# Disty0/sdnq

Hardware: AMD Instinct MI355X
Metric: quantized-matmul GOP/s (SDXL UNet int8 Linear step, bs=1) (higher is better)
Workload: dtype i8; 1 GPU; sdxl_int8: 741 quantized Linear layers of one denoising step, bs=1 (722 w8a8 GEMMs + 19 M=1 layers); parallelism=single GPU, launch=hipGraph replay, activations=bf16, distinct_activation_tensors=446, activation_quant_cache=True, requantized_weight_cache=True, fused_projections=False, linked_projection_groups=71, one_launch_linears=232, weights_dtype=int8, group_size=-1, use_quantized_matmul=True

## Files before the change

include/sdnq_hip.h:

```cpp
#ifndef SDNQ_HIP_H
#define SDNQ_HIP_H

#include <stddef.h>
#include <stdint.h>

#ifdef __cplusplus
extern "C" {
#endif

#define SDNQ_HIP_ABI_VERSION 1

typedef void* sdnq_stream_t;

typedef enum SdnqStatus {
    SDNQ_OK = 0,
    SDNQ_ERR_NULL = -1,
    SDNQ_ERR_DTYPE = -2,
    SDNQ_ERR_SHAPE = -3,
    SDNQ_ERR_ALIGN = -4,
    SDNQ_ERR_UNSUPPORTED = -5,
    SDNQ_ERR_ARCH = -6,
    SDNQ_ERR_LAUNCH = -7,
    SDNQ_ERR_WORKSPACE = -8
} SdnqStatus;

typedef enum SdnqFloat { SDNQ_F32 = 0, SDNQ_BF16 = 1, SDNQ_F16 = 2 } SdnqFloat;

typedef enum SdnqMM { SDNQ_MM_I8 = 0, SDNQ_MM_FP8 = 1, SDNQ_MM_F16 = 2  } SdnqMM;

typedef enum SdnqStorage {
    SDNQ_ST_PACKED_U8 = 0,
    SDNQ_ST_PACKED_I16 = 1,
    SDNQ_ST_RAW8 = 2,
    SDNQ_ST_RAW16 = 3
} SdnqStorage;

typedef enum SdnqKind {
    SDNQ_KIND_INT = 0,
    SDNQ_KIND_UINT = 1,
    SDNQ_KIND_FLOAT = 2,
    SDNQ_KIND_UFLOAT = 3,
    SDNQ_KIND_CODEBOOK = 4
} SdnqKind;

typedef struct SdnqWeight {
    const void* weight;
    const float* scale;
    const float* zero_point;
    const void* svd_up;
    const void* svd_down;
    int32_t n;
    int32_t k;
    int32_t group_size;
    int32_t svd_rank;
    int32_t svd_dtype;
    int32_t storage;
    int32_t kind;
    int32_t bits;
    int32_t exponent;
    int32_t mantissa;
    int32_t native_float;
    int32_t positions;
    int32_t scale_dtype;
} SdnqWeight;

int sdnq_hip_version(void);
const char* sdnq_hip_strerror(int status);
int sdnq_hip_device_supported(int ordinal);

int sdnq_hip_rowquant(const void* x, int x_dtype, int64_t m, int64_t k, int64_t ldx, int mm_dtype,
                      int hadamard_group, void* xq, float* xs, int32_t* rowsum, void* xrot,
                      const void* prefetch, int64_t prefetch_bytes, float* xzp, sdnq_stream_t stream);

int sdnq_hip_rowquant_lp(const void* x, int x_dtype, int64_t m, int64_t k, int64_t ldx, int mm_dtype, int hadamard_group,
                         void* xq, float* xs, int32_t* rowsum, void* xrot, sdnq_stream_t stream);

int sdnq_hip_scaled_mm(int mm_dtype, const void* a, const void* b, const float* sa, const float* sb,
                       const void* bias, int bias_dtype, int bias_ndim, int64_t ld_bias, void* out,
                       int out_dtype, int64_t m, int64_t n, int64_t k, sdnq_stream_t stream);

int sdnq_hip_scaled_mm_tile(int mm_dtype, int out_dtype, int has_bias, int64_t m, int64_t n, int64_t k, int* bm, int* bn, int* threads,
                            int64_t* workgroups);

int sdnq_hip_rowquant_f16(const void* x, int x_dtype, int64_t m, int64_t k, int64_t ldx, void* xq, float* xs, sdnq_stream_t stream);
int sdnq_hip_scaled_mm_f16(const void* a, const void* b, const float* sa, const float* sb, const void* bias, int bias_dtype, int bias_ndim,
                           int64_t ld_bias, void* out, int out_dtype, int64_t m, int64_t n, int64_t k, sdnq_stream_t stream);

int sdnq_hip_lut4_build(const SdnqWeight* w, int mm_dtype, float* ws, int ws_known, void* lut, sdnq_stream_t stream);
int sdnq_hip_scaled_mm_w4(const void* a, const void* codes, const void* lut, const float* sa, const float* sb, const void* bias, int bias_dtype,
                          void* out, int out_dtype, int64_t m, int64_t n, int64_t k, int64_t lda, sdnq_stream_t stream);
int sdnq_hip_scaled_mm_w4_supported(int mm_dtype, int out_dtype, int64_t m, int64_t n, int64_t k);

int sdnq_hip_scaled_mm_lp(int mm_dtype, const void* a, const void* b, const float* sa, const float* sb, const void* bias,
                          int bias_ndim, int64_t ld_bias, const void* t, const void* svd_up, int rank, void* out,
                          int64_t m, int64_t n, int64_t k, sdnq_stream_t stream);

int sdnq_hip_scaled_mm_lp_zp(int mm_dtype, const void* a, const void* b, const float* sa, const float* sb, const void* bias,
                             int bias_ndim, int64_t ld_bias, const void* t, const void* svd_up, int rank, const int32_t* zp_rowsum,
                             const float* zp, void* out, int64_t m, int64_t n, int64_t k, sdnq_stream_t stream);

int sdnq_hip_rowquant_lp_asym(const void* x, int x_dtype, int64_t m, int64_t k, int64_t ldx, int hadamard_group, void* xq, float* xs,
                              float* xzp, int32_t* rowsum, void* xrot, sdnq_stream_t stream);
int sdnq_hip_scaled_mm_lp_uzp(const void* a, const void* b, const float* sa, const float* sb, const void* bias, const int32_t* zp_rowsum,
                              const float* zp, const float* a_zp, const float* w_colsum_scaled, int64_t zp_k, void* out, int64_t m,
                              int64_t n, int64_t k, sdnq_stream_t stream);
int sdnq_hip_scaled_mm_lp_uzp_svd(const void* a, const void* b, const float* sa, const float* sb, const void* bias,
                                  const int32_t* zp_rowsum, const float* zp, const float* a_zp, const float* w_colsum_scaled, int64_t zp_k,
                                  const void* t, const void* svd_up, int rank, void* out, int64_t m, int64_t n, int64_t k,
                                  sdnq_stream_t stream);

int sdnq_hip_scaled_mm_multi(int mm_dtype, const void* a, const void* b, const float* sa, const float* sb, const void* bias,
                             int bias_dtype, void* const* outs, int n_outs, int64_t seg_n, int out_dtype, int64_t m, int64_t n,
                             int64_t k, sdnq_stream_t stream);

int sdnq_hip_linear_w8a16(const void* x, int x_dtype, const void* w, const float* scale, const float* zero_point, const void* bias,
                          void* out, int64_t m, int64_t n, int64_t k, int64_t ldx, sdnq_stream_t stream);

struct SdnqGemmUnit;
int sdnq_hip_linear_w8a16_grouped(const void* x, int x_dtype, const struct SdnqGemmUnit* units, int64_t n_units, int64_t unit_n,
                                  int has_bias, void* out, int64_t m, int64_t k, int64_t ldx, sdnq_stream_t stream);

typedef struct SdnqGemmUnit {
    const void* b;
    const float* sb;
    const void* bias;
    int64_t n_start;
    int32_t n_seg;
    int32_t n_loc;
} SdnqGemmUnit;
int sdnq_hip_scaled_mm_grouped(int mm_dtype, const void* a, const float* sa, const SdnqGemmUnit* units, int64_t n_units,
                               int64_t unit_n, int bias_dtype, void* out, int out_dtype, int64_t m, int64_t k,
                               sdnq_stream_t stream);

void sdnq_hip_set_tile_override(int tile_id);

int sdnq_hip_linear_float_multi(const void* x, const void* wd, const void* bias, int dtype, void* const* outs, int n_outs,
                                int64_t seg_n, int64_t m, int64_t n, int64_t k, int64_t ldx, sdnq_stream_t stream);

int sdnq_hip_dequant(const SdnqWeight* w, int hadamard_group, void* out, int out_dtype, sdnq_stream_t stream);

typedef enum SdnqIds { SDNQ_IDS_I32 = 0, SDNQ_IDS_I64 = 1 } SdnqIds;
int sdnq_hip_embedding(const SdnqWeight* w, int hadamard_group, const void* ids, int ids_dtype, int64_t n_ids,
                       int has_embed_scale, double embed_scale, void* out, int out_dtype, sdnq_stream_t stream);

int64_t sdnq_hip_dequant_loss_workspace_bytes(int64_t n, int64_t k);
int sdnq_hip_dequant_loss(const SdnqWeight* w, int hadamard_group, const void* ref, int ref_dtype, int64_t ld_ref,
                          double* sum_out, void* workspace, int64_t workspace_bytes, sdnq_stream_t stream);

int sdnq_hip_requant(const SdnqWeight* w, int mm_dtype, void* wq, float* ws, sdnq_stream_t stream);

int sdnq_hip_requant_ws(const SdnqWeight* w, int mm_dtype, void* wq, float* ws, int ws_known, sdnq_stream_t stream);

int sdnq_hip_requant_asym(const SdnqWeight* w, void* wq, float* ws, float* wzp, sdnq_stream_t stream);

int sdnq_hip_unpack_mm(const SdnqWeight* w, int mm_dtype, void* wq, sdnq_stream_t stream);

int sdnq_hip_hadamard(const void* x, int dtype, int64_t rows, int64_t k, int64_t ldx, int hadamard_group,
                      void* y, int64_t ldy, sdnq_stream_t stream);

int sdnq_hip_lowrank_down(const void* x, int x_dtype, int64_t m, int64_t k, int64_t ldx, const void* svd_down,
                          int svd_dtype, int rank, void* t, sdnq_stream_t stream);

int sdnq_hip_scaled_mm_lowrank(int mm_dtype, const void* a, const void* b, const float* sa, const float* sb,
                               const void* bias, int bias_dtype, const void* t, const void* svd_up, int svd_dtype,
                               int rank, const int32_t* zp_rowsum, const float* zp, const float* a_zp,
                               const float* w_colsum_scaled, void* out, int out_dtype,
                               int64_t m, int64_t n, int64_t k, sdnq_stream_t stream);

int sdnq_hip_linear_float(const void* x, const void* wd, const void* bias, int dtype, void* out, int64_t m,
                          int64_t n, int64_t k, int64_t ldx, sdnq_stream_t stream);

int sdnq_hip_linear_skinny(const SdnqWeight* w, int hadamard_group, const void* x, const void* bias, int dtype, void* out,
                           int64_t m, int64_t ldx, sdnq_stream_t stream);

int sdnq_hip_quantize_weight(const void* src, int src_dtype, int64_t ld_src, const SdnqWeight* w, float qmin,
                             float qmax, sdnq_stream_t stream);

int sdnq_hip_quantize_codebook(const void* src, int src_dtype, int64_t ld_src, const SdnqWeight* w, int steps, sdnq_stream_t stream);

int sdnq_hip_prefetch(const void* ptr, int64_t bytes, int workgroups, sdnq_stream_t stream);
int sdnq_hip_prefetch_hint(const void* p0, int64_t b0, const void* p1, int64_t b1, const void* p2, int64_t b2, const void* p3, int64_t b3);

#define SDNQ_MAX_TP_RANKS 64
int sdnq_hip_unshard_columns(const void* gathered, void* out, int elem_bytes, int64_t m0, int64_t m_rows, int64_t m,
                             int64_t wmax, int world, const int64_t* starts, sdnq_stream_t stream);

#define SDNQ_MAX_PUSH_RANKS 16
#define SDNQ_SIGNAL_UNCACHED 1
#define SDNQ_SIGNAL_FINEGRAINED 2
#define SDNQ_SIGNAL_HOST_COHERENT 3
int sdnq_hip_signal_alloc(int64_t bytes, int kind, void** ptr, int* granted);
int sdnq_hip_signal_free(void* ptr, int kind);
int sdnq_hip_ipc_export(const void* ptr, void* handle64);
int sdnq_hip_ipc_import(const void* handle64, void** ptr);
int sdnq_hip_ipc_close(void* ptr);
int sdnq_hip_push_post(void* const* post, int world, int rank, uint64_t seq, uint64_t arena_offset, sdnq_stream_t stream);
int sdnq_hip_push_columns(const void* y, int elem_bytes, int64_t rows, int64_t w, int64_t ldy, void* const* arena, void* const* post,
                          void* const* done, int world, int rank, uint64_t seq, int64_t ldc, int64_t col0, int64_t row0, void* ticket,
                          void* status, int timeout_ms, sdnq_stream_t stream);

int sdnq_hip_im2col(const void* x, int dtype, int batch, int channels, int height, int width, int kh, int kw, int stride_h,
                    int stride_w, int pad_h, int pad_w, int dil_h, int dil_w, void* out, sdnq_stream_t stream);

int sdnq_hip_linear_w8a8(int mm_dtype, const void* x, int x_dtype, int64_t m, int64_t k, int64_t ldx, int hadamard_group,
                         void* xq, float* xs, const void* b, const float* sb, const void* bias, int bias_dtype, void* out,
                         int out_dtype, int64_t n, sdnq_stream_t stream);

int sdnq_hip_stream_capture_id(sdnq_stream_t stream, unsigned long long* id);

int sdnq_hip_linear_w8a8_fused(int mm_dtype, const void* x, int x_dtype, int64_t m, int64_t k, int64_t ldx, const void* b, const float* sb,
                               const void* bias, int bias_dtype, void* out, int out_dtype, int64_t n, sdnq_stream_t stream);
int sdnq_hip_linear_w8a8_fused_supported(int mm_dtype, int x_dtype, int out_dtype, int64_t m, int64_t n, int64_t k);

typedef struct SdnqLinearArgs {
    int32_t struct_size;
    int32_t mm_dtype;
    int32_t x_dtype;
    int32_t out_dtype;
    int32_t bias_dtype;
    int32_t svd_dtype;
    int32_t hadamard_group;
    int32_t svd_rank;
    int32_t asymmetric;
    int32_t x_prequantized;
    int64_t m, n, k, ldx;
    const void* x;
    void* out;
    const void* wq;
    const float* ws;
    const void* bias;
    const void* svd_down;
    const void* svd_up;
    const float* zp;
    const float* w_colsum_scaled;
    void* xq;
    float* xs;
    int32_t* rowsum;
    void* xrot;
    float* xzp;
    void* workspace;
    int64_t workspace_bytes;
} SdnqLinearArgs;
int sdnq_hip_linear(const SdnqLinearArgs* args, sdnq_stream_t stream);
int sdnq_hip_linear_workspace_bytes(const SdnqLinearArgs* args, int64_t* bytes);

int sdnq_hip_scaled_mm_nchw(int mm_dtype, const void* a, const void* b, const float* sa, const float* sb, const void* bias,
                            int bias_dtype, void* out, int out_dtype, int64_t m, int64_t n, int64_t k, int64_t hw,
                            sdnq_stream_t stream);

int sdnq_hip_scaled_mm_strided(int mm_dtype, const void* a, int64_t lda, const void* b, const float* sa, const float* sb,
                               const void* bias, int bias_dtype, void* out, int64_t ldc, int out_dtype, int64_t m, int64_t n,
                               int64_t k, int64_t hw, sdnq_stream_t stream);

int sdnq_hip_scaled_mm_lowrank_strided(int mm_dtype, const void* a, int64_t lda, const void* b, const float* sa, const float* sb,
                                       const void* bias, int bias_dtype, const int32_t* zp_rowsum, const float* zp, const float* a_zp,
                                       const float* w_colsum_scaled, int64_t zp_k, void* out, int64_t ldc, int out_dtype, int64_t m,
                                       int64_t n, int64_t k, sdnq_stream_t stream);

int sdnq_hip_linear_float_strided(const void* x, const void* wd, const void* bias, int dtype, void* out, int64_t m,
                                  int64_t n, int64_t k, int64_t ldx, int64_t ldc, sdnq_stream_t stream);

int sdnq_hip_im2col_rowquant(const void* x, int dtype, int batch, int channels, int height, int width, int kh, int kw,
                             int stride_h, int stride_w, int pad_h, int pad_w, int dil_h, int dil_w, int mm_dtype,
                             void* xq, float* xs, void* amax_ws, sdnq_stream_t stream);

int sdnq_hip_im2col_rowquant_z(const void* x, int dtype, int batch, int channels, int height, int width, int kh, int kw,
                               int stride_h, int stride_w, int pad_h, int pad_w, int dil_h, int dil_w, int mm_dtype,
                               void* xq, float* xs, void* zeroed_ws, sdnq_stream_t stream);

int sdnq_hip_linear_skinny_svd(const SdnqWeight* w, const void* svd_down_t, const void* x, const void* bias, int dtype,
                               void* out, int64_t m, int64_t ldx, sdnq_stream_t stream);

int sdnq_hip_attn_prepare(const void* q, const void* k, const void* v, int dtype, int64_t batch, int64_t q_heads,
                          int64_t kv_heads, int64_t q_len, int64_t kv_len, int64_t head_dim, int smooth_k, int hadamard_group,
                          const int64_t* q_strides, const int64_t* k_strides, const int64_t* v_strides, void* qq, float* qs,
                          void* kq, float* ks, void* vt, float* kmean, sdnq_stream_t stream);
int sdnq_hip_attn_fwd(const void* qq, const float* qs, const void* kq, const float* ks, const void* vt, int v_dtype,
                      float sm_scale, int is_causal, const void* mask, int mask_dtype, int64_t mask_stride_b,
                      int64_t mask_stride_h, int64_t mask_stride_q, void* out, int out_dtype, const int64_t* out_strides,
                      int64_t batch, int64_t q_heads, int64_t kv_heads, int64_t q_len, int64_t kv_len, int64_t head_dim,
                      sdnq_stream_t stream);
int sdnq_hip_attn_fwd_q16(const void* q, const int64_t* q_strides, const void* kq, const float* ks, const void* vt, int v_dtype,
                          float sm_scale, int is_causal, const void* mask, int mask_dtype, int64_t mask_stride_b,
                          int64_t mask_stride_h, int64_t mask_stride_q, void* out, int out_dtype, const int64_t* out_strides,
                          int64_t batch, int64_t q_heads, int64_t kv_heads, int64_t q_len, int64_t kv_len, int64_t head_dim,
                          sdnq_stream_t stream);

int sdnq_hip_attn_prepare_ex(const void* q, const void* k, const void* v, int dtype, int64_t batch, int64_t q_heads, int64_t kv_heads,
                             int64_t q_len, int64_t kv_len, int64_t head_dim, int smooth_k, int hadamard_group, const int64_t* q_strides,
                             const int64_t* k_strides, const int64_t* v_strides, int qk_dtype, int pv_dtype, void* qq, float* qs, void* kq,
                             float* ks, void* vt, float* vs, float* kmean, sdnq_stream_t stream);
int sdnq_hip_attn_fwd_ex(const void* qq, const float* qs, const void* kq, const float* ks, const void* vt, const float* vs, int v_dtype,
                         int qk_dtype, int pv_dtype, float sm_scale, int is_causal, const void* mask, int mask_dtype, int64_t mask_stride_b,
                         int64_t mask_stride_h, int64_t mask_stride_q, void* out, int out_dtype, const int64_t* out_strides, int64_t batch,
                         int64_t q_heads, int64_t kv_heads, int64_t q_len, int64_t kv_len, int64_t head_dim, sdnq_stream_t stream);

int64_t sdnq_hip_attn_workspace_bytes(int64_t batch, int64_t q_heads, int64_t kv_heads, int64_t q_len, int64_t kv_len, int64_t head_dim,
                                      int hadamard_group);
int sdnq_hip_attn(const void* q, const void* k, const void* v, int dtype, int64_t batch, int64_t q_heads, int64_t kv_heads, int64_t q_len,
                  int64_t kv_len, int64_t head_dim, const int64_t* q_strides, const int64_t* k_strides, const int64_t* v_strides,
                  int smooth_k, int hadamard_group, float sm_scale, int is_causal, const void* mask, int mask_dtype,
                  int64_t mask_stride_b, int64_t mask_stride_h, int64_t mask_stride_q, void* out, int out_dtype,
                  const int64_t* out_strides, void* workspace, int64_t workspace_bytes, sdnq_stream_t stream);

int sdnq_hip_attn_lse(const void* qq, const float* qs, const void* kq, const float* ks, float sm_scale, int is_causal, const void* mask,
                      int mask_dtype, int64_t mask_stride_b, int64_t mask_stride_h, int64_t mask_stride_q, void* lse, int lse_dtype,
                      int64_t batch, int64_t q_heads, int64_t kv_heads, int64_t q_len, int64_t kv_len, int64_t head_dim, sdnq_stream_t stream);
int sdnq_hip_attn_bwd(const void* qq, const float* qs, const void* kq, const float* ks, const void* v, const int64_t* v_strides, int v_dtype,
                      const void* out, const int64_t* out_strides, const void* grad, const int64_t* grad_strides, int grad_dtype,
                      const void* grad_v, const int64_t* grad_v_strides, const void* lse, float sm_scale, int is_causal, const void* mask,
                      int mask_dtype, int64_t mask_stride_b, int64_t mask_stride_h, int64_t mask_stride_q, float* delta,
                      void* dq, const int64_t* dq_strides, int64_t dq_channels, void* dk, const int64_t* dk_strides, int64_t dk_channels,
                      void* dv, const int64_t* dv_strides, int64_t batch, int64_t q_heads, int64_t kv_heads, int64_t q_len,
                      int64_t kv_len, int64_t head_dim, sdnq_stream_t stream);

int64_t sdnq_hip_colquant_t_workspace_bytes(int64_t r, int64_t c);
int sdnq_hip_colquant_t(const void* x, int x_dtype, int64_t r, int64_t c, int64_t ldx, void* xq_t, int64_t ld_t, float* xs, float* colsum,
                        void* workspace, int64_t workspace_bytes, sdnq_stream_t stream);

int sdnq_hip_adamw_step(void* param, const void* grad, void* exp_avg, void* exp_avg_sq, int dtype, int64_t numel, float lr, float w1,
                        float w2, float bc1, float bc2, float clip, float decay, const float* grad_scale, int sr_param, int sr_state,
                        uint64_t seed, uint64_t offset, sdnq_stream_t stream);
int sdnq_hip_adamw_step_q8(void* param, const void* grad, int dtype, int64_t numel, void* exp_avg_q, float* exp_avg_scale,
                           float* exp_avg_zp, void* exp_avg_sq_q, float* exp_avg_sq_scale, float* exp_avg_sq_zp, float lr, float w1,
                           float w2, float bc1, float bc2, float clip, float decay, const float* grad_scale, int sr_param, int sr_state,
                           uint64_t seed, uint64_t offset, sdnq_stream_t stream);

int sdnq_hip_adamw_multi_capacity(int quantized);
int sdnq_hip_adamw_step_multi(int64_t count, void* const* params, const void* const* grads, void* const* exp_avgs,
                              void* const* exp_avg_sqs, const int64_t* numels, const float* bc1, const float* bc2,
                              const uint64_t* offsets, int dtype, float lr, float w1, float w2, float clip, float decay,
                              const float* grad_scale, int sr_param, int sr_state, uint64_t seed, sdnq_stream_t stream);
int sdnq_hip_adamw_step_multi_q8(int64_t count, void* const* params, const void* const* grads, void* const* exp_avg_qs,
                                 void* const* exp_avg_scales, void* const* exp_avg_zps, void* const* exp_avg_sq_qs,
                                 void* const* exp_avg_sq_scales, void* const* exp_avg_sq_zps, const int64_t* numels, const float* bc1,
                                 const float* bc2, const uint64_t* offsets, int dtype, float lr, float w1, float w2, float clip,
                                 float decay, const float* grad_scale, int sr_param, int sr_state, uint64_t seed, sdnq_stream_t stream);

int sdnq_hip_dequant_convt(const SdnqWeight* w, int groups, int scale_groups, void* out, int out_dtype, sdnq_stream_t stream);
int sdnq_hip_linear_float_f32out(const void* x, const void* wd, int dtype, float* out, int64_t m, int64_t n, int64_t k, int64_t ldx,
                                 sdnq_stream_t stream);
int sdnq_hip_linear_float_f32out_strided(const void* x, const void* wd, int dtype, float* out, int64_t m, int64_t n, int64_t k,
                                         int64_t ldx, int64_t ldc, sdnq_stream_t stream);
int sdnq_hip_col2im(const float* cols, int64_t ldcols, const void* bias, int dtype, void* out, int batch, int channels, int in_d,
                    int in_h, int in_w, int out_d, int out_h, int out_w, int kd, int kh, int kw, int stride_d, int stride_h,
                    int stride_w, int pad_d, int pad_h, int pad_w, int dil_d, int dil_h, int dil_w, sdnq_stream_t stream);

int sdnq_hip_dequant_t(const SdnqWeight* w, void* out, int out_dtype, sdnq_stream_t stream);
int sdnq_hip_transpose2d(const void* x, int dtype, int64_t r, int64_t c, int64_t ldx, void* out, sdnq_stream_t stream);

int sdnq_hip_im2col_bwd(const void* dy, int dtype, int batch, int channels, int out_h, int out_w, int in_h, int in_w, int kh, int kw,
                        int stride_h, int stride_w, int pad_h, int pad_w, int dil_h, int dil_w, int groups, int64_t row0, int64_t rows,
                        void* out, sdnq_stream_t stream);

int sdnq_hip_lowrank_add(const void* t, const void* up, int dtype, int rank, float scale, void* y, int64_t m, int64_t n, int64_t ldy,
                         sdnq_stream_t stream);
int64_t sdnq_hip_lowrank_grad_workspace_bytes(int64_t m, int64_t p, int rank);
int sdnq_hip_lowrank_grad(const void* a, int64_t lda, const void* b, int dtype, int64_t m, int64_t p, int rank, float scale, int out_t,
                          void* out, int out_dtype, void* workspace, int64_t workspace_bytes, sdnq_stream_t stream);

int sdnq_hip_lowrank_down_dropout(const void* x, int dtype, int64_t m, int64_t k, int64_t ldx, const void* down, int rank, void* t,
                                  int threshold, uint64_t seed, uint64_t offset, sdnq_stream_t stream);
int sdnq_hip_lowrank_add_dropout(const void* t, const void* up, int dtype, int rank, float scale, void* y, int64_t m, int64_t n, int64_t ldy,
                                 int threshold, uint64_t seed, uint64_t offset, sdnq_stream_t stream);
int sdnq_hip_lowrank_grad_dropout(const void* a, int64_t lda, const void* b, int dtype, int64_t m, int64_t p, int rank, float scale,
                                  int out_t, void* out, int out_dtype, void* workspace, int64_t workspace_bytes, int threshold,
                                  uint64_t seed, uint64_t offset, sdnq_stream_t stream);

int sdnq_hip_dora_normsq(const SdnqWeight* w, const void* up, const void* down, int dtype, int rank, float scale, float* out,
                         sdnq_stream_t stream);
int sdnq_hip_dora_normsq_dense(const void* wd, int dtype, int64_t n, int64_t k, int64_t ldw, const void* up, const void* down, int rank,
                               float scale, float* out, sdnq_stream_t stream);
int sdnq_hip_lowrank_add_dora(const void* t, const void* up, int dtype, int rank, float scale, void* y, int64_t m, int64_t n, int64_t ldy,
                              const float* c, const void* bias, sdnq_stream_t stream);
int64_t sdnq_hip_dora_bwd_workspace_bytes(int64_t m, int64_t n);
int sdnq_hip_dora_bwd(const void* dy, int64_t lddy, const void* y, int64_t ldy, const void* bias, const float* c, int dtype, int64_t m,
                      int64_t n, void* g, float* q, void* workspace, int64_t workspace_bytes, sdnq_stream_t stream);

int sdnq_hip_conv_lowrank_down(const void* x, int dtype, int batch, int channels, int height, int width, int kh, int kw, int stride_h,
                               int stride_w, int pad_h, int pad_w, int dil_h, int dil_w, const void* down, int rank, void* t,
                               sdnq_stream_t stream);
int64_t sdnq_hip_conv_lowrank_grad_workspace_bytes(int batch, int channels, int height, int width, int kh, int kw, int stride_h,
                                                   int stride_w, int pad_h, int pad_w, int dil_h, int dil_w, int rank);
int sdnq_hip_conv_lowrank_grad(const void* x, int dtype, int batch, int channels, int height, int width, int kh, int kw, int stride_h,
                               int stride_w, int pad_h, int pad_w, int dil_h, int dil_w, const void* g, int rank, float scale, void* out,
                               int out_dtype, void* workspace, int64_t workspace_bytes, sdnq_stream_t stream);

#ifdef __cplusplus
}
#endif
#endif
```

sdnq_amd/capture.py:

```python
from __future__ import annotations

import torch

from . import linear as _L


def _flatten(obj, out):
    if isinstance(obj, torch.Tensor):
        out.append(obj)
        return ("T", tuple(obj.shape), obj.dtype, str(obj.device))
    if isinstance(obj, (tuple, list)):
        return (type(obj).__name__, tuple(_flatten(o, out) for o in obj))
    if isinstance(obj, dict):
        return ("dict", tuple((k, _flatten(obj[k], out)) for k in sorted(obj)))
    try:
        hash(obj)
        return ("V", obj)
    except TypeError:
        return ("V", repr(obj))


def _rebuild(obj, it):
    if isinstance(obj, torch.Tensor):
        return next(it)
    if isinstance(obj, (tuple, list)):
        return type(obj)(_rebuild(o, it) for o in obj)
    if isinstance(obj, dict):
        return {k: _rebuild(obj[k], it) for k in obj}
    return obj


def _fingerprint(model: torch.nn.Module):
    fp = []
    for t in list(model.parameters()) + list(model.buffers()):
        fp.append((t.data_ptr(), t.numel(), t.dtype))
    for mod in model.modules():
        st = mod.__dict__.get("_sdnq_hip_state")
        if st is not None:
            for name in ("mm_weight", "mm_scale"):
                t = getattr(st, name, None)
                if isinstance(t, torch.Tensor):
                    fp.append((t.data_ptr(), t.numel(), t.dtype))
    return hash(tuple(fp))


class CapturedModel:

    def __init__(self, model: torch.nn.Module, args, kwargs, warmup: int = 3, clone_outputs: bool = False, recapture: bool = False, pool=None):
        if not torch.cuda.is_available():
            raise _L.ops._lib.SdnqHipError("sdnq_amd.capture needs a GPU (no CPU fallback)")
        self.model, self.warmup, self.clone_outputs, self.recapture, self.pool = model, max(int(warmup), 1), clone_outputs, recapture, pool
        self.replays = 0
        self.graph = None
        self._capture(args, kwargs)

    def _capture(self, args, kwargs):
        tensors = []
        self._spec = _flatten((args, kwargs), tensors)
        if not tensors or not all(t.is_cuda for t in tensors):
            raise ValueError("sdnq_amd.capture: every tensor argument must live on the GPU (the graph reads static device buffers)")
        self._device = tensors[0].device
        self._static_in = [t.detach().clone() for t in tensors]
        s_args, s_kwargs = _rebuild((args, kwargs), iter(self._static_in))
        self._stream = torch.cuda.Stream(device=self._device)
        self._stream.wait_stream(torch.cuda.current_stream(self._device))
        was_training = self.model.training
        self.model.eval()
        with torch.no_grad(), torch.cuda.stream(self._stream):
            for _ in range(self.warmup):
                _L.clear_activation_cache()
                self.model(*s_args, **s_kwargs)
                _L.join_weight_pipeline()
            self._stream.synchronize()
            _L.clear_activation_cache()
            self.graph = torch.cuda.CUDAGraph()
            with torch.cuda.graph(self.graph, stream=self._stream, **({"pool": self.pool} if self.pool is not None else {})):
                out = self.model(*s_args, **s_kwargs)
                _L.join_weight_pipeline()
            _L.clear_activation_cache()
        torch.cuda.current_stream(self._device).wait_stream(self._stream)
        self.model.train(was_training)
        self._static_out = out
        self._fp = _fingerprint(self.model)

    def __call__(self, *args, **kwargs):
        tensors = []
        spec = _flatten((args, kwargs), tensors)
        if spec != self._spec:
            if not self.recapture:
                raise ValueError("sdnq_amd.capture: the arguments differ from the captured ones in shape, dtype, device or a non-tensor value "
                                 "(capture again, or pass recapture=True)")
            self._capture(args, kwargs)
            tensors = []
            _flatten((args, kwargs), tensors)
        if _fingerprint(self.model) != self._fp:
            if not self.recapture:
                raise RuntimeError("sdnq_amd.capture: the model's parameters moved since the capture (model.to / load_state_dict / "
                                   "apply_sdnq_options_to_model?): the graph would read freed memory -- capture again")
            self._capture(args, kwargs)
        cur = torch.cuda.current_stream(self._device)
        with torch.no_grad():
            for dst, src in zip(self._static_in, tensors):
                if dst.data_ptr() != src.data_ptr():
                    dst.copy_(src, non_blocking=True)
        self.graph.replay()
        self.replays += 1
        del cur
        if self.clone_outputs:
            outs = []
            _flatten(self._static_out, outs)
            return _rebuild(self._static_out, iter([o.clone() for o in outs]))
        return self._static_out


def capture(model: torch.nn.Module, *example_args, warmup: int = 3, clone_outputs: bool = False, recapture: bool = False, pool=None,
            **example_kwargs) -> CapturedModel:
    return CapturedModel(model, example_args, example_kwargs, warmup=warmup, clone_outputs=clone_outputs, recapture=recapture, pool=pool)
```

sdnq_amd/csrc/fastpath.cpp:

```cpp
#define PY_SSIZE_T_CLEAN
#include <Python.h>
#include <structmember.h>

#include <ATen/ATen.h>
#include <c10/hip/HIPFunctions.h>
#include <c10/hip/HIPStream.h>
#include <torch/csrc/autograd/python_variable.h>

#include <dlfcn.h>

#include <atomic>
#include <memory>
#include <mutex>
#include <unordered_map>
#include <vector>

#include "../../include/sdnq_hip.h"

namespace {

decltype(&sdnq_hip_linear_w8a8) f_linear_w8a8 = nullptr;
decltype(&sdnq_hip_linear_w8a8_fused) f_fused = nullptr;
decltype(&sdnq_hip_linear_w8a8_fused_supported) f_fused_supported = nullptr;
decltype(&sdnq_hip_prefetch_hint) f_hint = nullptr;
decltype(&sdnq_hip_stream_capture_id) f_capture_id = nullptr;

std::atomic<long> g_epoch{0};
std::atomic<long> g_fused_calls{0};
std::atomic<long> g_plan_calls{0};
thread_local int t_no_reuse = 0;

int float_code(at::ScalarType t) {
    if (t == at::kBFloat16) return SDNQ_BF16;
    if (t == at::kHalf) return SDNQ_F16;
    if (t == at::kFloat) return SDNQ_F32;
    return -1;
}

struct Unit {
    const void* p[4] = {nullptr, nullptr, nullptr, nullptr};
    int64_t b[4] = {0, 0, 0, 0};
    int nr = 0;
    int device = -1;
    std::weak_ptr<Unit> next;
};
thread_local std::weak_ptr<Unit> t_prev;
thread_local int64_t t_last_hint[9] = {0, 0, 0, 0, 0, 0, 0, 0, 0};

void unit_launch(const std::shared_ptr<Unit>& u) {
    auto prev = t_prev.lock();
    if (prev && prev != u) {
        auto nx = prev->next.lock();
        if (nx != u) prev->next = u;
    }
    t_prev = u;
    auto n1 = u->next.lock();
    if (!n1 || n1->device != u->device) return;
    auto n2 = n1->next.lock();
    const void* p[4] = {nullptr, nullptr, nullptr, nullptr};
    int64_t b[4] = {0, 0, 0, 0};
    int c = 0;
    for (int i = 0; i < n1->nr && c < 4; ++i, ++c) { p[c] = n1->p[i]; b[c] = n1->b[i]; }
    if (n2 && n2 != u && n2->device == u->device)
        for (int i = 0; i < n2->nr && c < 4; ++i, ++c) { p[c] = n2->p[i]; b[c] = n2->b[i]; }
    if (c == 0 || !f_hint) return;
    t_last_hint[0] += 1;
    for (int i = 0; i < 4; ++i) { t_last_hint[1 + 2 * i] = (int64_t)(uintptr_t)p[i]; t_last_hint[2 + 2 * i] = b[i]; }
    f_hint(p[0], b[0], p[1], b[1], p[2], b[2], p[3], b[3]);
}

struct UnitObj {
    PyObject_HEAD
    std::shared_ptr<Unit>* u;
};

PyObject* unit_new(PyTypeObject* type, PyObject* args, PyObject*) {
    PyObject* ranges;
    int device;
    if (!PyArg_ParseTuple(args, "Oi", &ranges, &device)) return nullptr;
    PyObject* seq = PySequence_Fast(ranges, "ranges must be a sequence of (address, bytes)");
    if (!seq) return nullptr;
    auto u = std::make_shared<Unit>();
    u->device = device;
    Py_ssize_t n = PySequence_Fast_GET_SIZE(seq);
    if (n > 4) { Py_DECREF(seq); PyErr_SetString(PyExc_ValueError, "at most four ranges"); return nullptr; }
    for (Py_ssize_t i = 0; i < n; ++i) {
        unsigned long long ptr;
        long long bytes;
        if (!PyArg_ParseTuple(PySequence_Fast_GET_ITEM(seq, i), "KL", &ptr, &bytes)) { Py_DECREF(seq); return nullptr; }
        u->p[i] = (const void*)(uintptr_t)ptr;
        u->b[i] = bytes;
    }
    u->nr = (int)n;
    Py_DECREF(seq);
    UnitObj* self = (UnitObj*)type->tp_alloc(type, 0);
    if (!self) return nullptr;
    self->u = new std::shared_ptr<Unit>(std::move(u));
    return (PyObject*)self;
}
void unit_dealloc(UnitObj* self) {
    delete self->u;
    Py_TYPE(self)->tp_free((PyObject*)self);
}
PyObject* unit_launch_py(UnitObj* self, PyObject*) {
    unit_launch(*self->u);
    Py_RETURN_NONE;
}
PyMethodDef unit_methods[] = {{"launch", (PyCFunction)unit_launch_py, METH_NOARGS, "this unit launches now: link it behind the thread's previous unit, hand its successors' weights to the library"},
                              {nullptr, nullptr, 0, nullptr}};
PyTypeObject UnitType = {PyVarObject_HEAD_INIT(nullptr, 0)};

struct TensorKey {
    const void* ptr = nullptr;
    int64_t offset = 0, version = 0;
    std::vector<int64_t> sizes, strides;
    bool matches(const at::Tensor& t) const {
        return t.data_ptr() == ptr && t.storage_offset() == offset && (int64_t)t._version() == version && t.sizes() == at::IntArrayRef(sizes) &&
               t.strides() == at::IntArrayRef(strides);
    }
    void take(const at::Tensor& t) {
        ptr = t.data_ptr();
        offset = t.storage_offset();
        version = (int64_t)t._version();
        sizes = t.sizes().vec();
        strides = t.strides().vec();
    }
};

void* current_stream_of(const at::Tensor& t) {
    if (!t.is_cuda()) return nullptr;
    return (void*)c10::hip::getCurrentHIPStream(t.device().index()).stream();
}

struct GroupObj {
    PyObject_HEAD
    int n;
    int wasted;
    PyObject* input;
    TensorKey* key;
    void* stream;
    std::vector<PyObject*>* outs;
    std::vector<uint8_t>* pending;
    int n_pending;
};

void group_clear(GroupObj* g) {
    Py_CLEAR(g->input);
    for (PyObject* o : *g->outs) Py_XDECREF(o);
    g->outs->clear();
    std::fill(g->pending->begin(), g->pending->end(), (uint8_t)0);
    g->n_pending = 0;
}

PyObject* group_new(PyTypeObject* type, PyObject* args, PyObject*) {
    int n;
    if (!PyArg_ParseTuple(args, "i", &n)) return nullptr;
    if (n <= 0) { PyErr_SetString(PyExc_ValueError, "a group has at least one member"); return nullptr; }
    GroupObj* g = (GroupObj*)type->tp_alloc(type, 0);
    if (!g) return nullptr;
    g->n = n;
    g->wasted = 0;
    g->input = nullptr;
    g->key = new TensorKey();
    g->stream = nullptr;
    g->outs = new std::vector<PyObject*>();
    g->pending = new std::vector<uint8_t>((size_t)n, (uint8_t)0);
    g->n_pending = 0;
    return (PyObject*)g;
}
void group_dealloc(GroupObj* g) {
    group_clear(g);
    delete g->key;
    delete g->outs;
    delete g->pending;
    Py_TYPE(g)->tp_free((PyObject*)g);
}

PyObject* group_claim(GroupObj* g, int idx, PyObject* input_obj, const at::Tensor& x) {
    if (g->input == nullptr || g->input != input_obj || idx < 0 || idx >= g->n || !(*g->pending)[(size_t)idx]) return nullptr;
    if (x.is_inference() || !g->key->matches(x) || current_stream_of(x) != g->stream) return nullptr;
    const at::Tensor& o = THPVariable_Unpack((*g->outs)[(size_t)idx]);
    std::vector<int64_t> shape = x.sizes().vec();
    shape.back() = o.size(-1);
    at::Tensor y = o.view(shape);
    (*g->pending)[(size_t)idx] = 0;
    if (--g->n_pending == 0) {
        group_clear(g);
        g->wasted = 0;
    }
    return THPVariable_Wrap(y);
}

PyObject* group_claim_py(GroupObj* g, PyObject* args) {
    int idx;
    PyObject* input;
    if (!PyArg_ParseTuple(args, "iO", &idx, &input)) return nullptr;
    if (!THPVariable_Check(input)) Py_RETURN_NONE;
    try {
        PyObject* y = group_claim(g, idx, input, THPVariable_Unpack(input));
        if (y) return y;
        if (PyErr_Occurred()) return nullptr;
    } catch (const std::exception& e) {
        PyErr_SetString(PyExc_RuntimeError, e.what());
        return nullptr;
    }
    Py_RETURN_NONE;
}

PyObject* group_publish_py(GroupObj* g, PyObject* args) {
    PyObject *input, *outs;
    if (!PyArg_ParseTuple(args, "OO", &input, &outs)) return nullptr;
    if (!THPVariable_Check(input)) { PyErr_SetString(PyExc_TypeError, "input must be a tensor"); return nullptr; }
    PyObject* seq = PySequence_Fast(outs, "outs must be a sequence of tensors");
    if (!seq) return nullptr;
    if (PySequence_Fast_GET_SIZE(seq) != g->n) { Py_DECREF(seq); PyErr_SetString(PyExc_ValueError, "one output per member"); return nullptr; }
    for (Py_ssize_t i = 0; i < g->n; ++i)
        if (!THPVariable_Check(PySequence_Fast_GET_ITEM(seq, i))) { Py_DECREF(seq); PyErr_SetString(PyExc_TypeError, "outs must be tensors"); return nullptr; }
    try {
        const at::Tensor& x = THPVariable_Unpack(input);
        group_clear(g);
        if (x.is_inference()) { Py_DECREF(seq); Py_RETURN_NONE; }
        g->key->take(x);
        g->stream = current_stream_of(x);
    } catch (const std::exception& e) {
        Py_DECREF(seq);
        PyErr_SetString(PyExc_RuntimeError, e.what());
        return nullptr;
    }
    Py_INCREF(input);
    g->input = input;
    for (Py_ssize_t i = 0; i < g->n; ++i) {
        PyObject* o = PySequence_Fast_GET_ITEM(seq, i);
        Py_INCREF(o);
        g->outs->push_back(o);
        (*g->pending)[(size_t)i] = 1;
    }
    g->n_pending = g->n;
    Py_DECREF(seq);
    Py_RETURN_NONE;
}

PyObject* group_clear_py(GroupObj* g, PyObject*) {
    group_clear(g);
    Py_RETURN_NONE;
}
PyObject* group_pending_py(GroupObj* g, PyObject*) { return PyLong_FromLong(g->n_pending); }
PyObject* group_peek_py(GroupObj* g, PyObject*) {
    if (!g->input) Py_RETURN_NONE;
    PyObject* outs = PyList_New((Py_ssize_t)g->outs->size());
    if (!outs) return nullptr;
    for (size_t i = 0; i < g->outs->size(); ++i) {
        Py_INCREF((*g->outs)[i]);
        PyList_SET_ITEM(outs, (Py_ssize_t)i, (*g->outs)[i]);
    }
    PyObject* pend = PySet_New(nullptr);
    if (!pend) { Py_DECREF(outs); return nullptr; }
    for (int i = 0; i < g->n; ++i)
        if ((*g->pending)[(size_t)i]) {
            PyObject* v = PyLong_FromLong(i);
            PySet_Add(pend, v);
            Py_DECREF(v);
        }
    return Py_BuildValue("(ONN)", g->input, outs, pend);
}

PyMethodDef group_methods[] = {
    {"claim", (PyCFunction)group_claim_py, METH_VARARGS, "claim(idx, input) -> member idx's output as input.shape[:-1] + (N,), or None"},
    {"publish", (PyCFunction)group_publish_py, METH_VARARGS, "publish(input, outs): the group's launch computed outs from input"},
    {"clear", (PyCFunction)group_clear_py, METH_NOARGS, "forget the stored outputs"},
    {"pending", (PyCFunction)group_pending_py, METH_NOARGS, "how many stored outputs nobody has claimed"},
    {"peek", (PyCFunction)group_peek_py, METH_NOARGS, "(input, outputs, pending indices) or None"},
    {nullptr, nullptr, 0, nullptr}};
PyMemberDef group_members[] = {{"wasted", T_INT, offsetof(GroupObj, wasted), 0, "consecutive computes whose outputs were not all claimed"},
                               {nullptr, 0, 0, 0, nullptr}};
PyTypeObject GroupType = {PyVarObject_HEAD_INIT(nullptr, 0)};

struct WsKey {
    int dev;
    void* stream;
    bool operator==(const WsKey& o) const { return dev == o.dev && stream == o.stream; }
};
struct WsHash {
    size_t operator()(const WsKey& k) const { return std::hash<void*>()(k.stream) ^ (size_t)(k.dev * 0x9e3779b1u); }
};
std::unordered_map<WsKey, at::Tensor, WsHash>& workspaces() {
    static auto* m = new std::unordered_map<WsKey, at::Tensor, WsHash>();
    return *m;
}

uintptr_t workspace(const at::Tensor& like, void* stream, int64_t nbytes) {
    WsKey key{(int)like.device().index(), stream};
    auto& m = workspaces();
    auto it = m.find(key);
    if (it == m.end() || it->second.numel() < nbytes + 255) {
        at::Tensor buf = at::empty({std::max<int64_t>(nbytes, (int64_t)1 << 20) + 255}, like.options().dtype(at::kByte));
        m[key] = buf;
        return ((uintptr_t)buf.data_ptr() + 255) & ~(uintptr_t)255;
    }
    return ((uintptr_t)it->second.data_ptr() + 255) & ~(uintptr_t)255;
}

struct KeyEnt {
    PyObject* name;
    PyObject* ref;
    const void* ptr;
    int64_t version;
};

struct PlanObj {
    PyObject_HEAD
    vectorcallfunc vc;
    std::vector<KeyEnt>* keys;
    at::Tensor* wq;
    at::Tensor* ws;
    at::Tensor* bias;
    int mm, had, device, bias_code;
    int64_t n, k;
    bool allow_fused, allow_ws;
    std::shared_ptr<Unit>* unit;
    GroupObj* group;
    int idx;
    long epoch;
    std::vector<std::pair<int64_t, int>>* fused_yes;
    std::vector<std::pair<int64_t, int>>* fused_no;
};

PyObject *s_parameters, *s_buffers;

int64_t param_version(const at::Tensor& t) { return t.is_inference() ? -1 : (int64_t)t._version(); }

PyObject* module_attr(PyObject* dict, PyObject* params, PyObject* name) {
    PyObject* t = params ? PyDict_GetItem(params, name) : nullptr;
    if (t) return t;
    t = PyDict_GetItem(dict, name);
    if (t) return t;
    PyObject* buffers = PyDict_GetItem(dict, s_buffers);
    t = buffers ? PyDict_GetItem(buffers, name) : nullptr;
    return t ? t : Py_None;
}

bool keys_current(PlanObj* p, PyObject* mod) {
    PyObject** dp = _PyObject_GetDictPtr(mod);
    if (!dp || !*dp) return false;
    PyObject* params = PyDict_GetItem(*dp, s_parameters);
    for (const KeyEnt& e : *p->keys) {
        PyObject* t = module_attr(*dp, params, e.name);
        if (t != e.ref) return false;
        if (t == Py_None) continue;
        const at::Tensor& tt = THPVariable_Unpack(t);
        if (tt.data_ptr() != e.ptr || param_version(tt) != e.version) return false;
    }
    return true;
}

PyObject* plan_call(PyObject* self, PyObject* const* args, size_t nargsf, PyObject* kwnames) {
    PlanObj* p = (PlanObj*)self;
    if (PyVectorcall_NARGS(nargsf) != 2 || (kwnames && PyTuple_GET_SIZE(kwnames))) {
        PyErr_SetString(PyExc_TypeError, "Plan(mod, input)");
        return nullptr;
    }
    PyObject* mod = args[0];
    PyObject* in = args[1];
    if (p->epoch != g_epoch.load(std::memory_order_relaxed)) Py_RETURN_FALSE;
    if (!THPVariable_CheckExact(in)) Py_RETURN_NONE;
    try {
        const at::Tensor& x = THPVariable_Unpack(in);
        if (!x.is_cuda() || x.device().index() != p->device || x.dim() < 1 || x.size(-1) != p->k) Py_RETURN_NONE;
        const int code = float_code(x.scalar_type());
        if (code != SDNQ_BF16 && code != SDNQ_F16) Py_RETURN_NONE;
        const int64_t m = x.numel() / p->k;
        if (m < 32) Py_RETURN_NONE;
        if ((int)c10::hip::current_device() != p->device) Py_RETURN_NONE;
        if (!keys_current(p, mod)) Py_RETURN_FALSE;
        if (p->group) {
            if (t_no_reuse) Py_RETURN_NONE;
            PyObject* y = group_claim(p->group, p->idx, in, x);
            if (y) { g_plan_calls.fetch_add(1, std::memory_order_relaxed); return y; }
            if (PyErr_Occurred()) return nullptr;
            Py_RETURN_NONE;
        }
        at::Tensor x2 = x.dim() == 2 ? x : x.reshape({-1, p->k});
        if (x2.stride(-1) != 1 || (x2.stride(0) * (int64_t)x2.element_size()) % 16) x2 = x2.contiguous();
        void* stream = (void*)c10::hip::getCurrentHIPStream((c10::DeviceIndex)p->device).stream();
        bool fused = false;
        if (p->allow_fused && x2.stride(0) * 128 < ((int64_t)1 << 31)) {
            const std::pair<int64_t, int> q{m, code};
            bool known = false;
            for (auto& e : *p->fused_yes) if (e == q) { fused = true; known = true; break; }
            if (!known) for (auto& e : *p->fused_no) if (e == q) { known = true; break; }
            if (!known) {
                fused = f_fused_supported(p->mm, code, code, m, p->n, p->k) != 0;
                auto* v = fused ? p->fused_yes : p->fused_no;
                if (v->size() < 64) v->push_back(q);
            }
        }
        if (!fused) {
            if (!p->allow_ws) Py_RETURN_NONE;
            unsigned long long cap = 0;
            if (f_capture_id(stream, &cap) != SDNQ_OK || cap != 0) Py_RETURN_NONE;
        }
        if (p->unit) unit_launch(*p->unit);
        at::Tensor out = at::empty({m, p->n}, x.options());
        const void* bias = p->bias->defined() ? p->bias->data_ptr() : nullptr;
        int rc;
        if (fused) {
            rc = f_fused(p->mm, x2.data_ptr(), code, m, p->k, x2.stride(0), p->wq->data_ptr(), (const float*)p->ws->data_ptr(), bias, p->bias_code,
                         out.data_ptr(), code, p->n, stream);
            g_fused_calls.fetch_add(1, std::memory_order_relaxed);
        } else {
            const int64_t xq_bytes = (m * p->k + 255) & ~(int64_t)255;
            const uintptr_t base = workspace(x, stream, xq_bytes + 4 * m + 512);
            rc = f_linear_w8a8(p->mm, x2.data_ptr(), code, m, p->k, x2.stride(0), p->had, (void*)base, (float*)(base + (uintptr_t)xq_bytes), p->wq->data_ptr(),
                               (const float*)p->ws->data_ptr(), bias, p->bias_code, out.data_ptr(), code, p->n, stream);
        }
        if (rc != SDNQ_OK) Py_RETURN_NONE;
        g_plan_calls.fetch_add(1, std::memory_order_relaxed);
        if (x.dim() == 2) return THPVariable_Wrap(out);
        std::vector<int64_t> shape = x.sizes().vec();
        shape.back() = p->n;
        return THPVariable_Wrap(out.view(shape));
    } catch (const std::exception& e) {
        PyErr_SetString(PyExc_RuntimeError, e.what());
        return nullptr;
    }
}

PyObject* plan_new(PyTypeObject* type, PyObject* args, PyObject* kw) {
    static const char* kwlist[] = {"names", "refs", "mm", "n", "k", "wq", "ws", "bias", "had", "allow_fused", "allow_ws", "unit", "group", "idx", nullptr};
    PyObject *names, *refs, *wq = Py_None, *ws = Py_None, *bias = Py_None, *unit = Py_None, *group = Py_None;
    int mm = 0, had = 0, allow_fused = 0, allow_ws = 0, idx = 0;
    long long n = 0, k = 0;
    if (!PyArg_ParseTupleAndKeywords(args, kw, "OOiLL|OOOippOOi", (char**)kwlist, &names, &refs, &mm, &n, &k, &wq, &ws, &bias, &had, &allow_fused, &allow_ws, &unit,
                                     &group, &idx))
        return nullptr;
    if (!PyTuple_Check(names) || !PyTuple_Check(refs) || PyTuple_GET_SIZE(names) != PyTuple_GET_SIZE(refs)) {
        PyErr_SetString(PyExc_TypeError, "names and refs must be tuples of one length");
        return nullptr;
    }
    if (unit != Py_None && !PyObject_TypeCheck(unit, &UnitType)) { PyErr_SetString(PyExc_TypeError, "unit must be a Unit"); return nullptr; }
    if (group != Py_None && !PyObject_TypeCheck(group, &GroupType)) { PyErr_SetString(PyExc_TypeError, "group must be a Group"); return nullptr; }
    if (group == Py_None && (!THPVariable_Check(wq) || !THPVariable_Check(ws))) { PyErr_SetString(PyExc_TypeError, "wq / ws must be tensors"); return nullptr; }
    if (bias != Py_None && !THPVariable_Check(bias)) { PyErr_SetString(PyExc_TypeError, "bias must be a tensor or None"); return nullptr; }
    PlanObj* p = (PlanObj*)type->tp_alloc(type, 0);
    if (!p) return nullptr;
    p->vc = plan_call;
    p->keys = new std::vector<KeyEnt>();
    p->wq = new at::Tensor();
    p->ws = new at::Tensor();
    p->bias = new at::Tensor();
    p->unit = nullptr;
    p->group = nullptr;
    p->fused_yes = new std::vector<std::pair<int64_t, int>>();
    p->fused_no = new std::vector<std::pair<int64_t, int>>();
    p->mm = mm; p->had = had; p->n = n; p->k = k; p->idx = idx; p->device = -1; p->bias_code = 0;
    p->allow_fused = allow_fused != 0;
    p->allow_ws = allow_ws != 0;
    p->epoch = g_epoch.load();
    try {
        for (Py_ssize_t i = 0; i < PyTuple_GET_SIZE(names); ++i) {
            PyObject* name = PyTuple_GET_ITEM(names, i);
            PyObject* ref = PyTuple_GET_ITEM(refs, i);
            if (!PyUnicode_Check(name) || (ref != Py_None && !THPVariable_Check(ref))) {
                PyErr_SetString(PyExc_TypeError, "names must be str, refs tensors or None");
                Py_DECREF(p);
                return nullptr;
            }
            KeyEnt e{name, ref, nullptr, 0};
            Py_INCREF(name);
            PyUnicode_InternInPlace(&e.name);
            Py_INCREF(ref);
            if (ref != Py_None) {
                const at::Tensor& t = THPVariable_Unpack(ref);
                e.ptr = t.data_ptr();
                e.version = param_version(t);
                if (p->device < 0 && t.is_cuda()) p->device = (int)t.device().index();
            }
            p->keys->push_back(e);
        }
        if (group != Py_None) {
            Py_INCREF(group);
            p->group = (GroupObj*)group;
        } else {
            *p->wq = THPVariable_Unpack(wq);
            *p->ws = THPVariable_Unpack(ws);
            if (!p->wq->is_cuda() || !p->ws->is_cuda() || p->ws->scalar_type() != at::kFloat || !p->ws->is_contiguous()) {
                PyErr_SetString(PyExc_ValueError, "wq / ws must be device tensors, ws contiguous float32");
                Py_DECREF(p);
                return nullptr;
            }
            p->device = (int)p->wq->device().index();
            if (bias != Py_None) {
                *p->bias = THPVariable_Unpack(bias);
                p->bias_code = float_code(p->bias->scalar_type());
                if (!p->bias->is_cuda() || !p->bias->is_contiguous() || p->bias_code < 0 || p->bias->numel() != n) {
                    PyErr_SetString(PyExc_ValueError, "bias must be a contiguous device tensor of N floats");
                    Py_DECREF(p);
                    return nullptr;
                }
            }
            if (unit != Py_None) p->unit = new std::shared_ptr<Unit>(*((UnitObj*)unit)->u);
        }
    } catch (const std::exception& e) {
        PyErr_SetString(PyExc_RuntimeError, e.what());
        Py_DECREF(p);
        return nullptr;
    }
    if (p->device < 0) {
        PyErr_SetString(PyExc_ValueError, "a plan needs parameters on a device");
        Py_DECREF(p);
        return nullptr;
    }
    return (PyObject*)p;
}

void plan_dealloc(PlanObj* p) {
    if (p->keys) {
        for (KeyEnt& e : *p->keys) { Py_XDECREF(e.name); Py_XDECREF(e.ref); }
        delete p->keys;
    }
    delete p->wq;
    delete p->ws;
    delete p->bias;
    delete p->unit;
    Py_XDECREF((PyObject*)p->group);
    delete p->fused_yes;
    delete p->fused_no;
    Py_TYPE(p)->tp_free((PyObject*)p);
}
PyMemberDef plan_members[] = {{"mm", T_INT, offsetof(PlanObj, mm), READONLY, "matmul dtype code of the forward this plan restates"},
                              {nullptr, 0, 0, 0, nullptr}};
PyTypeObject PlanType = {PyVarObject_HEAD_INIT(nullptr, 0)};

PyObject* m_init(PyObject*, PyObject* arg) {
    const char* path = PyUnicode_AsUTF8(arg);
    if (!path) return nullptr;
    void* h = dlopen(path, RTLD_NOW | RTLD_GLOBAL);
    if (!h) { PyErr_Format(PyExc_OSError, "dlopen(%s): %s", path, dlerror()); return nullptr; }
#define RESOLVE(var, name)                                                                                          \
    var = (decltype(var))dlsym(h, #name);                                                                           \
    if (!var) { PyErr_Format(PyExc_OSError, "%s does not export " #name, path); return nullptr; }
    RESOLVE(f_linear_w8a8, sdnq_hip_linear_w8a8)
    RESOLVE(f_fused, sdnq_hip_linear_w8a8_fused)
    RESOLVE(f_fused_supported, sdnq_hip_linear_w8a8_fused_supported)
    RESOLVE(f_hint, sdnq_hip_prefetch_hint)
    RESOLVE(f_capture_id, sdnq_hip_stream_capture_id)
#undef RESOLVE
    Py_RETURN_NONE;
}
PyObject* m_bump_epoch(PyObject*, PyObject*) { return PyLong_FromLong(g_epoch.fetch_add(1) + 1); }
PyObject* m_set_no_reuse(PyObject*, PyObject* arg) {
    long v = PyLong_AsLong(arg);
    if (v == -1 && PyErr_Occurred()) return nullptr;
    t_no_reuse = (int)v;
    Py_RETURN_NONE;
}
PyObject* m_chain_reset(PyObject*, PyObject*) {
    t_prev.reset();
    Py_RETURN_NONE;
}
PyObject* m_last_hint(PyObject*, PyObject*) {
    PyObject* t = PyTuple_New(9);
    if (!t) return nullptr;
    for (int i = 0; i < 9; ++i) PyTuple_SET_ITEM(t, i, PyLong_FromLongLong(t_last_hint[i]));
    return t;
}
PyObject* m_fused_calls(PyObject*, PyObject*) { return PyLong_FromLong(g_fused_calls.load()); }
PyObject* m_plan_calls(PyObject*, PyObject*) { return PyLong_FromLong(g_plan_calls.load()); }
PyObject* m_reset_counters(PyObject*, PyObject*) {
    g_fused_calls = 0;
    g_plan_calls = 0;
    Py_RETURN_NONE;
}

PyMethodDef module_methods[] = {
    {"init", m_init, METH_O, "init(path of libsdnq_hip.so): resolve the entry points the plans launch"},
    {"bump_epoch", m_bump_epoch, METH_NOARGS, "every plan made so far is stale from now on"},
    {"set_no_reuse", m_set_no_reuse, METH_O, "this thread's identity_reuse_disabled() depth"},
    {"chain_reset", m_chain_reset, METH_NOARGS, "this thread's prefetch chain forgets its last unit"},
    {"last_hint", m_last_hint, METH_NOARGS, "(hints handed to the library by this thread, then the ranges of the last one)"},
    {"fused_calls", m_fused_calls, METH_NOARGS, "plan calls that took the one-launch route"},
    {"plan_calls", m_plan_calls, METH_NOARGS, "calls a plan carried"},
    {"reset_counters", m_reset_counters, METH_NOARGS, ""},
    {nullptr, nullptr, 0, nullptr}};
struct PyModuleDef module_def = {PyModuleDef_HEAD_INIT, "_fastpath", "host-side fast path of the eager SDNQ Linear forward (see csrc/fastpath.cpp)", -1, module_methods};

}

PyMODINIT_FUNC PyInit__fastpath(void) {
    s_parameters = PyUnicode_InternFromString("_parameters");
    s_buffers = PyUnicode_InternFromString("_buffers");

    UnitType.tp_name = "sdnq_amd._fastpath.Unit";
    UnitType.tp_basicsize = sizeof(UnitObj);
    UnitType.tp_flags = Py_TPFLAGS_DEFAULT;
    UnitType.tp_new = unit_new;
    UnitType.tp_dealloc = (destructor)unit_dealloc;
    UnitType.tp_methods = unit_methods;

    GroupType.tp_name = "sdnq_amd._fastpath.Group";
    GroupType.tp_basicsize = sizeof(GroupObj);
    GroupType.tp_flags = Py_TPFLAGS_DEFAULT;
    GroupType.tp_new = group_new;
    GroupType.tp_dealloc = (destructor)group_dealloc;
    GroupType.tp_methods = group_methods;
    GroupType.tp_members = group_members;

    PlanType.tp_name = "sdnq_amd._fastpath.Plan";
    PlanType.tp_basicsize = sizeof(PlanObj);
    PlanType.tp_flags = Py_TPFLAGS_DEFAULT | Py_TPFLAGS_HAVE_VECTORCALL;
    PlanType.tp_new = plan_new;
    PlanType.tp_dealloc = (destructor)plan_dealloc;
    PlanType.tp_members = plan_members;
    PlanType.tp_call = PyVectorcall_Call;
    PlanType.tp_vectorcall_offset = offsetof(PlanObj, vc);

    if (PyType_Ready(&UnitType) < 0 || PyType_Ready(&GroupType) < 0 || PyType_Ready(&PlanType) < 0) return nullptr;
    PyObject* m = PyModule_Create(&module_def);
    if (!m) return nullptr;
    Py_INCREF(&UnitType);
    Py_INCREF(&GroupType);
    Py_INCREF(&PlanType);
    PyModule_AddObject(m, "Unit", (PyObject*)&UnitType);
    PyModule_AddObject(m, "Group", (PyObject*)&GroupType);
    PyModule_AddObject(m, "Plan", (PyObject*)&PlanType);
    return m;
}
```

sdnq_amd/csrc/gemm_aq.hip:

```cpp
#include "gemm_dev.h"
#include "quant8_dev.h"

namespace {

constexpr int BK = 128, NW = 8, NT = NW * 64;

struct AqParams {
    const float* sb;
    const void* bias;
    void* out;
    int64_t ldc;
    int bias_dtype;
    const uint8_t* pf_ptr[4];
    int pf_lines[4];
    unsigned long long* trace;
#ifdef SDNQ_AQ_LAB
    int lab;
#endif
};

typedef unsigned short us2 __attribute__((ext_vector_type(2)));

template <int MM> struct AqMma;
template <> struct AqMma<SDNQ_MM_I8> {
    typedef v16i acc_t;
    typedef v4i frag_t;
    static constexpr int KB = 32;
    static __device__ __forceinline__ frag_t load(const uint8_t* s, int r, int ks, int fgrp) {
        return *(const v4i*)(s + r * 128 + (((ks * 2 + fgrp) ^ ((r >> 1) & 7)) << 4));
    }
    static __device__ __forceinline__ void mma(acc_t& c, const frag_t& w, const frag_t& x) { c = __builtin_amdgcn_mfma_i32_32x32x32_i8(w, x, c, 0, 0, 0); }
    static __device__ __forceinline__ float tof(const acc_t& c, int i) { return (float)c[i]; }
};
template <> struct AqMma<SDNQ_MM_FP8> {
    typedef v16f acc_t;
    typedef v8i frag_t;
    static constexpr int KB = 64;
    static __device__ __forceinline__ frag_t load(const uint8_t* s, int r, int ks, int fgrp) {
        const int sw = (r >> 1) & 7;
        const v4i lo = *(const v4i*)(s + r * 128 + (((ks * 4 + fgrp * 2) ^ sw) << 4));
        const v4i hi = *(const v4i*)(s + r * 128 + (((ks * 4 + fgrp * 2 + 1) ^ sw) << 4));
        return (v8i){lo[0], lo[1], lo[2], lo[3], hi[0], hi[1], hi[2], hi[3]};
    }
    static __device__ __forceinline__ void mma(acc_t& c, const frag_t& w, const frag_t& x) {
        c = __builtin_amdgcn_mfma_scale_f32_32x32x64_f8f6f4(w, x, c, 0, 0, 0, 0x7f7f7f7f, 0, 0x7f7f7f7f);
    }
    static __device__ __forceinline__ float tof(const acc_t& c, int i) { return c[i]; }
};

template <int X_T, int MM, bool HAS_BIAS, int NJ, int NSB, int BM, int BN>
__global__ __launch_bounds__(NT) void linear_aq_kernel(const uint16_t* __restrict__ x, const uint8_t* __restrict__ w, int ldx, int ldb, int M, int N,
                                                       int K, int tiles_m, int tiles_n, int group_m, AqParams p_) {
    SDNQ_KERNARGS_NOW("s"(x), "s"(w), "s"(ldx), "s"(ldb), "s"(M), "s"(N), "s"(K), "s"(tiles_m), "s"(tiles_n), "s"(group_m));
    const AqParams& p = p_;
    typedef AqMma<MM> MT;
    constexpr int NACC = (BM / 32) * (BN / 32) / NW;
    static_assert(BM % 32 == 0 && BN % 32 == 0 && NACC * NW == (BM / 32) * (BN / 32) && NACC >= 1 && NACC <= 2, "one or two 32x32 accumulators per wave");
    constexpr int A_STAGE = BM * BK, B_STAGE = BN * BK;
    constexpr int PS = BM / (4 * NW);
    constexpr int PPW = BN / (8 * NW);
    static_assert(PS >= 1 && PS <= 4 && PS * 4 * NW == BM && PPW >= 1 && PPW * 8 * NW == BN && BN <= NT, "geometry");
    constexpr bool SLAB = BN / 32 == NW;
    constexpr int KS = BK / MT::KB;
    static_assert(!SLAB || (NSB <= NJ && PPW == 4), "register slab: the ring is no deeper than the stages held; a wave's 32 rows are four pieces");
    extern __shared__ __attribute__((aligned(1024))) uint8_t lds[];
    uint8_t* const ldsA = lds;
    uint8_t* const ldsB = lds + NJ * A_STAGE;
    float* const s_sb = (float*)(ldsB + NSB * B_STAGE);
    float* const s_bias = s_sb + BN;
    float* const s_xs = s_bias + BN;

    const int tid = threadIdx.x, lane = tid & 63;
    const int wave = __builtin_amdgcn_readfirstlane(tid >> 6);
    const int nwg = tiles_m * tiles_n;
    const int bid = blockIdx.x;
    if (bid >= nwg) {
        SDNQ_PREFETCH_LINES(tid, bid - nwg, NT, (int)gridDim.x - nwg, p);
        return;
    }
    const unsigned long long t_entry = __builtin_amdgcn_s_memtime();
    int tile_m, tile_n;
    grouped_tile(xcd_contiguous(bid, nwg), tiles_m, tiles_n, group_m, tile_m, tile_n);
    const int m0 = tile_m * BM, n0 = tile_n * BN;
    const int nk = K / BK;
    const int m_rows = (M - m0) < BM ? (M - m0) : BM, n_lim = (N - n0) < BN ? (N - n0) : BN;

    const auto rsX = SDNQ_MAKE_RSRC_N((const uint8_t*)x + (int64_t)m0 * ldx * 2, ((int64_t)(m_rows - 1) * ldx + K) * 2);
    v4i xr[PS][NJ];
    int qrow[PS];
#pragma unroll
    for (int ps = 0; ps < PS; ++ps) {
        qrow[ps] = wave * (4 * PS) + ps * 4 + (lane >> 4);
        const int rc = qrow[ps] < m_rows ? qrow[ps] : m_rows - 1;
        const int vo = rc * ldx * 2 + (lane & 15) * 16;
#pragma unroll
        for (int j = 0; j < NJ; ++j) xr[ps][j] = SDNQ_BUF_LOAD16(rsX, vo, j < nk ? j * 256 : 0x40000000);
    }
    const auto rsB = SDNQ_MAKE_RSRC_N(w + (int64_t)n0 * ldb, (int64_t)(n_lim - 1) * ldb + K);
    int voB[PPW];
    auto pieceB = [&](int u) { return SLAB ? wave * PPW + u : wave + u * NW; };
#pragma unroll
    for (int u = 0; u < PPW; ++u) {
        const int r = pieceB(u) * 8 + (lane >> 3);
        const int rc = r < n_lim ? r : n_lim - 1;
        voB[u] = rc * ldb + (((lane & 7) ^ ((r >> 1) & 7)) << 4);
    }
    auto issueB = [&](int st, int slot) {
        const int s = st < nk ? st : 0;
#pragma unroll
        for (int u = 0; u < PPW; ++u) SDNQ_DMA16(rsB, ldsB + slot * B_STAGE + pieceB(u) * 1024, voB[u], s * BK);
    };
    constexpr int AHEAD = SLAB ? NSB : NSB - 1;
#pragma unroll
    for (int s = 0; s < AHEAD; ++s) issueB(s, s);
    __builtin_amdgcn_sched_barrier(0);
    SDNQ_KERNARGS_NOW("s"(p_.sb), "s"(p_.bias), "s"(p_.out), "s"(p_.ldc), "s"(p_.bias_dtype), "s"(p_.trace));
    if (p.trace != nullptr && tid == 0 && blockIdx.x < 1024) p.trace[blockIdx.x * 8] = t_entry;
    SDNQ_PHASE_STAMP(p.trace, 1);
    float ev_sb = 0.0f;
    u32 ev_bias = 0;
    if (tid < BN) {
        const int64_t gi = n0 + (tid < n_lim ? tid : n_lim - 1);
        ev_sb = p.sb[gi];
        if constexpr (HAS_BIAS) {
            if (p.bias_dtype == SDNQ_F32) ev_bias = ((const u32*)p.bias)[gi];
            else ev_bias = ((const uint16_t*)p.bias)[gi];
        }
    }

    constexpr float QMAX = (MM == SDNQ_MM_I8) ? 127.0f : 448.0f;
    constexpr int DF = !SLAB ? 0 : (NJ < 2 ? NJ : 2);
    typename MT::frag_t fbr[DF > 0 ? DF : 1][KS], fbs[KS];
    auto drainB = [&](int j, typename MT::frag_t* dst) {
        if (j < nk) {
            static_for_up<NJ>([&](auto jc) {
                constexpr int later = NJ - 1 - decltype(jc)::value;
                if (decltype(jc)::value == j) wait_vmcnt<PPW * (later < NSB - 1 ? later : NSB - 1)>();
            });
#ifdef SDNQ_AQ_LAB
            if (!(p.lab & 2))
#endif
            static_for_up<KS>([&](auto ksc) { dst[decltype(ksc)::value] = MT::load(ldsB + (j % NSB) * B_STAGE, wave * 32 + (lane & 31), decltype(ksc)::value, lane >> 5); });
            asm volatile("s_waitcnt lgkmcnt(0)" ::: "memory");
        }
        if (j + NSB < NJ) issueB(j + NSB, j % NSB);
    };
#pragma unroll
    for (int ps = 0; ps < PS; ++ps) {
        static_for_up<PS>([&](auto pc) {
            if (decltype(pc)::value == ps) wait_vmcnt<(PS - 1 - decltype(pc)::value) * NJ + PPW * AHEAD>();
        });
        us2 mx = {0, 0};
#pragma unroll
        for (int j = 0; j < NJ; ++j)
#pragma unroll
            for (int d = 0; d < 4; ++d)
                mx = __builtin_elementwise_max(mx, __builtin_bit_cast(us2, (u32)xr[ps][j][d] & 0x7fff7fffu));
        u32 m32 = __builtin_bit_cast(u32, mx);
#pragma unroll
        for (int s = 1; s <= 8; s <<= 1) {
            const u32 o = (u32)lane_xor_i32((int)m32, s);
            m32 = __builtin_bit_cast(u32, __builtin_elementwise_max(__builtin_bit_cast(us2, m32), __builtin_bit_cast(us2, o)));
        }
        u32 mb = (m32 & 0xffffu) > (m32 >> 16) ? (m32 & 0xffffu) : (m32 >> 16);
        constexpr u32 INF_BITS = X_T == SDNQ_BF16 ? 0x7f80u : 0x7c00u;
        if (__builtin_amdgcn_ballot_w64(mb > INF_BITS) != 0) {
            u32 mn = 0;
#pragma unroll
            for (int j = 0; j < NJ; ++j)
#pragma unroll
                for (int d = 0; d < 4; ++d) {
                    const u32 lo = (u32)xr[ps][j][d] & 0x7fffu, hi = ((u32)xr[ps][j][d] >> 16) & 0x7fffu;
                    mn = lo > INF_BITS ? mn : (lo > mn ? lo : mn);
                    mn = hi > INF_BITS ? mn : (hi > mn ? hi : mn);
                }
#pragma unroll
            for (int s = 1; s <= 8; s <<= 1) {
                const u32 o = (u32)lane_xor_i32((int)mn, s);
                mn = o > mn ? o : mn;
            }
            mb = mn;
        }
        const float amax = X_T == SDNQ_BF16 ? __uint_as_float(mb << 16) : f16_bits_to_f32((uint16_t)mb);
        const float scale = amax / QMAX;
        RowDiv rd;
        rd.set(scale);
        if ((lane & 15) == 0) s_xs[qrow[ps]] = scale;
        const int r = qrow[ps];
        uint8_t* dst = ldsA + r * 128 + ((lane & 1) << 3) + ((((lane & 15) >> 1) ^ ((r >> 1) & 7)) << 4);
        const bool all_fast = __builtin_amdgcn_ballot_w64(!rd.fast) == 0;
#ifdef SDNQ_AQ_LAB
        if (p.lab & 16) {
            if constexpr (SLAB) {
                if (ps == PS - 1) {
#pragma unroll
                    for (int j = 0; j < DF; ++j) drainB(j, fbr[j]);
                }
            }
            continue;
        }
#endif
        if (all_fast) {
#pragma unroll
            for (int j = 0; j < NJ; ++j) {
                float v[8];
                const v4i t = xr[ps][j];
                Vec16<X_T>::unpack(make_uint4((u32)t[0], (u32)t[1], (u32)t[2], (u32)t[3]), v);
                const uint2 q = quant8_fast<MM>(v, rd);
                *(v2i*)(dst + j * A_STAGE) = (v2i){(int)q.x, (int)q.y};
                if constexpr (DF > 0) { if (ps == PS - 1 && j >= NJ - DF) drainB(j - (NJ - DF), fbr[j - (NJ - DF)]); }
            }
        } else {
#pragma unroll
            for (int j = 0; j < NJ; ++j) {
                float v[8];
                const v4i t = xr[ps][j];
                Vec16<X_T>::unpack(make_uint4((u32)t[0], (u32)t[1], (u32)t[2], (u32)t[3]), v);
                int isum = 0;
                const uint2 q = quant8<MM>(v, rd, isum);
                *(v2i*)(dst + j * A_STAGE) = (v2i){(int)q.x, (int)q.y};
                if constexpr (DF > 0) { if (ps == PS - 1 && j >= NJ - DF) drainB(j - (NJ - DF), fbr[j - (NJ - DF)]); }
            }
        }
    }
    if (tid < BN && !SLAB) {
        s_sb[tid] = ev_sb;
        if constexpr (HAS_BIAS)
            s_bias[tid] = p.bias_dtype == SDNQ_F32 ? __uint_as_float(ev_bias) : (p.bias_dtype == SDNQ_BF16 ? __uint_as_float(ev_bias << 16) : f16_bits_to_f32((uint16_t)ev_bias));
    }
    SDNQ_PHASE_STAMP(p.trace, 2);

    typename MT::acc_t acc[NACC];
#pragma unroll
    for (int a = 0; a < NACC; ++a)
#pragma unroll
        for (int e = 0; e < 16; ++e) acc[a][e] = 0;
    const int wm = (wave / (BN / 32)) * NACC, wn = wave % (BN / 32);
    const int frow = lane & 31, fgrp = lane >> 5;
    asm volatile("s_waitcnt lgkmcnt(0)" ::: "memory");
#ifdef SDNQ_AQ_LAB
    const int lab = __builtin_amdgcn_readfirstlane(p.lab);
#else
    constexpr int lab = 0;
#endif
    typename MT::frag_t fa[2][NACC][KS];
    if constexpr (SLAB) {
        auto read_a = [&](auto setc, auto ksc, int st) {
            constexpr int sx = decltype(setc)::value, ks = decltype(ksc)::value;
#pragma unroll
            for (int a = 0; a < NACC; ++a) fa[sx][a][ks] = MT::load(ldsA + (st < nk ? st : 0) * A_STAGE, (wm + a) * 32 + frow, ks, fgrp);
        };
        __builtin_amdgcn_s_barrier();
        __builtin_amdgcn_sched_barrier(0);
        static_for_up<KS>([&](auto ksc) { read_a(std::integral_constant<int, 0>{}, ksc, 0); });
        static_for_up<NJ>([&](auto ktc) {
            constexpr int kt = decltype(ktc)::value, sx = kt & 1;
            if (kt < nk) {
                if constexpr (kt >= DF) drainB(kt, fbs);
                __builtin_amdgcn_sched_barrier(0);
                static_for_up<KS>([&](auto ksc) {
                    constexpr int ks = decltype(ksc)::value;
                    if (!(lab & 4)) {
#pragma unroll
                        for (int a = 0; a < NACC; ++a) MT::mma(acc[a], kt < DF ? fbr[kt < DF ? kt : 0][ks] : fbs[ks], fa[sx][a][ks]);
                    }
                    __builtin_amdgcn_sched_barrier(0);
                    if constexpr (kt + 1 < NJ) { if (!(lab & 2)) read_a(std::integral_constant<int, sx ^ 1>{}, ksc, kt + 1); }
                    __builtin_amdgcn_sched_barrier(0);
                });
            }
        });
    } else {
        typename MT::frag_t fb[2][KS];
        auto read_stage = [&](auto setc, auto ksc, int st, int slot) {
            constexpr int sx = decltype(setc)::value, ks = decltype(ksc)::value;
#pragma unroll
            for (int a = 0; a < NACC; ++a) fa[sx][a][ks] = MT::load(ldsA + (st < nk ? st : 0) * A_STAGE, (wm + a) * 32 + frow, ks, fgrp);
            fb[sx][ks] = MT::load(ldsB + slot * B_STAGE, wn * 32 + frow, ks, fgrp);
        };
        wait_vmcnt<(AHEAD - 1) * PPW>();
        __builtin_amdgcn_s_barrier();
        __builtin_amdgcn_sched_barrier(0);
        issueB(AHEAD, AHEAD);
        static_for_up<KS>([&](auto ksc) { read_stage(std::integral_constant<int, 0>{}, ksc, 0, 0); });
        int slot_c = 0;
        auto half = [&](auto setc, int kt) {
            constexpr int sx = decltype(setc)::value;
            wait_vmcnt<(NSB - 2) * PPW>();
            asm volatile("s_waitcnt lgkmcnt(0)" ::: "memory");
            __builtin_amdgcn_sched_barrier(0);
            if (!(lab & 8)) __builtin_amdgcn_s_barrier();
            __builtin_amdgcn_sched_barrier(0);
            const int slot_free = slot_c;
            slot_c = (slot_c + 1 == NSB) ? 0 : slot_c + 1;
            static_for_up<KS>([&](auto ksc) {
                constexpr int ks = decltype(ksc)::value;
                if (!(lab & 4)) {
#pragma unroll
                    for (int a = 0; a < NACC; ++a) MT::mma(acc[a], fb[sx][ks], fa[sx][a][ks]);
                }
                __builtin_amdgcn_sched_barrier(0);
                if (!(lab & 2)) read_stage(std::integral_constant<int, sx ^ 1>{}, ksc, kt + 1, slot_c);
                if constexpr (ks == 0) { if (!(lab & 1)) issueB(kt + NSB, slot_free); }
                __builtin_amdgcn_sched_barrier(0);
            });
        };
#pragma nounroll
        for (int kt = 0; kt < nk; kt += 2) {
            half(std::integral_constant<int, 0>{}, kt);
            if (kt + 1 < nk) half(std::integral_constant<int, 1>{}, kt + 1);
        }
    }
    SDNQ_PHASE_STAMP(p.trace, 3);
    if (tid < BN && SLAB) {
        s_sb[tid] = ev_sb;
        if constexpr (HAS_BIAS)
            s_bias[tid] = p.bias_dtype == SDNQ_F32 ? __uint_as_float(ev_bias) : (p.bias_dtype == SDNQ_BF16 ? __uint_as_float(ev_bias << 16) : f16_bits_to_f32((uint16_t)ev_bias));
    }
    asm volatile("s_waitcnt vmcnt(0)" ::: "memory");
    __syncthreads();
    SDNQ_PHASE_STAMP(p.trace, 4);

    constexpr int OUT_ROW = BN * 2 + 16;
    static_assert(BM * OUT_ROW <= NJ * A_STAGE + NSB * B_STAGE, "output staging fits the operand area");
#pragma unroll
    for (int a = 0; a < NACC; ++a) {
        const int ml = (wm + a) * 32 + frow;
        const float sa = s_xs[ml];
#pragma unroll
        for (int q = 0; q < 4; ++q) {
            const int nl0 = wn * 32 + 8 * q + 4 * fgrp;
            float o[4];
#pragma unroll
            for (int e = 0; e < 4; ++e) {
                const float vv = MT::tof(acc[a], 4 * q + e) * sa;
                if constexpr (HAS_BIAS) o[e] = fmaf(vv, s_sb[nl0 + e], s_bias[nl0 + e]);
                else o[e] = vv * s_sb[nl0 + e];
            }
            *(uint2*)(lds + ml * OUT_ROW + nl0 * 2) = make_uint2(pack2<X_T>(o[0], o[1]), pack2<X_T>(o[2], o[3]));
        }
    }
    __syncthreads();
    SDNQ_PHASE_STAMP(p.trace, 5);
    constexpr int PPR = BN * 2 / 16;
#pragma unroll
    for (int v = tid; v < BM * PPR; v += NT) {
        const int r = v / PPR, c = v % PPR;
        if (r >= m_rows || c * 8 >= n_lim) continue;
        const uint4 val = *(const uint4*)(lds + r * OUT_ROW + c * 16);
        __builtin_nontemporal_store((v4i){(int)val.x, (int)val.y, (int)val.z, (int)val.w},
                                    (v4i*)((uint8_t*)p.out + ((int64_t)(m0 + r) * p.ldc + n0 + c * 8) * 2));
    }
    SDNQ_PHASE_STAMP(p.trace, 6);
}

std::atomic<unsigned long long*> g_aq_trace{nullptr};
std::atomic<int> g_aq_geometry{-1};

constexpr int64_t AQ_TALL_MAX_K = 640;

struct AqPlan { int geometry, bm, bn, tiles_m, tiles_n, group_m, resident; int64_t prefetch_room; };
inline AqPlan aq_plan(int mm_dtype, int64_t m, int64_t n, int64_t k, int cus) {
    static const int geo_env = (int)env_int("SDNQ_HIP_FUSED_ROWQUANT_GEOMETRY", -1);
    static const int gm_env = (int)env_int("SDNQ_HIP_FUSED_ROWQUANT_GROUP_M", 8);
    static const int gm_tall_env = (int)env_int("SDNQ_HIP_FUSED_ROWQUANT_GROUP_M_TALL", 8);
    static const int tall = env_int("SDNQ_HIP_FUSED_ROWQUANT_TALL_GEOMETRY", 2) == 3 ? 3 : 2;
    struct Geo { int bm, bn, resident; };
    static constexpr Geo GEOS[4] = {{64, 128, 1}, {32, 256, 1}, {64, 128, 2}, {128, 128, 1}};
    const bool tall_ok = mm_dtype == SDNQ_MM_I8 && k <= AQ_TALL_MAX_K;
    auto tiles_of = [&](int g) { return ((m + GEOS[g].bm - 1) / GEOS[g].bm) * ((n + GEOS[g].bn - 1) / GEOS[g].bn); };
    int geo = g_aq_geometry.load(std::memory_order_relaxed);
    if (geo < 0) geo = geo_env;
    if (geo > 3 || (geo >= 2 && !tall_ok)) geo = -1;
    if (geo < 0) {
        if (mm_dtype == SDNQ_MM_I8 && k > 640 && (n % 256) == 0 && ((m + 31) / 32) * (n / 256) <= cus) geo = 1;
        else if (tall_ok && tiles_of(0) > cus && tiles_of(tall) <= (int64_t)GEOS[tall].resident * cus) geo = tall;
        else geo = 0;
    }
    AqPlan pl;
    pl.geometry = geo;
    pl.bm = GEOS[geo].bm;
    pl.bn = GEOS[geo].bn;
    pl.resident = GEOS[geo].resident;
    pl.tiles_m = (int)((m + pl.bm - 1) / pl.bm);
    pl.tiles_n = (int)((n + pl.bn - 1) / pl.bn);
    const int gm_e = geo >= 2 ? gm_tall_env : gm_env;
    const int gm = gm_e < 1 ? 1 : gm_e;
    pl.group_m = gm > pl.tiles_m ? pl.tiles_m : gm;
    pl.prefetch_room = (int64_t)pl.resident * cus - (int64_t)pl.tiles_m * pl.tiles_n;
    return pl;
}

template <int X_T, int MM, bool HAS_BIAS, int NJ, int NSB, int BM, int BN, int RESIDENT = 1>
int launch_aq(const void* x, const void* w, int64_t ldx, int64_t m, int64_t n, int64_t k, const AqPlan& pl, AqParams p, hipStream_t s) {
    constexpr int LDS_BYTES = NJ * BM * BK + NSB * BN * BK + (2 * BN + BM) * 4;
    static_assert(RESIDENT * LDS_BYTES <= 160 * 1024 && (RESIDENT + 1) * LDS_BYTES > 160 * 1024, "LDS budget: exactly RESIDENT workgroups per CU (aq_plan's prefetch room)");
    auto kern = linear_aq_kernel<X_T, MM, HAS_BIAS, NJ, NSB, BM, BN>;
    static std::atomic<uint64_t> attr_devices{0};
    if (LDS_BYTES > 64 * 1024 && !allow_dynamic_lds((const void*)kern, LDS_BYTES, attr_devices)) return SDNQ_ERR_LAUNCH;
    if (pl.bm != BM || pl.bn != BN || pl.resident != RESIDENT) return SDNQ_ERR_LAUNCH;
    const int tiles_m = pl.tiles_m, tiles_n = pl.tiles_n, group_m = pl.group_m;
    const int64_t tiles = (int64_t)tiles_m * tiles_n;
    p.trace = g_aq_trace.load(std::memory_order_relaxed);
#ifdef SDNQ_AQ_LAB
    p.lab = (int)env_int("SDNQ_HIP_AQ_LAB", 0);
#endif
    const int pf_wgs = sdnq_internal_take_prefetch(pl.prefetch_room, NT, p.pf_ptr, p.pf_lines);
    hipLaunchKernelGGL(kern, dim3((unsigned)(tiles + pf_wgs)), dim3(NT), LDS_BYTES, s, (const uint16_t*)x, (const uint8_t*)w, (int)ldx, (int)k, (int)m,
                       (int)n, (int)k, tiles_m, tiles_n, group_m, p);
    SDNQ_CHECK_LAUNCH();
    return SDNQ_OK;
}

}

extern "C" int sdnq_hip_linear_w8a8_fused_supported(int mm_dtype, int x_dtype, int out_dtype, int64_t m, int64_t n, int64_t k) {
    static const int64_t on = env_int("SDNQ_HIP_FUSED_ROWQUANT", 1), max_tn = env_int("SDNQ_HIP_FUSED_ROWQUANT_MAX_TILES_N", 12),
                         min_m = env_int("SDNQ_HIP_FUSED_ROWQUANT_MIN_M", 33), min_k = env_int("SDNQ_HIP_FUSED_ROWQUANT_MIN_K", 128),
                         max_k = env_int("SDNQ_HIP_FUSED_ROWQUANT_MAX_K", 1280);
    static const int64_t fp8_on = env_int("SDNQ_HIP_FUSED_ROWQUANT_FP8", 0);
    if (!on) return 0;
    if (mm_dtype != SDNQ_MM_I8 && !(mm_dtype == SDNQ_MM_FP8 && fp8_on)) return 0;
    if ((x_dtype != SDNQ_BF16 && x_dtype != SDNQ_F16) || out_dtype != x_dtype) return 0;
    if (m < min_m || n <= 0 || (n % 8) != 0 || k <= 0 || (k % 128) != 0 || k > 1280) return 0;
    const int64_t tiles_m = (m + 63) / 64, tiles_n = (n + 127) / 128;
    if (tiles_n > max_tn || k < min_k || k > max_k) return 0;
    if (tiles_m * tiles_n > (int64_t)cu_count() && aq_plan(mm_dtype, m, n, k, cu_count()).geometry < 2) return 0;
    return 1;
}

extern "C" int sdnq_hip_linear_w8a8_fused(int mm_dtype, const void* x, int x_dtype, int64_t m, int64_t k, int64_t ldx, const void* b,
                                          const float* sb, const void* bias, int bias_dtype, void* out, int out_dtype, int64_t n,
                                          sdnq_stream_t stream) {
    if (!x || !b || !sb || !out) return SDNQ_ERR_NULL;
    if (mm_dtype != SDNQ_MM_I8 && mm_dtype != SDNQ_MM_FP8) return SDNQ_ERR_DTYPE;
    if ((x_dtype != SDNQ_BF16 && x_dtype != SDNQ_F16) || out_dtype != x_dtype) return SDNQ_ERR_UNSUPPORTED;
    if (bias && (bias_dtype < 0 || bias_dtype > 2)) return SDNQ_ERR_DTYPE;
    if (m <= 0 || n <= 0 || k <= 0 || ldx < k || (n % 8) != 0) return SDNQ_ERR_SHAPE;
    if ((k % 128) != 0 || k > 1280) return SDNQ_ERR_UNSUPPORTED;
    if (m > 0x7fffffffll / 2 || n > 0x7fffffffll || ldx * 2 * 128 > 0x7fffffffll || k * 128 > 0x7fffffffll) return SDNQ_ERR_SHAPE;
    if (((uintptr_t)x % 16) || ((uintptr_t)b % 16) || ((uintptr_t)out % 16) || ((ldx * 2) % 16)) return SDNQ_ERR_ALIGN;
    AqParams p{};
    p.sb = sb; p.bias = bias; p.out = out; p.ldc = n; p.bias_dtype = bias_dtype;
    hipStream_t s = (hipStream_t)stream;
    const AqPlan pl = aq_plan(mm_dtype, m, n, k, cu_count());
#define AQ_L(XT, MMV, HB, NJV, ...) launch_aq<XT, MMV, HB, NJV, __VA_ARGS__>(x, b, ldx, m, n, k, pl, p, s)
#define AQ_G(XT, MMV, HB, NJV) (pl.geometry == 1 ? AQ_L(XT, MMV, HB, NJV, 3, 32, 256) : AQ_L(XT, MMV, HB, NJV, 4, 64, 128))
#define AQ_NJ(XT, MMV, HB) (k <= 640 ? AQ_G(XT, MMV, HB, 5) : AQ_G(XT, MMV, HB, 10))
#define AQ_B(XT, MMV) (bias ? AQ_NJ(XT, MMV, true) : AQ_NJ(XT, MMV, false))
#define AQ_X(MMV) (x_dtype == SDNQ_BF16 ? AQ_B(SDNQ_BF16, MMV) : AQ_B(SDNQ_F16, MMV))
#define AQ_TB(XT, ...) (bias ? AQ_L(XT, SDNQ_MM_I8, true, 5, __VA_ARGS__) : AQ_L(XT, SDNQ_MM_I8, false, 5, __VA_ARGS__))
#define AQ_T(...) (x_dtype == SDNQ_BF16 ? AQ_TB(SDNQ_BF16, __VA_ARGS__) : AQ_TB(SDNQ_F16, __VA_ARGS__))
    if (pl.geometry == 2) return AQ_T(2, 64, 128, 2);
    if (pl.geometry == 3) return AQ_T(3, 128, 128, 1);
    return mm_dtype == SDNQ_MM_I8 ? AQ_X(SDNQ_MM_I8) : AQ_X(SDNQ_MM_FP8);
#undef AQ_T
#undef AQ_TB
#undef AQ_X
#undef AQ_B
#undef AQ_NJ
#undef AQ_G
#undef AQ_L
}

void sdnq_internal_aq_trace(unsigned long long* device_buf) { g_aq_trace.store(device_buf, std::memory_order_relaxed); }

void sdnq_internal_aq_geometry(int geometry) { g_aq_geometry.store(geometry < 0 ? -1 : (geometry <= 3 ? geometry : 1), std::memory_order_relaxed); }

void sdnq_internal_aq_plan(int mm_dtype, long long m, long long n, long long k, int cus, long long* out) {
    const AqPlan pl = aq_plan(mm_dtype, m, n, k, cus);
    out[0] = pl.geometry; out[1] = pl.bm; out[2] = pl.bn; out[3] = pl.tiles_m; out[4] = pl.tiles_n; out[5] = pl.group_m; out[6] = pl.prefetch_room;
}
```

sdnq_amd/csrc/gemm_dev.h:

```cpp
#pragma once
#include <atomic>
#include <cstdlib>
#include <type_traits>

#include "sdnq_dev.h"

int sdnq_internal_take_prefetch(int64_t room, int threads, const uint8_t* pf_ptr[4], int pf_lines[4]);
int sdnq_float_gemm(const void* x, const void* w, const void* bias, int dtype, void* out, int64_t m, int64_t n, int64_t k,
                    int64_t ldx, hipStream_t s, void* const* outs = nullptr, int n_outs = 0, int64_t seg_n = 0, int64_t ldc = 0);
int sdnq_float_gemm_f32out(const void* x, const void* w, int dtype, float* out, int64_t m, int64_t n, int64_t k, int64_t ldx, int64_t ldc,
                           hipStream_t s);
bool sdnq_internal_ks_eligible(int64_t m, int64_t n, int64_t k, int64_t lda, int64_t ldb);
bool sdnq_internal_ks_preferred(int64_t m, int64_t n, int64_t k);
int sdnq_internal_scaled_mm_ks(const void* a, const void* b, const float* sa, const float* sb, const void* bias, int bias_dtype, void* out,
                               int out_dtype, int64_t m, int64_t n, int64_t k, int64_t lda, int64_t ldb, int64_t ldc, hipStream_t s);
void sdnq_internal_ks_trace(unsigned long long* device_buf);
void sdnq_internal_aq_trace(unsigned long long* device_buf);
void sdnq_internal_aq_geometry(int geometry);
void sdnq_internal_aq_plan(int mm_dtype, long long m, long long n, long long k, int cus, long long* out);

template <int N> __device__ __forceinline__ void wait_vmcnt() { asm volatile("s_waitcnt vmcnt(%0)" ::"n"(N) : "memory"); }

template <int N, int I = 0, typename F> __device__ __forceinline__ void static_for_up(F&& f) {
    if constexpr (I < N) {
        f(std::integral_constant<int, I>{});
        static_for_up<N, I + 1>(f);
    }
}

#define SDNQ_PHASE_STAMP(trace, slot)                                                                                                      \
    do {                                                                                                                                   \
        if ((trace) != nullptr && threadIdx.x == 0 && blockIdx.x < 1024) (trace)[blockIdx.x * 8 + (slot)] = __builtin_amdgcn_s_memtime(); \
    } while (0)

__device__ __forceinline__ int xcd_contiguous(int bid, int nwg) {
    const int q = nwg / 8, r = nwg % 8, xcd = bid % 8, j = bid / 8;
    return (xcd < r ? xcd * (q + 1) : r * (q + 1) + (xcd - r) * q) + j;
}

__device__ __forceinline__ void grouped_tile(int pos, int tiles_m, int tiles_n, int group_m, int& tile_m, int& tile_n) {
    const int per_group = group_m * tiles_n;
    const int gid = pos / per_group, first_m = gid * group_m;
    const int gsz = (tiles_m - first_m) < group_m ? (tiles_m - first_m) : group_m;
    const int in_g = pos - gid * per_group;
    tile_n = in_g / gsz;
    tile_m = first_m + in_g - tile_n * gsz;
}

#define SDNQ_PREFETCH_LINES(tid, wg, nt, nwgs, p)                                                                           \
    do {                                                                                                                    \
        const int t = (wg) * (nt) + (tid), stride = (nwgs) * (nt);                                                          \
        _Pragma("nounroll") for (int r = 0; r < 4; ++r) {                                                                   \
            const uint8_t* base = (p).pf_ptr[r];                                                                            \
            const int lines = (p).pf_lines[r];                                                                              \
            for (int i = t; i < lines; i += stride) {                                                                       \
                int v;                                                                                                      \
                asm volatile("global_load_dword %0, %1, off" : "=v"(v) : "v"(base + (int64_t)i * 128) : "memory");          \
            }                                                                                                               \
        }                                                                                                                   \
        asm volatile("s_waitcnt vmcnt(0)" ::: "memory");                                                                    \
    } while (0)

inline int64_t env_int(const char* name, int64_t dflt) {
    const char* e = getenv(name);
    return e ? atoll(e) : dflt;
}

inline int cu_count() {
    static std::atomic<int> cus[64];
    int dev = 0;
    if (hipGetDevice(&dev) != hipSuccess || dev < 0 || dev >= 64) return 256;
    int v = cus[dev].load(std::memory_order_relaxed);
    if (v == 0) {
        if (hipDeviceGetAttribute(&v, hipDeviceAttributeMultiprocessorCount, dev) != hipSuccess || v <= 0) v = 256;
        cus[dev].store(v, std::memory_order_relaxed);
    }
    return v;
}

inline bool allow_dynamic_lds(const void* kern, int bytes, std::atomic<uint64_t>& attr_devices) {
    int dev = 0;
    if (hipGetDevice(&dev) != hipSuccess) return false;
    const uint64_t bit = 1ull << (dev & 63);
    if (!(attr_devices.load(std::memory_order_acquire) & bit)) {
        if (hipFuncSetAttribute(kern, hipFuncAttributeMaxDynamicSharedMemorySize, bytes) != hipSuccess) return false;
        attr_devices.fetch_or(bit, std::memory_order_release);
    }
    return true;
}
```

sdnq_amd/linear.py:

```python
from __future__ import annotations

import functools
import os

import torch

from . import ops
from .common import dtype_dict

CACHE_WEIGHTS = os.environ.get("SDNQ_HIP_CACHE_WEIGHTS", "1").lower() not in {"0", "false", "no"}
PIPELINE_WEIGHTS = os.environ.get("SDNQ_HIP_PIPELINE_WEIGHTS", "0").lower() not in {"0", "false", "no"}
PREFETCH_WEIGHTS = os.environ.get("SDNQ_HIP_PREFETCH_WEIGHTS", "0").lower() not in {"0", "false", "no"}
PREFETCH_NEXT = os.environ.get("SDNQ_HIP_PREFETCH_NEXT", "1").lower() not in {"0", "false", "no"}
PREFETCH_NEXT_MAX_BYTES = int(os.environ.get("SDNQ_HIP_PREFETCH_NEXT_MAX_MB", "48")) << 20
FUSED_SKINNY = os.environ.get("SDNQ_HIP_FUSED_SKINNY", "1").lower() not in {"0", "false", "no"}
FUSED_DEQUANT_GEMM = os.environ.get("SDNQ_HIP_FUSED_DEQUANT_GEMM", "1").lower() not in {"0", "false", "no"}
FUSED_DEQUANT_GEMM_MAX_FLOP = float(os.environ.get("SDNQ_HIP_FUSED_DEQUANT_GEMM_MAX_FLOP", "4e10"))
FUSED_DEQUANT_GEMM_MAX_K = int(os.environ.get("SDNQ_HIP_FUSED_DEQUANT_GEMM_MAX_K", str(1 << 30)))
FUSED_ROWQUANT = os.environ.get("SDNQ_HIP_FUSED_ROWQUANT", "1").lower() not in {"0", "false", "no"}
FUSED_LUT4 = os.environ.get("SDNQ_HIP_FUSED_LUT4", "1").lower() not in {"0", "false", "no"}
CACHE_ACTIVATIONS = int(os.environ.get("SDNQ_HIP_CACHE_ACTIVATIONS", "12"))
_FP = ops._lib.fastpath()
FAST_PLANS = _FP is not None
_PLAN_NAMES = ("weight", "scale", "zero_point", "svd_up", "svd_down", "bias")


UNSHARED_FAST_PATH = os.environ.get("SDNQ_HIP_UNSHARED_FAST_PATH", "1").lower() not in {"0", "false", "no"}
UNSHARED_AFTER = 2
CACHE_ACTIVATION_BYTES = int(os.environ.get("SDNQ_HIP_CACHE_ACTIVATION_MB", "256")) << 20


def tensor_key(t: torch.Tensor):
    if t.is_inference():
        return None
    return (t.data_ptr(), t.storage_offset(), t.shape, t.stride(), t._version)


def _param_version(t: torch.Tensor) -> int:
    return -1 if t.is_inference() else t._version


class _ActivationCache:

    def __init__(self, size: int | None = None, max_bytes: int | None = None):
        self.size = size
        self.max_bytes = max_bytes
        self.entries = []

    def get(self, t: torch.Tensor, params, key=None):
        if key is None:
            key = None if _no_identity_reuse[0] else tensor_key(t)
        if key is None:
            return None
        for i in range(len(self.entries) - 1, -1, -1):
            e = self.entries[i]
            if e[0] is t and e[1] == key and e[2] == params:
                self.entries.append(self.entries.pop(i))
                e[6][0] = True
                return e[3]
        return None

    def put(self, t: torch.Tensor, params, result, key=None, nbytes=None, producer=None):
        if key is None:
            key = None if _no_identity_reuse[0] else tensor_key(t)
        if key is None:
            return
        if nbytes is None:
            nbytes = t.numel() * t.element_size() + sum(r.numel() * r.element_size() for r in result if isinstance(r, torch.Tensor) and r is not t)
        self.entries.append((t, key, params, result, nbytes, producer, [False]))
        cap = max(CACHE_ACTIVATIONS, 0) if self.size is None else self.size
        lim = CACHE_ACTIVATION_BYTES if self.max_bytes is None else self.max_bytes
        while len(self.entries) > cap or (len(self.entries) > 1 and sum(e[4] for e in self.entries) > lim):
            self._retire(self.entries.pop(0))

    @staticmethod
    def _retire(e):
        mod = e[5]
        if mod is not None:
            d = mod.__dict__
            d["_sdnq_unshared"] = -(1 << 30) if e[6][0] else d.get("_sdnq_unshared", 0) + 1

    def invalidate(self, t: torch.Tensor | None = None):
        if t is None:
            self.clear()
            return
        base = t.untyped_storage().data_ptr() if t.numel() else None
        keep = []
        for e in self.entries:
            if e[0] is not t and (base is None or e[0].untyped_storage().data_ptr() != base):
                keep.append(e)
            else:
                self._retire(e)
        self.entries = keep

    def clear(self):
        for e in self.entries:
            self._retire(e)
        self.entries.clear()


class _ThreadState(__import__("threading").local):

    def __init__(self):
        self.act_cache = _ActivationCache()
        self.no_reuse = 0
        self.weight_pipeline = None


_ts = _ThreadState()


class _PerThread:

    def __init__(self, getter):
        object.__setattr__(self, "_get", getter)

    def __getattr__(self, name):
        return getattr(self._get(), name)

    def __setattr__(self, name, value):
        setattr(self._get(), name, value)


class _PerThreadFlag:

    def __getitem__(self, i):
        return _ts.no_reuse

    def __setitem__(self, i, v):
        _ts.no_reuse = v
        if _FP is not None:
            _FP.set_no_reuse(v)


_act_cache = _PerThread(lambda: _ts.act_cache)

_no_identity_reuse = _PerThreadFlag()


class identity_reuse_disabled:
    def __enter__(self):
        _ts.no_reuse += 1
        if _FP is not None:
            _FP.set_no_reuse(_ts.no_reuse)

    def __exit__(self, *exc):
        _ts.no_reuse -= 1
        if _FP is not None:
            _FP.set_no_reuse(_ts.no_reuse)
        return False
_groups = []
_groups_lock = __import__("threading").Lock()


def clear_activation_cache():
    _ts.act_cache.clear()
    _weight_pipeline.start_step()


def invalidate(tensor: torch.Tensor | None = None):
    _ts.act_cache.invalidate(tensor)
    if tensor is None:
        _weight_pipeline.start_step()
    with _groups_lock:
        _groups[:] = [ref for ref in _groups if ref() is not None]
        live = list(_groups)
    for ref in live:
        g = ref()
        if g is None:
            continue
        if g.last is not None and (tensor is None or g.last[0] is tensor
                                     or (tensor.numel() and g.last[0].untyped_storage().data_ptr() == tensor.untyped_storage().data_ptr())):
            g.last = None


def _rowquant_cached(input: torch.Tensor, k: int, mm: int, had: int, want_rowsum: bool, want_xrot: bool, prefetch, asymmetric=False,
                     cache: bool = True):
    params = (mm, had, want_rowsum, want_xrot, asymmetric, ops._stream(input) if input.is_cuda else -1)
    cache = cache and CACHE_ACTIVATIONS > 0
    if cache:
        hit = _ts.act_cache.get(input, params)
        if hit is not None:
            return hit
    x2 = input.reshape(-1, k)
    if x2.stride(-1) != 1 or (x2.stride(0) * x2.element_size()) % 16:
        x2 = x2.contiguous()
    res = ops.rowquant(x2, mm, had, want_rowsum=want_rowsum, want_xrot=want_xrot, prefetch=prefetch, asymmetric=asymmetric)
    res = (x2,) + tuple(res)
    if cache:
        _ts.act_cache.put(input, params, res)
    return res


class _State:
    __slots__ = ("key", "qw", "mm", "mm_weight", "mm_scale", "mm_zp", "mm_wcs", "svd_up", "svd_down", "svd_down_t", "wd", "bias", "pf", "lut")


class _LaunchUnit:
    __slots__ = ("tensors", "ranges", "next", "device", "c", "__weakref__")

    def __init__(self, tensors):
        self.tensors = tuple(tensors)
        self.device = self.tensors[0].device if self.tensors else None
        if any(t.device != self.device for t in self.tensors):
            self.device = None
        self.ranges = tuple((t.data_ptr(), t.numel() * t.element_size()) for t in self.tensors) if self.device is not None else ()
        if sum(b for _, b in self.ranges) > PREFETCH_NEXT_MAX_BYTES or len(self.ranges) > 4:
            self.ranges = ()
        self.next = None
        self.c = None if _FP is None else _FP.Unit(self.ranges, -1 if self.device is None or self.device.index is None else self.device.index)


class _PrefetchChain:

    def __init__(self):
        import threading
        self._tls = threading.local()

    def launch(self, unit: _LaunchUnit):
        if unit.c is not None:
            unit.c.launch()
            return
        tls = self._tls
        prev = getattr(tls, "prev", None)
        prev = prev() if prev is not None else None
        if prev is not None and prev is not unit:
            nx = prev.next
            if nx is None or nx() is not unit:
                import weakref
                prev.next = weakref.ref(unit)
        import weakref
        tls.prev = weakref.ref(unit)
        n1 = unit.next() if unit.next is not None else None
        if n1 is None:
            return
        if n1.device != unit.device:
            return
        n2 = n1.next() if n1.next is not None else None
        rs = n1.ranges + (n2.ranges if (n2 is not None and n2 is not unit and n2.device == unit.device) else ())
        if not rs:
            return
        rs = (rs + ((0, 0),) * 4)[:4]
        ops._lib.load().sdnq_hip_prefetch_hint(rs[0][0], rs[0][1], rs[1][0], rs[1][1], rs[2][0], rs[2][1], rs[3][0], rs[3][1])

    def reset(self):
        self._tls.prev = None
        if _FP is not None:
            _FP.chain_reset()


_prefetch_chain = _PrefetchChain()


def _pf_launch(holder, tensors):
    unit = holder.pf
    if unit is None or len(unit.tensors) != len(tensors) or any(a is not b for a, b in zip(unit.tensors, tensors)):
        unit = holder.pf = _LaunchUnit(tensors)
    _prefetch_chain.launch(unit)


_STATE_FIELDS = ("weight", "scale", "zero_point", "svd_up", "svd_down")


def _no_grad(fn, plan_mm=None):
    import functools
    grad_on, no_grad = torch.is_grad_enabled, torch.no_grad

    @functools.wraps(fn)
    def forward(self, input):
        plan = self.__dict__.get("_sdnq_plan")
        if plan is not None:
            if plan.mm == plan_mm:
                y = plan(self, input)
                if y is not None:
                    if y is not False:
                        return y
                    del self.__dict__["_sdnq_plan"]
            else:
                del self.__dict__["_sdnq_plan"]
        if grad_on():
            with no_grad():
                return fn(self, input)
        return fn(self, input)
    return forward


def _install_plan(mod, **kw):
    refs = tuple(_attr(mod, name) for name in _PLAN_NAMES)
    try:
        mod.__dict__["_sdnq_plan"] = _FP.Plan(_PLAN_NAMES, refs, **kw)
    except (TypeError, ValueError):
        mod.__dict__["_sdnq_plan_declined"] = True


def drop_plans(mods):
    for m in mods:
        m.__dict__.pop("_sdnq_plan", None)
        m.__dict__.pop("_sdnq_plan_declined", None)


def _attr(mod, name):
    d = mod.__dict__
    t = d["_parameters"].get(name, d)
    if t is d:
        t = d.get(name, d)
        if t is d:
            t = getattr(mod, name, None)
    return t


def _signature(mod):
    out = []
    for name in _STATE_FIELDS:
        t = _attr(mod, name)
        out.append((name, t, None if t is None else t.data_ptr(), None if t is None else _param_version(t)))
    return tuple(out)


def _state(mod) -> _State:
    st = mod.__dict__.get("_sdnq_hip_state")
    if st is not None:
        for name, ref, ptr, ver in st.key:
            t = _attr(mod, name)
            if t is not ref or (t is not None and (t.data_ptr() != ptr or _param_version(t) != ver)):
                break
        else:
            return st
    from .support import require
    require(mod)
    dq = mod.sdnq_dequantizer
    st = _State()
    st.key = _signature(mod)
    st.qw = dq.quant_weight(mod.weight, mod.scale, getattr(mod, "zero_point", None), getattr(mod, "svd_up", None),
                            getattr(mod, "svd_down", None))
    st.mm = None
    st.mm_weight = st.mm_scale = st.mm_zp = st.mm_wcs = None
    st.svd_up, st.svd_down = st.qw.keep[3], st.qw.keep[4]
    st.svd_down_t = None
    st.wd = None
    st.pf = None
    st.lut = None
    mod.__dict__["_sdnq_hip_state"] = st
    return st


def _float_forward(mod, input: torch.Tensor, st: _State) -> torch.Tensor:
    dq = mod.sdnq_dequantizer
    k, n = dq.in_features, dq.out_features
    if input.dtype != dq.result_dtype:
        raise RuntimeError(f"expected input dtype {dq.result_dtype} (the layer's result_dtype) but got {input.dtype}")
    m = input.numel() // input.shape[-1]
    if m == 0:
        if not input.is_cuda:
            raise ops._lib.SdnqHipError("sdnq_amd forwards need CUDA/HIP tensors (no CPU fallback)")
        return input.new_empty(*input.shape[:-1], n)
    if FUSED_SKINNY and m <= 32 and st.svd_up is None and k % 16 == 0:
        x2 = input.reshape(-1, k)
        if x2.stride(-1) != 1 or (x2.stride(0) * x2.element_size()) % 16:
            x2 = x2.contiguous()
        return ops.linear_skinny(st.qw, x2, mod.bias, dq.hadamard_group_size if dq.use_hadamard else 0).view(*input.shape[:-1], n)
    if (FUSED_SKINNY and m <= 4 and st.svd_up is not None and not dq.use_hadamard and not dq.use_codebook and dq.weights_dtype in ("int8", "uint8", "int4", "uint4")
            and (dq.group_size <= 0 or dq.group_size % 4 == 0) and dq.kernel_positions == 1 and k % 32 == 0 and st.svd_up.shape[1] % 16 == 0 and input.dtype in (torch.bfloat16, torch.float16)
            and st.svd_up.dtype == input.dtype and m * k * 4 <= 150 * 1024):
        if st.svd_down_t is None:
            st.svd_down_t = st.svd_down.t().contiguous()
        x2 = input.reshape(-1, k)
        if x2.stride(-1) != 1:
            x2 = x2.contiguous()
        return ops.linear_skinny_svd(st.qw, st.svd_down_t, x2, mod.bias).view(*input.shape[:-1], n)
    group = mod.__dict__.get("_sdnq_group")
    if group is not None and group[0].float_mode and LINK_PROJECTIONS and m > 32 and input.is_cuda and st.wd is None and n % 8 == 0:
        y = group[0].forward_float(mod, group[1], input)
        if y is not None:
            return y
    if (FUSED_DEQUANT_GEMM and m > 32 and st.svd_up is None and not dq.use_hadamard and not dq.use_codebook and dq.weights_dtype in ("int8", "uint8")
            and dq.group_size <= 0 and dq.kernel_positions == 1 and input.dtype in (torch.bfloat16, torch.float16) and k % 16 == 0 and n % 8 == 0
            and st.wd is None and input.is_cuda and 2 * m * n * k <= FUSED_DEQUANT_GEMM_MAX_FLOP and k <= FUSED_DEQUANT_GEMM_MAX_K):
        x2 = input.reshape(-1, k)
        if x2.stride(-1) != 1 or (x2.stride(0) * x2.element_size()) % 16:
            x2 = x2.contiguous()
        w_phys, sc, zp = st.qw.keep[0], st.qw.keep[1], st.qw.keep[2]
        if PREFETCH_NEXT:
            _pf_launch(st, (w_phys,))
        return ops.linear_w8a16(x2, w_phys, sc, zp, _attr(mod, "bias")).view(*input.shape[:-1], n)
    wd = st.wd
    if wd is None:
        wd = ops.dequant(st.qw, dq.result_dtype, dq.hadamard_group_size if dq.use_hadamard else 0)
        if CACHE_WEIGHTS and os.environ.get("SDNQ_HIP_CACHE_DEQUANT", "0") == "1":
            st.wd = wd
    x2 = input.reshape(-1, k)
    if x2.stride(-1) != 1:
        x2 = x2.contiguous()
    y = ops.linear_float(x2, wd, mod.bias)
    return y.view(*input.shape[:-1], n)


@_no_grad
def quantized_linear_forward(self, input: torch.Tensor) -> torch.Tensor:
    return _float_forward(self, input, _state(self))


class _WeightPipeline:

    def __init__(self):
        self.order = {}
        self.prev = None
        self.pending = None
        self.slot = 0
        self.scratch = {}
        self.side = {}
        self.stats = {"prefetched": 0, "inline": 0, "wasted": 0}

    def _buffer(self, dev: torch.device, slot: int, nbytes: int) -> torch.Tensor:
        key = (dev.index, slot)
        buf = self.scratch.get(key)
        if buf is None or buf.numel() < nbytes:
            if torch.cuda.is_current_stream_capturing():
                raise ops._lib.SdnqHipError("per-call weight pipeline: run one eager step before capturing a graph (scratch not sized yet)")
            buf = torch.empty((nbytes + 255) // 256 * 256, device=dev, dtype=torch.uint8)
            self.scratch[key] = buf
        return buf

    def scratch_bytes(self) -> int:
        return sum(b.numel() for b in self.scratch.values())

    def join(self):
        if self.pending is not None:
            torch.cuda.current_stream(self.pending[2].device).wait_event(self.pending[4])
            self.pending = None
            self.stats["wasted"] += 1

    def start_step(self):
        self.join()
        self.prev = None

    def weights(self, mod, st, mm: int, known_ws):
        import weakref
        dev = st.qw.keep[0].device
        cur = torch.cuda.current_stream(dev)
        nbytes = st.qw.n * st.qw.k
        p = self.pending
        if p is not None and p[0] is st and p[1] == mm and p[6] == cur.cuda_stream:
            cur.wait_event(p[4])
            wq, ws, self.slot = p[2], p[3], p[5]
            self.pending = None
            self.stats["prefetched"] += 1
        else:
            self.join()
            self.slot ^= 1
            wq, ws = ops.requant(st.qw, mm, known_ws, out=self._buffer(dev, self.slot, nbytes))
            self.stats["inline"] += 1
        prev = self.prev() if self.prev is not None else None
        if prev is not None:
            self.order[id(prev)] = weakref.ref(mod)
        self.prev = weakref.ref(mod)
        nref = self.order.get(id(mod))
        nxt = nref() if nref is not None else None
        if nxt is not None and nxt is not mod:
            nst = nxt.__dict__.get("_sdnq_hip_state")
            ndq = getattr(nxt, "sdnq_dequantizer", None)
            if (nst is not None and ndq is not None and ndq.re_quantize_for_matmul and nst.mm == (mm, False) and nst.mm_weight is None
                    and nst.mm_scale is not None and nst.qw.keep[0].device == dev):
                side = self.side.get(dev.index)
                if side is None:
                    side = self.side[dev.index] = torch.cuda.Stream(device=dev)
                slot = self.slot ^ 1
                out = self._buffer(dev, slot, nst.qw.n * nst.qw.k)
                start = torch.cuda.Event()
                start.record(cur)
                with torch.cuda.stream(side):
                    side.wait_event(start)
                    nwq, nws = ops.requant(nst.qw, mm, nst.mm_scale, out=out)
                    done = torch.cuda.Event()
                    done.record(side)
                self.pending = (nst, mm, nwq, nws, done, slot, cur.cuda_stream)
        return wq, ws


def _thread_weight_pipeline():
    wp = _ts.weight_pipeline
    if wp is None:
        wp = _ts.weight_pipeline = _WeightPipeline()
    return wp


_weight_pipeline = _PerThread(_thread_weight_pipeline)


def join_weight_pipeline():
    _weight_pipeline.join()


def _prepare_mm_weights(mod, st: _State, mm: int, asymmetric: bool = False, for_group: bool = False):
    dq = mod.sdnq_dequantizer
    key = (mm, asymmetric)
    if st.mm == key and st.mm_weight is not None:
        return st.mm_weight, st.mm_scale, st.mm_zp
    zp = None
    if dq.re_quantize_for_matmul and asymmetric:
        wq, ws, zp = ops.requant_asym(st.qw)
    elif dq.re_quantize_for_matmul:
        known = st.mm_scale if (st.mm == key and st.mm_weight is None) else None
        if not CACHE_WEIGHTS and PIPELINE_WEIGHTS and known is not None and st.qw.keep[0].is_cuda and not for_group:
            wq, ws = _weight_pipeline.weights(mod, st, mm, known)
        else:
            wq, ws = ops.requant(st.qw, mm, known)
    else:
        ws = st.qw.keep[1]
        ent = dtype_dict[dq.weights_dtype]
        plain = (not ent["is_packed"]) and ((mm == ops.MM_I8 and dq.weights_dtype == "int8")
                                            or (mm == ops.MM_FP8 and ent["torch_dtype"] == torch.float8_e4m3fn))
        if plain:
            wq = st.qw.keep[0]
            if wq.dtype == torch.uint8:
                wq = wq.view(torch.int8)
        else:
            wq = ops.unpack_mm(st.qw, mm)
        if mm == ops.MM_I8 and ent["is_unsigned"]:
            zp = st.qw.keep[2]
            if not ent["is_packed"]:
                zp = torch.add(zp, ws, alpha=128) if zp is not None else ws * 128
                if st.qw.scale_dtype != torch.float32:
                    zp = zp.to(st.qw.scale_dtype).float()
    if CACHE_WEIGHTS:
        st.mm, st.mm_weight, st.mm_scale, st.mm_zp, st.mm_wcs = key, wq, ws, zp, None
    elif dq.re_quantize_for_matmul and not asymmetric:
        st.mm, st.mm_weight, st.mm_scale, st.mm_zp, st.mm_wcs = key, None, ws, None, None
    return wq, ws, zp


class ProjectionGroup:

    def __init__(self, mods, float_mode: bool = False):
        import weakref
        self.mods = list(mods)
        self.float_mode = float_mode
        self.sig = None
        self.gemm = None
        self._c = None if _FP is None else _FP.Group(len(self.mods))
        self._last = None
        self._wasted = 0
        self.fallback = None
        self.pf = None
        self.pf_tensors = ()
        with _groups_lock:
            _groups.append(weakref.ref(self))

    @property
    def last(self):
        if self._c is None:
            return self._last
        st = self._c.peek()
        return None if st is None else (st[0], None, None, st[1], st[2])

    @last.setter
    def last(self, value):
        if self._c is None:
            self._last = value
        elif value is None:
            self._c.clear()
        else:
            self._c.publish(value[0], value[3])

    @property
    def wasted(self):
        return self._wasted if self._c is None else self._c.wasted

    @wasted.setter
    def wasted(self, value):
        if self._c is None:
            self._wasted = value
        else:
            self._c.wasted = value

    def dissolve(self):
        for m in self.mods:
            if m.__dict__.get("_sdnq_group", (None,))[0] is self:
                m.__dict__.pop("_sdnq_group", None)
        drop_plans(self.mods)
        self.last = None
        self.gemm = None

    def _member_sig(self, m):
        out = []
        for name in ("weight", "scale", "bias"):
            t = _attr(m, name)
            out.append(None if t is None else (t, t.data_ptr(), _param_version(t), t.device))
        return out

    def _sig_current(self, mm) -> bool:
        sig = self.sig
        if sig is None or sig[0] != mm:
            return False
        for m, ref in zip(self.mods, sig[1]):
            for name, r in zip(("weight", "scale", "bias"), ref):
                t = _attr(m, name)
                if r is None:
                    if t is not None:
                        return False
                elif t is not r[0] or t.data_ptr() != r[1] or _param_version(t) != r[2] or t.device != r[3]:
                    return False
        return True

    def _operands(self, mm):
        if self._sig_current(mm):
            return self.gemm is not None
        self.sig = (mm, [self._member_sig(m) for m in self.mods])
        self.last = None
        self.gemm = None
        devs = set()
        for m in self.mods:
            for name in ("weight", "scale"):
                t = _attr(m, name)
                devs.add(None if t is None else t.device)
        if len(devs) != 1 or None in devs or next(iter(devs)).type != "cuda":
            return False
        try:
            states = [_state(m) for m in self.mods]
            parts = [_prepare_mm_weights(m, st, mm, for_group=True) for m, st in zip(self.mods, states)]
        except ops._lib.SdnqHipError:
            return False
        if any(zp is not None for (_, _, zp) in parts) or len({w.device for (w, _, _) in parts}) != 1:
            return False
        members = []
        for m, (wq, ws, _) in zip(self.mods, parts):
            members.append((wq.reshape(wq.shape[0], -1), ws.reshape(-1), _attr(m, "bias")))
        try:
            self.gemm = ops.GemmGroup(members)
        except ops._lib.SdnqHipError:
            return False
        self.pf_tensors = tuple(wq for (wq, _, _) in parts)
        return True

    def _float_operands(self, input: torch.Tensor) -> bool:
        tag = ("w8a16", input.dtype)
        if self._sig_current(tag):
            return self.gemm is not None
        self.sig = (tag, [self._member_sig(m) for m in self.mods])
        self.last = None
        self.gemm = None
        if input.dtype not in (torch.bfloat16, torch.float16):
            return False
        members = []
        for m in self.mods:
            d = m.sdnq_dequantizer
            st = _state(m)
            bias = _attr(m, "bias")
            if (d.weights_dtype != "int8" or d.group_size > 0 or d.use_hadamard or d.kernel_positions != 1 or st.svd_up is not None
                    or d.in_features % 16 or (bias is not None and bias.dtype != input.dtype) or st.wd is not None):
                return False
            members.append((st.qw.keep[0].view(torch.int8).reshape(d.out_features, -1), st.qw.keep[1].reshape(-1), bias))
        try:
            self.gemm = ops.GemmGroup(members)
        except ops._lib.SdnqHipError:
            return False
        self.pf_tensors = tuple(w for (w, _, _) in members)
        return True

    def _claim(self, idx: int, input: torch.Tensor, key, stream):
        if self._c is not None:
            return self._c.claim(idx, input)
        last = self._last
        if last is None or last[0] is not input or last[1] != key or last[2] != stream or idx not in last[4]:
            return None
        y = last[3][idx].view(*input.shape[:-1], -1)
        last[4].discard(idx)
        if not last[4]:
            self._last = None
            self._wasted = 0
        return y

    def _begin_compute(self) -> bool:
        if (self._c.pending() if self._c is not None else (self._last is not None and self._last[4])):
            self.wasted += 1
            if self.wasted >= 2:
                fallback = self.fallback
                self.dissolve()
                if fallback:
                    from . import loader
                    for mods in fallback:
                        if all("_sdnq_group" not in m.__dict__ for m in mods):
                            loader.link_layers(mods)
                return False
        return True

    def forward(self, mod, idx: int, input: torch.Tensor, mm: int):
        key = None if _ts.no_reuse else tensor_key(input)
        if key is None:
            return None
        stream = ops._stream(input)
        y = self._claim(idx, input, key, stream)
        if y is not None:
            return y
        if not self._begin_compute() or not self._operands(mm):
            return None
        x2, xq, xs, _, _ = _rowquant_cached(input, input.shape[-1], mm, 0, False, False, None)
        if PREFETCH_NEXT:
            _pf_launch(self, self.pf_tensors)
        outs = ops.scaled_mm_grouped(mm, xq, xs, self.gemm, input.dtype)
        self.last = (input, key, stream, outs, set(range(len(self.mods))))
        if FAST_PLANS and self._c is not None and "_sdnq_plan" not in mod.__dict__:
            for i, m in enumerate(self.mods):
                if "_sdnq_plan" not in m.__dict__ and m.__dict__.get("_sdnq_group", (None,))[0] is self:
                    _install_plan(m, mm=mm, n=m.sdnq_dequantizer.out_features, k=m.sdnq_dequantizer.in_features, group=self._c,
                                  idx=m.__dict__["_sdnq_group"][1])
        return self._claim(idx, input, key, stream)

    def forward_float(self, mod, idx: int, input: torch.Tensor):
        key = tensor_key(input)
        if key is None:
            return None
        stream = ops._stream(input)
        y = self._claim(idx, input, key, stream)
        if y is not None:
            return y
        if not self._begin_compute():
            return None
        dq = mod.sdnq_dequantizer
        k, n = dq.in_features, dq.out_features
        x2 = input.reshape(-1, k)
        if x2.stride(-1) != 1 or (x2.stride(0) * x2.element_size()) % 16:
            x2 = x2.contiguous()
        g = len(self.mods)
        if FUSED_DEQUANT_GEMM and self._float_operands(input):
            if PREFETCH_NEXT:
                _pf_launch(self, self.pf_tensors)
            outs = ops.linear_w8a16_grouped(x2, self.gemm)
            self.last = (input, key, stream, outs, set(range(g)))
            return self._claim(idx, input, key, stream)
        wd = torch.empty((g * n, k), device=input.device, dtype=input.dtype)
        for i, m in enumerate(self.mods):
            d = m.sdnq_dequantizer
            ops.dequant(_state(m).qw, input.dtype, d.hadamard_group_size if d.use_hadamard else 0, out=wd[i * n:(i + 1) * n])
        biases = [_attr(m, "bias") for m in self.mods]
        bias = None if biases[0] is None else torch.cat(biases, dim=0)
        outs = ops.linear_float_multi(x2, wd, bias, g)
        self.last = (input, key, stream, outs, set(range(g)))
        return self._claim(idx, input, key, stream)


LINK_PROJECTIONS = os.environ.get("SDNQ_HIP_LINK_PROJECTIONS", "1").lower() not in {"0", "false", "no"}


def _quantized_matmul_forward(self, input: torch.Tensor, mm: int, small_batch_branch: bool = True, cache_input: bool = True) -> torch.Tensor:
    dq = self.sdnq_dequantizer
    st = _state(self)
    k, n = dq.in_features, dq.out_features
    m = input.numel() // input.shape[-1]
    if m == 0 or (small_batch_branch and m < 32):
        return _float_forward(self, input, st)
    if st.qw.scale_dtype != torch.float32:
        return _lp_matmul_forward(self, input, st, mm)
    group = self.__dict__.get("_sdnq_group")
    if group is not None and not group[0].float_mode and LINK_PROJECTIONS and input.is_cuda:
        y = group[0].forward(self, group[1], input, mm)
        if y is not None:
            return y
    if FUSED_LUT4 and not CACHE_WEIGHTS and dq.re_quantize_for_matmul and mm == ops.MM_I8 and st.lut is not False and st.svd_up is None and input.is_cuda:
        y = _lut4_forward(self, input, st, mm, cache_input)
        if y is not None:
            return y
    wq, ws, zp = _prepare_mm_weights(self, st, mm)
    had = dq.hadamard_group_size if dq.use_hadamard else 0
    has_svd = st.svd_up is not None
    bias = _attr(self, "bias")
    pf_on = PREFETCH_NEXT and st.mm_weight is wq and input.is_cuda
    if pf_on:
        _pf_launch(st, (wq,))
    plannable = cache_input and small_batch_branch and group is None and st.mm_weight is wq
    if not has_svd and zp is None and (had == 0 or k <= 5120):
        use_cache = cache_input and CACHE_ACTIVATIONS > 0
        if (FUSED_ROWQUANT and had == 0 and input.is_cuda
                and (not use_cache or (UNSHARED_FAST_PATH and self.__dict__.get("_sdnq_unshared", 0) >= UNSHARED_AFTER))):
            x2 = input if input.dim() == 2 else input.reshape(-1, k)
            if x2.stride(-1) != 1 or (x2.stride(0) * x2.element_size()) % 16:
                x2 = x2.contiguous()
            if ops.linear_w8a8_fused_supported(mm, x2, n, input.dtype):
                y = ops.linear_w8a8_fused(mm, x2, wq, ws, bias, input.dtype)
                if FAST_PLANS and plannable and "_sdnq_plan_declined" not in self.__dict__:
                    _install_plan(self, mm=mm, n=n, k=k, wq=wq, ws=ws, bias=bias, had=0, allow_fused=True,
                                  allow_ws=use_cache and UNSHARED_FAST_PATH, unit=st.pf.c if pf_on else None)
                return y if input.dim() == 2 else y.view(*input.shape[:-1], n)
        if (use_cache and UNSHARED_FAST_PATH and self.__dict__.get("_sdnq_unshared", 0) >= UNSHARED_AFTER and input.is_cuda
                and not torch.cuda.is_current_stream_capturing()):
            x2 = input if input.dim() == 2 else input.reshape(-1, k)
            if x2.stride(-1) != 1 or (x2.stride(0) * x2.element_size()) % 16:
                x2 = x2.contiguous()
            y = ops.linear_w8a8_ws(mm, x2, wq, ws, bias, input.dtype, had)
            if FAST_PLANS and plannable and "_sdnq_plan_declined" not in self.__dict__:
                _install_plan(self, mm=mm, n=n, k=k, wq=wq, ws=ws, bias=bias, had=had, allow_fused=FUSED_ROWQUANT and had == 0, allow_ws=True,
                              unit=st.pf.c if pf_on else None)
            return y if input.dim() == 2 else y.view(*input.shape[:-1], n)
        params = (mm, had, False, False, False, ops._stream(input) if input.is_cuda else -1)
        key = tensor_key(input) if (use_cache and not _ts.no_reuse) else None
        hit = _ts.act_cache.get(input, params, key) if key is not None else None
        if hit is None:
            x2 = input if input.dim() == 2 else input.reshape(-1, k)
            if x2.stride(-1) != 1 or (x2.stride(0) * x2.element_size()) % 16:
                x2 = x2.contiguous()
            if not x2.is_cuda:
                raise ops._lib.SdnqHipError("sdnq_amd forwards need CUDA/HIP tensors (no CPU fallback)")
            y, xq, xs = ops.linear_w8a8(mm, x2, wq, ws, bias, input.dtype, had)
            if key is not None:
                _ts.act_cache.put(input, params, (x2, xq, xs, None, None), key, m * k * (input.element_size() + 1) + 4 * m, self)
            return y if input.dim() == 2 else y.view(*input.shape[:-1], n)
        x2, xq, xs, rowsum, xrot = hit
        return ops.scaled_mm(mm, xq, wq, xs, ws, bias, input.dtype).view(*input.shape[:-1], n)
    params = (mm, had, zp is not None, has_svd, False, ops._stream(input) if input.is_cuda else -1)
    use_cache = cache_input and CACHE_ACTIVATIONS > 0
    key = tensor_key(input) if (use_cache and not _ts.no_reuse) else None
    hit = _ts.act_cache.get(input, params, key) if key is not None else None
    if hit is not None:
        x2, xq, xs, rowsum, xrot = hit
        pre = (xq, xs, rowsum, xrot, None)
    else:
        x2 = input if input.dim() == 2 else input.reshape(-1, k)
        if x2.stride(-1) != 1 or (x2.stride(0) * x2.element_size()) % 16:
            x2 = x2.contiguous()
        pre = None
    svd_ok = (not has_svd) or st.svd_up.dtype == x2.dtype
    if not svd_ok:
        if pre is None:
            x2, xq, xs, rowsum, xrot = _rowquant_cached(input, k, mm, had, zp is not None, has_svd, None, cache=cache_input)
        t = ops.lowrank_down(xrot if xrot is not None else x2, st.svd_down)
        return ops.scaled_mm_lowrank(mm, xq, wq, xs, ws, bias, t, st.svd_up, rowsum, zp, input.dtype).view(*input.shape[:-1], n)
    y, inter = ops.linear_call(mm, x2, wq, ws, bias, input.dtype, had, st.svd_down if has_svd else None, st.svd_up if has_svd else None, zp,
                               pre=pre)
    if hit is None and key is not None:
        _ts.act_cache.put(input, params, (x2,) + tuple(inter[:4]), key)
    return y.view(*input.shape[:-1], n)


def _lut4_forward(self, input: torch.Tensor, st: _State, mm: int, cache_input: bool):
    dq = self.sdnq_dequantizer
    k, n = dq.in_features, dq.out_features
    m = input.numel() // input.shape[-1]
    if not ops.scaled_mm_w4_supported(mm, m, n, k, input.dtype):
        return None
    if st.lut is None:
        ent = dtype_dict[dq.weights_dtype]
        ok = (ent["num_bits"] == 4 and ent["is_packed"] and st.qw.scale_dtype == torch.float32 and dq.kernel_positions == 1 and k % 128 == 0
              and st.qw.group_size % 64 == 0)
        if ok:
            try:
                st.lut = ops.lut4_build(st.qw, mm)
            except ops._lib.SdnqHipError:
                ok = False
        if not ok:
            st.lut = False
            return None
    lut, ws = st.lut
    had = dq.hadamard_group_size if dq.use_hadamard else 0
    x2, xq, xs, _, _ = _rowquant_cached(input, k, mm, had, False, False, None, cache=cache_input)
    if PREFETCH_NEXT:
        _pf_launch(st, (st.qw.keep[0], lut))
    y = ops.scaled_mm_w4(xq, st.qw.keep[0], lut, xs, ws, _attr(self, "bias"), input.dtype)
    return y.view(*input.shape[:-1], n)


def _lp_matmul_forward(self, input: torch.Tensor, st: _State, mm: int) -> torch.Tensor:
    dq = self.sdnq_dequantizer
    sdt = st.qw.scale_dtype
    k, n = dq.in_features, dq.out_features
    if input.dtype != sdt:
        raise NotImplementedError(f"16-bit scales ({sdt}) with {input.dtype} activations are not built (the layer's dtype must match)")
    wq, ws, zp = _prepare_mm_weights(self, st, mm)
    had = dq.hadamard_group_size if dq.use_hadamard else 0
    has_svd = st.svd_up is not None
    bias = _attr(self, "bias")
    x2 = input.reshape(-1, k)
    if x2.stride(-1) != 1 or (x2.stride(0) * x2.element_size()) % 16:
        x2 = x2.contiguous()
    xq, xs, rowsum, xrot = ops.rowquant_lp(x2, mm, had, want_rowsum=zp is not None, want_xrot=has_svd)
    t = ops.lowrank_down(xrot if xrot is not None else x2, st.svd_down) if has_svd else None
    if sdt == torch.bfloat16:
        y = ops.scaled_mm_lp(mm, xq, wq, xs, ws, bias, t, st.svd_up if has_svd else None, rowsum, zp)
    elif has_svd or zp is not None:
        y = ops.scaled_mm_lowrank(mm, xq, wq, xs, ws, bias, t, st.svd_up if has_svd else None, rowsum, zp, input.dtype)
    else:
        y = ops.scaled_mm(mm, xq, wq, xs, ws, bias, input.dtype)
    return y.view(*input.shape[:-1], n)


@functools.partial(_no_grad, plan_mm=ops.MM_I8)
def quantized_linear_forward_int8_matmul(self, input: torch.Tensor) -> torch.Tensor:
    return _quantized_matmul_forward(self, input, ops.MM_I8)


@functools.partial(_no_grad, plan_mm=ops.MM_FP8)
def quantized_linear_forward_fp8_matmul(self, input: torch.Tensor) -> torch.Tensor:
    return _quantized_matmul_forward(self, input, ops.MM_FP8)


def _uint8_matmul_forward(self, input: torch.Tensor, small_batch_branch: bool = True, cache_input: bool = True, conv_form: bool = False) -> torch.Tensor:
    dq = self.sdnq_dequantizer
    st = _state(self)
    k, n = dq.in_features, dq.out_features
    m = input.numel() // input.shape[-1]
    if m == 0 or (small_batch_branch and m < 32):
        return _float_forward(self, input, st)
    if st.qw.scale_dtype != torch.float32:
        return _uint8_lp_matmul_forward(self, input, st, conv_form=conv_form)
    wq, ws, zp = _prepare_mm_weights(self, st, ops.MM_I8, asymmetric=True)
    wcs = st.mm_wcs
    if wcs is None:
        wcs = wq.to(torch.int32).sum(dim=1).to(torch.float32).mul_(ws)
        if CACHE_WEIGHTS:
            st.mm_wcs = wcs
    had = dq.hadamard_group_size if dq.use_hadamard else 0
    has_svd = st.svd_up is not None
    x2, xq, xs, rowsum, xrot, xzp = _rowquant_cached(input, k, ops.MM_I8, had, zp is not None, has_svd,
                                                     wq if PREFETCH_WEIGHTS else None, asymmetric=True, cache=cache_input)
    if conv_form and not has_svd:
        y = torch.empty((xq.shape[0], n), device=xq.device, dtype=input.dtype)
        ops.scaled_mm_zp_into(ops.MM_I8, xq, wq, xs, ws.reshape(-1), self.bias, None if zp is None else rowsum, None if zp is None else zp.reshape(-1),
                              xzp, wcs.reshape(-1), -k, y, 0)
        return y.view(*input.shape[:-1], n)
    t = ops.lowrank_down(xrot if xrot is not None else x2, st.svd_down) if has_svd else None
    y = ops.scaled_mm_lowrank(ops.MM_I8, xq, wq, xs, ws, self.bias, t, st.svd_up, rowsum, zp, input.dtype, a_zp=xzp,
                              w_colsum_scaled=wcs)
    return y.view(*input.shape[:-1], n)


def _uint8_lp_matmul_forward(self, input: torch.Tensor, st: _State, conv_form: bool = False) -> torch.Tensor:
    dq = self.sdnq_dequantizer
    sdt = st.qw.scale_dtype
    k, n = dq.in_features, dq.out_features
    if sdt != torch.bfloat16 or input.dtype != sdt:
        raise NotImplementedError(f"the uint8 matmul with 16-bit scales is built for bfloat16 layers (scale dtype {sdt}, activations {input.dtype})")
    has_svd = st.svd_up is not None
    if has_svd and st.svd_up.dtype != sdt:
        raise NotImplementedError(f"the uint8 matmul with bfloat16 scales needs bfloat16 SVD factors (got {st.svd_up.dtype})")
    wq, ws, zp = _prepare_mm_weights(self, st, ops.MM_I8, asymmetric=True)
    wcs = st.mm_wcs
    if wcs is None:
        wcs = wq.to(torch.int32).sum(dim=1).to(torch.bfloat16).mul_(ws.reshape(-1).to(torch.bfloat16)).float()
        if CACHE_WEIGHTS:
            st.mm_wcs = wcs
    had = dq.hadamard_group_size if dq.use_hadamard else 0
    x2 = input.reshape(-1, k)
    if x2.stride(-1) != 1 or (x2.stride(0) * x2.element_size()) % 16:
        x2 = x2.contiguous()
    xq, xs, xzp, rowsum, xrot = ops.rowquant_lp_asym(x2, had, want_rowsum=zp is not None, want_xrot=has_svd)
    t = ops.lowrank_down(xrot if xrot is not None else x2, st.svd_down) if has_svd else None
    y = ops.scaled_mm_lp_uzp(xq, wq, xs, ws, _attr(self, "bias"), rowsum, zp, xzp, wcs, zp_k=-k if conv_form else 0, t=t,
                             svd_up=st.svd_up if has_svd else None)
    return y.view(*input.shape[:-1], n)


@_no_grad
def quantized_linear_forward_uint8_matmul(self, input: torch.Tensor) -> torch.Tensor:
    return _uint8_matmul_forward(self, input)


def _fp16_matmul_forward(self, input: torch.Tensor, small_batch_branch: bool = True) -> torch.Tensor:
    dq = self.sdnq_dequantizer
    st = _state(self)
    k, n = dq.in_features, dq.out_features
    m = input.numel() // input.shape[-1]
    if small_batch_branch and m < 32:
        return _float_forward(self, input, st)
    if not input.is_cuda:
        raise ops._lib.SdnqHipError("sdnq_amd forwards need CUDA/HIP tensors (no CPU fallback)")
    key = ("f16", False)
    if st.mm != key or st.mm_weight is None:
        if dq.re_quantize_for_matmul:
            w16, ws = ops.rowquant_f16(ops.dequant(st.qw, torch.float32, 0, use_svd=False).reshape(n, -1))
        else:
            w16, ws = ops.unpack_mm_f16(st.qw), st.qw.keep[1]
        st.mm, st.mm_weight, st.mm_scale, st.mm_zp, st.mm_wcs = key, w16, ws.reshape(-1), None, None
    x2 = input.reshape(-1, k)
    if x2.stride(-1) != 1 or (x2.stride(0) * x2.element_size()) % 16:
        x2 = x2.contiguous()
    if dq.use_hadamard:
        x2 = ops.hadamard(x2, dq.hadamard_group_size)
    bias = _attr(self, "bias")
    if st.svd_up is not None:
        t = ops.lowrank_down(x2, st.svd_down)
        bias = ops.linear_float(t, st.svd_up.contiguous(), None if bias is None else bias.to(st.svd_up.dtype))
    xq, xs = ops.rowquant_f16(x2)
    return ops.scaled_mm_f16(xq, st.mm_weight, xs, st.mm_scale, bias, input.dtype).view(*input.shape[:-1], n)


@_no_grad
def quantized_linear_forward_fp16_matmul(self, input: torch.Tensor) -> torch.Tensor:
    return _fp16_matmul_forward(self, input)


class _SwitchModule(__import__("types").ModuleType):

    def __setattr__(self, name, value):
        super().__setattr__(name, value)
        if name.isupper() and _FP is not None:
            _FP.bump_epoch()

    def __delattr__(self, name):
        super().__delattr__(name)
        if name.isupper() and _FP is not None:
            _FP.bump_epoch()


__import__("sys").modules[__name__].__class__ = _SwitchModule
```

sdnq_amd/ops.py:

```python
from __future__ import annotations

import ctypes
import os
from dataclasses import dataclass

import torch

from . import _lib
from ._lib import BF16, F16, F32, MM_FP8, MM_I8, SdnqWeight, check
from .common import dtype_dict

_FLOAT_CODE = {torch.float32: F32, torch.bfloat16: BF16, torch.float16: F16}
_MM_TORCH = {MM_I8: torch.int8, MM_FP8: torch.float8_e4m3fn}


def float_code(dt: torch.dtype) -> int:
    try:
        return _FLOAT_CODE[dt]
    except KeyError:
        raise _lib.SdnqHipError(f"unsupported float dtype {dt}") from None


def mm_code(matmul_dtype: str) -> int:
    if matmul_dtype == "int8":
# ... 103 lines not shown
    up = down = None
    rank, svd_dt = 0, 0
    if svd_up is not None:
        if svd_transposed:
            up = svd_up.t().contiguous()
            down = svd_down.t().contiguous()
        else:
            up = svd_up.contiguous()
            down = svd_down.contiguous()
        rank = up.shape[1]
        svd_dt = float_code(up.dtype)
    d = SdnqWeight(weight=_ptr(w_phys), scale=_ptr(sc), zero_point=_ptr(zp), svd_up=_ptr(up), svd_down=_ptr(down),
                   n=n, k=k, group_size=group_size, svd_rank=rank, svd_dtype=svd_dt, storage=storage, kind=kind,
                   bits=bits, exponent=ebits, mantissa=mbits, native_float=native, positions=positions,
                   scale_dtype=float_code(scale_dtype))
    return QuantWeight(desc=d, n=n, k=k, group_size=group_size, keep=(w_phys, sc, zp, up, down), scale_dtype=scale_dtype)


def rowquant(x2d: torch.Tensor, mm: int, hadamard_group: int = 0, want_rowsum: bool = False, want_xrot: bool = False,
             prefetch: torch.Tensor | None = None, asymmetric: bool = False):
    _require_cuda(x2d)
    assert x2d.ndim == 2 and x2d.stride(1) == 1
    m, k = x2d.shape
    xq = torch.empty((m, k), device=x2d.device, dtype=_MM_TORCH[mm])
    xs = torch.empty((m, 1), device=x2d.device, dtype=torch.float32)
    rowsum = torch.empty((m,), device=x2d.device, dtype=torch.int32) if want_rowsum else None
    mfma_rot = hadamard_group == 256 and x2d.dtype != torch.float32 and k <= 16384 and not asymmetric
    need_rot = bool(hadamard_group) and (want_xrot or (k > 5120 and not mfma_rot))
    xrot = torch.empty((m, k), device=x2d.device, dtype=x2d.dtype) if need_rot else None
    xzp = torch.empty((m,), device=x2d.device, dtype=torch.float32) if asymmetric else None
    check(_lib.load().sdnq_hip_rowquant(x2d.data_ptr(), float_code(x2d.dtype), m, k, x2d.stride(0), mm, hadamard_group,
                                        xq.data_ptr(), xs.data_ptr(), _ptr(rowsum), _ptr(xrot), _ptr(prefetch),
                                        0 if prefetch is None else prefetch.numel() * prefetch.element_size(), _ptr(xzp),
                                        _stream(x2d)), "rowquant")
    if not want_xrot:
        xrot = None
    if asymmetric:
        return xq, xs, rowsum, xrot, xzp
    return xq, xs, rowsum, xrot


def colquant_t(x2d: torch.Tensor, want_colsum: bool = False):
    _require_cuda(x2d)
    assert x2d.ndim == 2 and x2d.stride(1) == 1
    r, c = x2d.shape
    lib = _lib.load()
    nbytes = lib.sdnq_hip_colquant_t_workspace_bytes(r, c)
    if nbytes < 0:
        check(int(nbytes), "colquant_t")
    ld_t = (r + 15) // 16 * 16
    xq_t = torch.empty((c, ld_t), device=x2d.device, dtype=torch.int8)
    xs = torch.empty((c, 1), device=x2d.device, dtype=torch.float32)
    colsum = torch.empty((c,), device=x2d.device, dtype=torch.float32) if want_colsum else None
    ws = torch.empty((nbytes,), device=x2d.device, dtype=torch.uint8)
    check(lib.sdnq_hip_colquant_t(x2d.data_ptr(), float_code(x2d.dtype), r, c, x2d.stride(0), xq_t.data_ptr(), ld_t, xs.data_ptr(),
                                  _ptr(colsum), ws.data_ptr(), nbytes, _stream(x2d)), "colquant_t")
    return xq_t, xs, colsum


def rowquant_lp(x2d: torch.Tensor, mm: int, hadamard_group: int = 0, want_rowsum: bool = False, want_xrot: bool = False):
    _require_cuda(x2d)
    assert x2d.ndim == 2 and x2d.stride(1) == 1 and x2d.dtype in (torch.bfloat16, torch.float16)
    m, k = x2d.shape
    xq = torch.empty((m, k), device=x2d.device, dtype=_MM_TORCH[mm])
    xs = torch.empty((m, 1), device=x2d.device, dtype=torch.float32)
    rowsum = torch.empty((m,), device=x2d.device, dtype=torch.int32) if want_rowsum else None
    xrot = torch.empty((m, k), device=x2d.device, dtype=x2d.dtype) if (hadamard_group and want_xrot) else None
    check(_lib.load().sdnq_hip_rowquant_lp(x2d.data_ptr(), float_code(x2d.dtype), m, k, x2d.stride(0), mm, hadamard_group,
                                           xq.data_ptr(), xs.data_ptr(), _ptr(rowsum), _ptr(xrot), _stream(x2d)), "rowquant_lp")
    return xq, xs, rowsum, xrot


def rowquant_lp_asym(x2d: torch.Tensor, hadamard_group: int = 0, want_rowsum: bool = False, want_xrot: bool = False):
    _require_cuda(x2d)
    assert x2d.ndim == 2 and x2d.stride(1) == 1 and x2d.dtype in (torch.bfloat16, torch.float16)
    m, k = x2d.shape
    xq = torch.empty((m, k), device=x2d.device, dtype=torch.int8)
    xs = torch.empty((m, 1), device=x2d.device, dtype=torch.float32)
    xzp = torch.empty((m,), device=x2d.device, dtype=torch.float32)
    rowsum = torch.empty((m,), device=x2d.device, dtype=torch.int32) if want_rowsum else None
    xrot = torch.empty((m, k), device=x2d.device, dtype=x2d.dtype) if (want_xrot and hadamard_group) else None
    check(_lib.load().sdnq_hip_rowquant_lp_asym(x2d.data_ptr(), float_code(x2d.dtype), m, k, x2d.stride(0), hadamard_group, xq.data_ptr(),
                                                xs.data_ptr(), xzp.data_ptr(), _ptr(rowsum), _ptr(xrot), _stream(x2d)), "rowquant_lp_asym")
    return xq, xs, xzp, rowsum, xrot


def scaled_mm_lp_uzp(a: torch.Tensor, b_phys: torch.Tensor, sa: torch.Tensor, sb: torch.Tensor, bias, rowsum, zp, a_zp: torch.Tensor,
                     w_colsum_scaled: torch.Tensor, zp_k: int = 0, t=None, svd_up=None) -> torch.Tensor:
    _require_cuda(a, b_phys, sa, sb, bias, rowsum, zp, a_zp, w_colsum_scaled, t, svd_up)
    m, k = a.shape
    n = b_phys.shape[0]
    if bias is not None and bias.dtype != torch.bfloat16:
        raise _lib.SdnqHipError("scaled_mm_lp_uzp: bias must be bfloat16")
    out = torch.empty((m, n), device=a.device, dtype=torch.bfloat16)
    f32 = lambda t: None if t is None else t.reshape(-1).to(torch.float32).contiguous()
    sa_, sb_, zp_, azp_, wcs_ = f32(sa), f32(sb), f32(zp), f32(a_zp), f32(w_colsum_scaled)
    if t is not None:
        if t.dtype != torch.bfloat16 or svd_up.dtype != torch.bfloat16:
            raise _lib.SdnqHipError("scaled_mm_lp_uzp: low-rank factors must be bfloat16")
        t, svd_up = t.contiguous(), svd_up.contiguous()
        check(_lib.load().sdnq_hip_scaled_mm_lp_uzp_svd(a.data_ptr(), b_phys.data_ptr(), sa_.data_ptr(), sb_.data_ptr(), _ptr(None if bias is None else bias.contiguous()),
                                                        _ptr(rowsum), _ptr(zp_), azp_.data_ptr(), wcs_.data_ptr(), zp_k, t.data_ptr(), svd_up.data_ptr(),
                                                        t.shape[1], out.data_ptr(), m, n, k, _stream(a)), "scaled_mm_lp_uzp_svd")
        return out
    check(_lib.load().sdnq_hip_scaled_mm_lp_uzp(a.data_ptr(), b_phys.data_ptr(), sa_.data_ptr(), sb_.data_ptr(), _ptr(None if bias is None else bias.contiguous()),
                                                _ptr(rowsum), _ptr(zp_), azp_.data_ptr(), wcs_.data_ptr(), zp_k, out.data_ptr(), m, n, k, _stream(a)),
          "scaled_mm_lp_uzp")
    return out


def scaled_mm_lp(mm: int, a: torch.Tensor, b_phys: torch.Tensor, sa: torch.Tensor, sb: torch.Tensor, bias, t=None, svd_up=None,
                 rowsum=None, zp=None):
    _require_cuda(a, b_phys, sa, sb, bias, t, svd_up, rowsum, zp)
    m, k = a.shape
    n = b_phys.shape[0]
    out = torch.empty((m, n), device=a.device, dtype=torch.bfloat16)
    bias_ndim, ld_bias = 0, 0
    if bias is not None:
        if bias.dtype != torch.bfloat16:
            raise _lib.SdnqHipError("scaled_mm_lp: bias must be bfloat16")
        bias = bias.contiguous()
        bias_ndim, ld_bias = bias.ndim, bias.shape[-1]
    rank = 0
    if t is not None:
        if t.dtype != torch.bfloat16 or svd_up.dtype != torch.bfloat16:
            raise _lib.SdnqHipError("scaled_mm_lp: low-rank factors must be bfloat16")
        t, svd_up = t.contiguous(), svd_up.contiguous()
        rank = t.shape[1]
    if zp is not None:
        zp = zp.reshape(-1).contiguous()
        assert zp.dtype == torch.float32 and rowsum is not None and rowsum.dtype == torch.int32
    check(_lib.load().sdnq_hip_scaled_mm_lp_zp(mm, a.data_ptr(), b_phys.data_ptr(), sa.data_ptr(), sb.data_ptr(), _ptr(bias), bias_ndim,
                                               ld_bias, _ptr(t), _ptr(svd_up), rank, _ptr(rowsum if zp is not None else None), _ptr(zp),
                                               out.data_ptr(), m, n, k, _stream(a)), "scaled_mm_lp")
    return out


def scaled_mm(mm: int, a: torch.Tensor, b_phys: torch.Tensor, sa: torch.Tensor, sb: torch.Tensor, bias, out_dtype: torch.dtype):
    _require_cuda(a, b_phys, sa, sb, bias)
    m, k = a.shape
    n = b_phys.shape[0]
    out = torch.empty((m, n), device=a.device, dtype=out_dtype)
    bias_ndim, ld_bias, bias_dt = 0, 0, 0
    if bias is not None:
        bias = bias.contiguous()
        bias_ndim = bias.ndim
        ld_bias = bias.shape[-1]
        bias_dt = float_code(bias.dtype)
    check(_lib.load().sdnq_hip_scaled_mm(mm, a.data_ptr(), b_phys.data_ptr(), sa.data_ptr(), sb.data_ptr(), _ptr(bias),
                                         bias_dt, bias_ndim, ld_bias, out.data_ptr(), float_code(out_dtype), m, n, k,
                                         _stream(a)), "scaled_mm")
    return out


def scaled_mm_multi(mm: int, a: torch.Tensor, b_phys: torch.Tensor, sa: torch.Tensor, sb: torch.Tensor, bias, out_dtype: torch.dtype,
                    n_outs: int):
    _require_cuda(a, b_phys)
    m, k = a.shape
    n = b_phys.shape[0]
    seg = n // n_outs
    outs = [torch.empty((m, seg), device=a.device, dtype=out_dtype) for _ in range(n_outs)]
    ptrs = (ctypes.c_void_p * n_outs)(*[o.data_ptr() for o in outs])
    check(_lib.load().sdnq_hip_scaled_mm_multi(mm, a.data_ptr(), b_phys.data_ptr(), sa.data_ptr(), sb.data_ptr(), _ptr(bias),
                                               float_code(bias.dtype) if bias is not None else 0, ptrs, n_outs, seg, float_code(out_dtype),
                                               m, n, k, _stream(a)), "scaled_mm_multi")
    return outs


class GemmGroup:

    def __init__(self, members):
        import math
        import numpy as np
        ns = [int(w.shape[0]) for (w, _, _) in members]
        unit = 0
        for n in ns:
            unit = math.gcd(unit, n)
        if unit % 64:
            raise _lib.SdnqHipError(f"grouped matmul needs layer widths with a common divisor that is a multiple of 64 (got {ns})")
        while unit > 2048 and unit % 128 == 0:
            unit //= 2
        has_bias = members[0][2] is not None
        if any((b is not None) != has_bias for (_, _, b) in members):
            raise _lib.SdnqHipError("grouped matmul: either every layer has a bias or none has")
        self.k = int(members[0][0].shape[1])
        self.keep = []
        rows = []
        n_start = 0
        for (w, ws, bias) in members:
            _require_cuda(w, ws, bias)
            n = int(w.shape[0])
            if w.shape[1] != self.k or not w.is_contiguous() or w.element_size() != 1:
                raise _lib.SdnqHipError("grouped matmul: weights must be contiguous [N, K] 1-byte operands of one K")
            ws = ws.reshape(-1)
            if ws.dtype != torch.float32 or not ws.is_contiguous() or ws.numel() != n:
                raise _lib.SdnqHipError("grouped matmul: scales must be contiguous float32 [N]")
            if bias is not None:
                bias = bias.contiguous()
                if bias.dtype != members[0][2].dtype:
                    raise _lib.SdnqHipError("grouped matmul: one bias dtype per group")
            self.keep.append((w, ws, bias))
            for loc in range(0, n, unit):
                rows.append((w.data_ptr() + loc * self.k, ws.data_ptr() + 4 * loc,
                             0 if bias is None else bias.data_ptr() + loc * bias.element_size(), n_start, n, loc))
            n_start += n
        table = np.array(rows, dtype=np.dtype(_lib.SdnqGemmUnit))
        self.device = members[0][0].device
        self.table = torch.from_numpy(table.view(np.uint8).copy()).to(self.device)
        self.n_units, self.unit_n, self.n_total = len(rows), unit, n_start
        self.widths = ns
        self.bias_dtype = float_code(members[0][2].dtype) if has_bias else -1
        self.mm_torch = members[0][0].dtype


def scaled_mm_grouped(mm: int, a: torch.Tensor, sa: torch.Tensor, group: GemmGroup, out_dtype: torch.dtype):
    _require_cuda(a, sa)
    m, k = a.shape
    if k != group.k:
        raise _lib.SdnqHipError(f"grouped matmul: activation has K={k}, the group K={group.k}")
    out = torch.empty((m * group.n_total,), device=a.device, dtype=out_dtype)
    check(_lib.load().sdnq_hip_scaled_mm_grouped(mm, a.data_ptr(), sa.data_ptr(), group.table.data_ptr(), group.n_units, group.unit_n,
                                                 group.bias_dtype, out.data_ptr(), float_code(out_dtype), m, k, _stream(a)),
          "scaled_mm_grouped")
    outs, start = [], 0
    for n in group.widths:
        outs.append(out[m * start:m * (start + n)].view(m, n))
        start += n
    return outs


def linear_float_multi(x2d: torch.Tensor, wd: torch.Tensor, bias, n_outs: int):
    _require_cuda(x2d, wd)
    m, k = x2d.shape
    n = wd.shape[0]
    seg = n // n_outs
    outs = [torch.empty((m, seg), device=x2d.device, dtype=x2d.dtype) for _ in range(n_outs)]
    ptrs = (ctypes.c_void_p * n_outs)(*[o.data_ptr() for o in outs])
    check(_lib.load().sdnq_hip_linear_float_multi(x2d.data_ptr(), wd.data_ptr(), _ptr(bias), float_code(x2d.dtype), ptrs, n_outs, seg,
                                                  m, n, k, x2d.stride(0), _stream(x2d)), "linear_float_multi")
    return outs


def linear_w8a8(mm: int, x2d: torch.Tensor, b_phys: torch.Tensor, sb: torch.Tensor, bias, out_dtype: torch.dtype, hadamard_group: int = 0):
    m, k = x2d.shape
    n = b_phys.shape[0]
    dev = x2d.device
    xq = torch.empty((m, k), device=dev, dtype=_MM_TORCH[mm])
    xs = torch.empty((m, 1), device=dev, dtype=torch.float32)
    out = torch.empty((m, n), device=dev, dtype=out_dtype)
    bias_dt = 0
    if bias is not None:
        bias_dt = float_code(bias.dtype)
    check(_lib.load().sdnq_hip_linear_w8a8(mm, x2d.data_ptr(), float_code(x2d.dtype), m, k, x2d.stride(0), hadamard_group, xq.data_ptr(),
                                           xs.data_ptr(), b_phys.data_ptr(), sb.data_ptr(), _ptr(bias), bias_dt, out.data_ptr(),
                                           float_code(out_dtype), n, _stream(x2d)), "linear_w8a8")
    return out, xq, xs


def linear_w8a8_ws(mm: int, x2d: torch.Tensor, b_phys: torch.Tensor, sb: torch.Tensor, bias, out_dtype: torch.dtype, hadamard_group: int = 0):
    m, k = x2d.shape
    n = b_phys.shape[0]
    stream = _stream(x2d)
    xq_bytes = (m * k + 255) & ~255
    if torch.cuda.is_current_stream_capturing():
        scratch = torch.empty((xq_bytes + 4 * m + 512 + 255,), device=x2d.device, dtype=torch.uint8)
    else:
        scratch = _workspace(x2d.device, stream, xq_bytes + 4 * m + 512)
    base = (scratch.data_ptr() + 255) & ~255
    out = torch.empty((m, n), device=x2d.device, dtype=out_dtype)
    check(_lib.load().sdnq_hip_linear_w8a8(mm, x2d.data_ptr(), float_code(x2d.dtype), m, k, x2d.stride(0), hadamard_group, base,
                                           base + xq_bytes, b_phys.data_ptr(), sb.data_ptr(), _ptr(bias), 0 if bias is None else float_code(bias.dtype),
                                           out.data_ptr(), float_code(out_dtype), n, stream), "linear_w8a8")
    return out


def linear_w8a8_fused_supported(mm: int, x2d: torch.Tensor, n: int, out_dtype: torch.dtype) -> bool:
    if x2d.dtype not in (torch.bfloat16, torch.float16) or out_dtype != x2d.dtype or not x2d.is_cuda or x2d.stride(0) * 128 >= (1 << 31):
        return False
    key = (mm, x2d.dtype, x2d.shape[0], n, x2d.shape[1], x2d.device.index)
    r = _fused_ok.get(key)
    if r is None:
        with torch.cuda.device(x2d.device):
            r = bool(_lib.load().sdnq_hip_linear_w8a8_fused_supported(mm, float_code(x2d.dtype), float_code(out_dtype), x2d.shape[0], n, x2d.shape[1]))
        _fused_ok[key] = r
    return r


_fused_ok = {}
fused_calls = [0]


def fused_call_count() -> int:
    fp = _lib.fastpath()
    return fused_calls[0] + (fp.fused_calls() if fp is not None else 0)


def reset_fused_calls():
    fused_calls[0] = 0
    fp = _lib.fastpath()
    if fp is not None:
        fp.reset_counters()


def linear_w8a8_fused(mm: int, x2d: torch.Tensor, b_phys: torch.Tensor, sb: torch.Tensor, bias, out_dtype: torch.dtype) -> torch.Tensor:
    _require_cuda(x2d, b_phys, sb, bias)
    m, k = x2d.shape
    n = b_phys.shape[0]
    out = torch.empty((m, n), device=x2d.device, dtype=out_dtype)
    if bias is not None:
        bias = bias.contiguous()
    fused_calls[0] += 1
    check(_lib.load().sdnq_hip_linear_w8a8_fused(mm, x2d.data_ptr(), float_code(x2d.dtype), m, k, x2d.stride(0), b_phys.data_ptr(), sb.data_ptr(),
                                                 _ptr(bias), 0 if bias is None else float_code(bias.dtype), out.data_ptr(), float_code(out_dtype),
                                                 n, _stream(x2d)), "linear_w8a8_fused")
    return out


def scaled_mm_nchw(mm: int, a: torch.Tensor, b_phys: torch.Tensor, sa: torch.Tensor, sb: torch.Tensor, bias, out_dtype: torch.dtype,
                   batch: int, pixels: int) -> torch.Tensor:
    _require_cuda(a, b_phys, sa, sb, bias)
    m, k = a.shape
    n = b_phys.shape[0]
    assert m == batch * pixels
    out = torch.empty((batch, n, pixels), device=a.device, dtype=out_dtype)
    bias_dt = 0
    if bias is not None:
        bias = bias.contiguous()
        bias_dt = float_code(bias.dtype)
    check(_lib.load().sdnq_hip_scaled_mm_nchw(mm, a.data_ptr(), b_phys.data_ptr(), sa.data_ptr(), sb.data_ptr(), _ptr(bias), bias_dt,
                                              out.data_ptr(), float_code(out_dtype), m, n, k, pixels, _stream(a)), "scaled_mm_nchw")
    return out


def scaled_mm_into(mm: int, a: torch.Tensor, b_phys: torch.Tensor, sa: torch.Tensor, sb: torch.Tensor, bias, out: torch.Tensor,
                   chan0: int, pixels: int = 0) -> None:
    _require_cuda(a, b_phys, sa, sb, bias, out)
    m, k = a.shape
    n = b_phys.shape[0]
    assert a.stride(1) == 1 and b_phys.is_contiguous() and out.is_contiguous()
    c_total = out.shape[1]
    esz = out.element_size()
    dst = out.data_ptr() + (chan0 * pixels * esz if pixels else chan0 * esz)
    bias_dt = 0
    if bias is not None:
        bias = bias.contiguous()
        bias_dt = float_code(bias.dtype)
    check(_lib.load().sdnq_hip_scaled_mm_strided(mm, a.data_ptr(), a.stride(0), b_phys.data_ptr(), sa.data_ptr(), sb.data_ptr(), _ptr(bias),
                                                 bias_dt, dst, c_total, float_code(out.dtype), m, n, k, pixels, _stream(a)), "scaled_mm_strided")


def scaled_mm_zp_into(mm: int, a: torch.Tensor, b_phys: torch.Tensor, sa: torch.Tensor, sb: torch.Tensor, bias, rowsum, zp, a_zp, w_colsum_scaled,
                      zp_k: int, out: torch.Tensor, chan0: int) -> None:
    _require_cuda(a, b_phys, sa, sb, bias, rowsum, zp, a_zp, w_colsum_scaled, out)
    m, k = a.shape
    n = b_phys.shape[0]
    assert a.stride(1) == 1 and b_phys.is_contiguous() and out.is_contiguous() and out.dim() == 2
    bias_dt = 0
    if bias is not None:
        bias = bias.contiguous()
        bias_dt = float_code(bias.dtype)
    check(_lib.load().sdnq_hip_scaled_mm_lowrank_strided(mm, a.data_ptr(), a.stride(0), b_phys.data_ptr(), sa.data_ptr(), sb.data_ptr(), _ptr(bias),
                                                         bias_dt, _ptr(rowsum), _ptr(zp), _ptr(a_zp), _ptr(w_colsum_scaled), int(zp_k),
                                                         out.data_ptr() + chan0 * out.element_size(), out.shape[1], float_code(out.dtype), m, n, k,
                                                         _stream(a)), "scaled_mm_lowrank_strided")


def linear_float_into(x2d: torch.Tensor, w: torch.Tensor, bias, out: torch.Tensor, chan0: int) -> None:
    _require_cuda(x2d, w, bias, out)
    m, k = x2d.shape
    n = w.shape[0]
    assert w.is_contiguous() and x2d.stride(1) == 1 and w.dtype == x2d.dtype == out.dtype and out.is_contiguous()
    if bias is not None and bias.dtype != x2d.dtype:
        bias = bias.to(x2d.dtype)
    check(_lib.load().sdnq_hip_linear_float_strided(x2d.data_ptr(), w.data_ptr(), _ptr(bias), float_code(x2d.dtype),
                                                    out.data_ptr() + chan0 * out.element_size(), m, n, k, x2d.stride(0), out.shape[1],
                                                    _stream(x2d)), "linear_float_strided")


def scaled_mm_lowrank(mm: int, a, b_phys, sa, sb, bias, t, svd_up_phys, rowsum, zp, out_dtype: torch.dtype, a_zp=None,
                      w_colsum_scaled=None):
    _require_cuda(a, b_phys)
    m, k = a.shape
    n = b_phys.shape[0]
    out = torch.empty((m, n), device=a.device, dtype=out_dtype)
    rank = 0 if t is None else t.shape[1]
    svd_dt = 0 if t is None else float_code(t.dtype)
    bias_dt = 0
    if bias is not None:
        if t is not None and bias.dtype != t.dtype:
            bias = bias.to(t.dtype)
        bias = bias.contiguous()
        bias_dt = float_code(bias.dtype)
    check(_lib.load().sdnq_hip_scaled_mm_lowrank(mm, a.data_ptr(), b_phys.data_ptr(), sa.data_ptr(), sb.data_ptr(), _ptr(bias),
                                                 bias_dt, _ptr(t), _ptr(svd_up_phys), svd_dt, rank, _ptr(rowsum), _ptr(zp),
                                                 _ptr(a_zp), _ptr(w_colsum_scaled), out.data_ptr(), float_code(out_dtype), m, n, k, _stream(a)), "scaled_mm_lowrank")
    return out


def dequant(qw: QuantWeight, out_dtype: torch.dtype, hadamard_group: int = 0, use_svd: bool = True, out: torch.Tensor | None = None) -> torch.Tensor:
    dev = qw.keep[0].device
    if out is None:
        out = torch.empty((qw.n, qw.k), device=dev, dtype=out_dtype)
    d = qw.desc
    if not use_svd and d.svd_up:
        d = SdnqWeight.from_buffer_copy(bytes(d))
        d.svd_up = None
        d.svd_down = None
        d.svd_rank = 0
    check(_lib.load().sdnq_hip_dequant(ctypes.byref(d), hadamard_group, out.data_ptr(), float_code(out_dtype),
                                       torch.cuda.current_stream(dev).cuda_stream), "dequant")
    return out


def dequant_t(qw: QuantWeight, out_dtype: torch.dtype, out: torch.Tensor | None = None) -> torch.Tensor:
    dev = qw.keep[0].device
    if out is None:
        out = torch.empty((qw.k, qw.n), device=dev, dtype=out_dtype)
    elif out.dtype != out_dtype or out.numel() != qw.n * qw.k or not out.is_contiguous():
        raise _lib.SdnqHipError(f"dequant_t: out must be {qw.k * qw.n} contiguous elements of {out_dtype}")
    check(_lib.load().sdnq_hip_dequant_t(ctypes.byref(qw.desc), out.data_ptr(), float_code(out_dtype), _stream(out)), "dequant_t")
    return out.view(qw.k, qw.n)


def transpose2d(x: torch.Tensor, out: torch.Tensor | None = None) -> torch.Tensor:
    _require_cuda(x, out)
    if x.ndim != 2 or x.stride(1) != 1:
        raise _lib.SdnqHipError(f"transpose2d takes a 2-D tensor with contiguous rows (got shape {tuple(x.shape)}, strides {x.stride()})")
    r, c = x.shape
    if out is None:
        out = torch.empty((c, r), device=x.device, dtype=x.dtype)
    elif out.dtype != x.dtype or out.numel() != r * c or not out.is_contiguous():
        raise _lib.SdnqHipError(f"transpose2d: out must be {r * c} contiguous elements of {x.dtype}")
    check(_lib.load().sdnq_hip_transpose2d(x.data_ptr(), float_code(x.dtype), r, c, x.stride(0), out.data_ptr(), _stream(x)), "transpose2d")
    return out.view(c, r)


def weight_t(qw: QuantWeight, out_dtype: torch.dtype, hadamard_group: int, scratch) -> torch.Tensor:
    first, second = scratch
    nk = qw.n * qw.k
    if not qw.desc.svd_up and not hadamard_group:
        return dequant_t(qw, out_dtype, out=first[:nk])
    if second is None:
        raise _lib.SdnqHipError("weight_t: a layer with SVD factors or a Hadamard rotation needs the second scratch buffer")
    wd = dequant(qw, out_dtype, hadamard_group, out=second[:nk].view(qw.n, qw.k))
    return transpose2d(wd, out=first[:nk])


def make_convt_weight(weights_dtype: str, weight: torch.Tensor, scale: torch.Tensor, zero_point, c_in: int, p_cols: int, kprod: int) -> QuantWeight:
    _require_cuda(weight, scale)
    storage, kind, bits, ebits, mbits, native = _storage_kind(weights_dtype)
    w_phys = weight if weight.is_contiguous() else weight.contiguous()
    if w_phys.dtype in (torch.int64, torch.bool):
        w_phys = w_phys.to(torch.uint8)
    scale_dtype = scale.dtype
    if scale_dtype not in (torch.float32, torch.bfloat16, torch.float16):
        raise _lib.SdnqHipError(f"scale must be float32, bfloat16 or float16, got {scale_dtype}")
    if scale_dtype != torch.float32 and bits > 8:
        raise _lib.SdnqHipError("16-bit scales with formats wider than 8 bits are not built (the codes are not exact in the scale dtype)")
    if zero_point is not None and zero_point.dtype != scale_dtype:
        raise _lib.SdnqHipError("scale and zero_point must share one dtype (loader.py:277-280 casts both)")
    sc = scale.to(torch.float32).contiguous().view(-1)
    if sc.numel() == p_cols and (scale.ndim < 1 or scale.shape[0] == 1):
        num_groups = 1
    elif sc.numel() % (c_in * kprod) == 0 and scale.shape[0] == c_in:
        num_groups = sc.numel() // (c_in * kprod)
    else:
        raise _lib.SdnqHipError(f"scale of shape {tuple(scale.shape)} is neither [1, P] nor [C_in, 1, groups, *kernel] for C_in = {c_in}, P = {p_cols}")
    zp = None
    if zero_point is not None:
        zp = zero_point.to(torch.float32).contiguous().view(-1)
        if zp.numel() != sc.numel():
            raise _lib.SdnqHipError("zero_point size mismatch")
    d = SdnqWeight(weight=_ptr(w_phys), scale=_ptr(sc), zero_point=_ptr(zp), svd_up=None, svd_down=None, n=c_in, k=p_cols,
                   group_size=p_cols, svd_rank=0, svd_dtype=0, storage=storage, kind=kind, bits=bits, exponent=ebits, mantissa=mbits,
                   native_float=native, positions=kprod, scale_dtype=float_code(scale_dtype))
    return QuantWeight(desc=d, n=c_in, k=p_cols, group_size=num_groups, keep=(w_phys, sc, zp, None, None), scale_dtype=scale_dtype)


def dequant_convt(qw: QuantWeight, out_dtype: torch.dtype, groups: int = 1) -> torch.Tensor:
    dev = qw.keep[0].device
    if qw.n % groups:
        raise _lib.SdnqHipError(f"groups={groups} does not divide the {qw.n} input channels")
    out = torch.empty((groups, qw.k, qw.n // groups), device=dev, dtype=out_dtype)
    check(_lib.load().sdnq_hip_dequant_convt(ctypes.byref(qw.desc), groups, qw.group_size, out.data_ptr(), float_code(out_dtype),
                                             _stream(out)), "dequant_convt")
    return out


def linear_float_f32_into(x2d: torch.Tensor, w: torch.Tensor, out: torch.Tensor, col0: int) -> None:
    _require_cuda(x2d, w, out)
    m, k = x2d.shape
    n = w.shape[0]
    assert w.is_contiguous() and x2d.stride(1) == 1 and w.dtype == x2d.dtype and out.dtype == torch.float32 and out.is_contiguous()
    assert 0 <= col0 and col0 + n <= out.shape[1] and out.shape[0] == m and w.shape[1] == k
    check(_lib.load().sdnq_hip_linear_float_f32out_strided(x2d.data_ptr(), w.data_ptr(), float_code(x2d.dtype),
                                                           out.data_ptr() + col0 * 4, m, n, k, x2d.stride(0), out.shape[1],
                                                           _stream(x2d)), "linear_float_f32out_strided")


def col2im(cols: torch.Tensor, bias, out_dtype: torch.dtype, batch: int, channels: int, in_size, out_size, kernel, stride, padding,
           dilation) -> torch.Tensor:
    _require_cuda(cols, bias)
    nd = len(in_size)
    lead = 3 - nd

    def three(v, fill):
        return [fill] * lead + [int(e) for e in v]
    i3, o3, k3, s3, p3, d3 = three(in_size, 1), three(out_size, 1), three(kernel, 1), three(stride, 1), three(padding, 0), three(dilation, 1)
    if cols.dtype != torch.float32 or cols.ndim != 2 or cols.stride(1) != 1 or cols.shape[0] != batch * i3[0] * i3[1] * i3[2]:
        raise _lib.SdnqHipError("col2im expects float32 cols [batch * input positions, columns]")
    if bias is not None:
        bias = bias.to(out_dtype).contiguous()
        if bias.numel() != channels:
            raise _lib.SdnqHipError("col2im: bias must hold one value per output channel")
    out = torch.empty((batch, channels, *[int(e) for e in out_size]), device=cols.device, dtype=out_dtype)
    check(_lib.load().sdnq_hip_col2im(cols.data_ptr(), cols.stride(0), _ptr(bias), float_code(out_dtype), out.data_ptr(), batch, channels,
                                      *i3, *o3, *k3, *s3, *p3, *d3, _stream(cols)), "col2im")
    return out


def dequant_loss_sum(qw: QuantWeight, ref: torch.Tensor, hadamard_group: int = 0) -> torch.Tensor:
    _require_cuda(ref)
    dev = qw.keep[0].device
    if ref.device != dev:
        raise _lib.SdnqHipError(f"dequant_loss: ref on {ref.device}, weight on {dev}")
    r = ref.reshape(qw.n, -1) if ref.dim() != 2 else ref
    if tuple(r.shape) != (qw.n, qw.k):
        raise _lib.SdnqHipError(f"dequant_loss: ref shape {tuple(ref.shape)} is not [N, K] = ({qw.n}, {qw.k})")
    if r.stride(1) != 1 or r.data_ptr() % 16 or (r.stride(0) * r.element_size()) % 16:
        r = r.contiguous()
    lib = _lib.load()
    nbytes = int(lib.sdnq_hip_dequant_loss_workspace_bytes(qw.n, qw.k))
    check(nbytes if nbytes < 0 else 0, "dequant_loss_workspace_bytes")
    ws = torch.empty((nbytes // 8 + 1,), device=dev, dtype=torch.float64)
    out = ws[-1:]
    check(lib.sdnq_hip_dequant_loss(ctypes.byref(qw.desc), hadamard_group, r.data_ptr(), float_code(r.dtype), r.stride(0), out.data_ptr(),
                                    ws.data_ptr(), nbytes, _stream(r)), "dequant_loss")
    return out.view(())


def dequant_loss(qw: QuantWeight, ref: torch.Tensor, hadamard_group: int = 0) -> float:
    return float(dequant_loss_sum(qw, ref, hadamard_group).item())


def embedding(qw: QuantWeight, ids: torch.Tensor, out_dtype: torch.dtype, hadamard_group: int = 0, embed_scale: float | None = None) -> torch.Tensor:
    _require_cuda(ids)
    if ids.dtype not in (torch.int32, torch.int64):
        raise _lib.SdnqHipError(f"embedding ids must be int32 or int64, got {ids.dtype}")
    dev = qw.keep[0].device
    if ids.device != dev:
        raise _lib.SdnqHipError(f"embedding ids on {ids.device}, table on {dev}")
    flat = ids if ids.is_contiguous() else ids.contiguous()
    out = torch.empty((*ids.shape, qw.k), device=dev, dtype=out_dtype)
    check(_lib.load().sdnq_hip_embedding(ctypes.addressof(qw.desc), hadamard_group, flat.data_ptr(),
                                         _lib.IDS_I64 if ids.dtype == torch.int64 else _lib.IDS_I32, flat.numel(),
                                         0 if embed_scale is None else 1, 0.0 if embed_scale is None else float(embed_scale),
                                         out.data_ptr(), float_code(out_dtype), _stream(flat)), "embedding")
    return out


def requant(qw: QuantWeight, mm: int, ws: torch.Tensor | None = None, out: torch.Tensor | None = None):
    dev = qw.keep[0].device
    if out is not None:
        assert out.is_cuda and out.element_size() == 1 and out.numel() >= qw.n * qw.k and out.data_ptr() % 16 == 0
        wq = out[: qw.n * qw.k].view(_MM_TORCH[mm]).view(qw.n, qw.k)
    else:
        wq = torch.empty((qw.n, qw.k), device=dev, dtype=_MM_TORCH[mm])
    known = ws is not None
    if not known:
        ws = torch.empty((qw.n,), device=dev, dtype=torch.float32)
    check(_lib.load().sdnq_hip_requant_ws(ctypes.byref(qw.desc), mm, wq.data_ptr(), ws.data_ptr(), 1 if known else 0,
                                          torch.cuda.current_stream(dev).cuda_stream), "requant")
    return wq, ws


def lut4_build(qw: QuantWeight, mm: int, ws: torch.Tensor | None = None):
    dev = qw.keep[0].device
    lut = torch.empty((qw.n, qw.k // 64, 16), device=dev, dtype=torch.uint8)
    known = ws is not None
    if not known:
        ws = torch.empty((qw.n,), device=dev, dtype=torch.float32)
    check(_lib.load().sdnq_hip_lut4_build(ctypes.byref(qw.desc), mm, ws.data_ptr(), 1 if known else 0, lut.data_ptr(),
                                          torch.cuda.current_stream(dev).cuda_stream), "lut4_build")
    return lut, ws


def scaled_mm_w4_supported(mm: int, m: int, n: int, k: int, out_dtype: torch.dtype) -> bool:
    return out_dtype in (torch.bfloat16, torch.float16) and bool(_lib.load().sdnq_hip_scaled_mm_w4_supported(mm, float_code(out_dtype), m, n, k))


def scaled_mm_w4(a: torch.Tensor, codes: torch.Tensor, lut: torch.Tensor, sa: torch.Tensor, sb: torch.Tensor, bias, out_dtype: torch.dtype):
    _require_cuda(a, codes, lut, sa, sb, bias)
    m, k = a.shape
    n = lut.shape[0]
    if a.stride(-1) != 1 or codes.numel() * codes.element_size() != n * k // 2 or not codes.is_contiguous() or tuple(lut.shape) != (n, k // 64, 16):
        raise _lib.SdnqHipError("scaled_mm_w4: a [M, K] int8 (unit inner stride), contiguous packed codes of N * K / 2 bytes, lut [N, K / 64, 16]")
    out = torch.empty((m, n), device=a.device, dtype=out_dtype)
    check(_lib.load().sdnq_hip_scaled_mm_w4(a.data_ptr(), codes.data_ptr(), lut.data_ptr(), sa.data_ptr(), sb.data_ptr(), _ptr(bias),
                                            0 if bias is None else float_code(bias.dtype), out.data_ptr(), float_code(out_dtype), m, n, k,
                                            a.stride(0), _stream(a)), "scaled_mm_w4")
    return out


def rowquant_f16(x2d: torch.Tensor):
    _require_cuda(x2d)
    m, k = x2d.shape
    if x2d.stride(-1) != 1:
        raise _lib.SdnqHipError("rowquant_f16: unit inner stride")
    xq = torch.empty((m, k), device=x2d.device, dtype=torch.float16)
    xs = torch.empty((m,), device=x2d.device, dtype=torch.float32)
    check(_lib.load().sdnq_hip_rowquant_f16(x2d.data_ptr(), float_code(x2d.dtype), m, k, x2d.stride(0), xq.data_ptr(), xs.data_ptr(), _stream(x2d)), "rowquant_f16")
    return xq, xs


# ... 771 lines not shown
```

Baseline: 633,300 GOP/s.

## Add fragment-ordered weight slab copy and direct-to-register B loads in fused rowquant GEMM

Adds a one-time pack kernel that rewrites int8 weights into an MFMA-fragment-ordered slab, cached per layer. The fused activation-quant GEMM gets a DIRECT mode that loads these fragments straight from global memory into registers through a small ring of stages, skipping the LDS staging of B. The slab is used only for the geometry-1 int8 tall-skinny plan, and the prefetch hint now targets the slab. The cost is an extra copy of each eligible weight in memory, plus a risk that direct global loads hide latency worse than the LDS pipeline.

After: 639,900 GOP/s, median of 6. +1.0%, better.

```diff
diff --git a/include/sdnq_hip.h b/include/sdnq_hip.h
--- a/include/sdnq_hip.h
+++ b/include/sdnq_hip.h
@@ -211,6 +211,13 @@
 int sdnq_hip_linear_w8a8_fused(int mm_dtype, const void* x, int x_dtype, int64_t m, int64_t k, int64_t ldx, const void* b, const float* sb,
                                const void* bias, int bias_dtype, void* out, int out_dtype, int64_t n, sdnq_stream_t stream);
 int sdnq_hip_linear_w8a8_fused_supported(int mm_dtype, int x_dtype, int out_dtype, int64_t m, int64_t n, int64_t k);
+
+int64_t sdnq_hip_aq_slab_bytes(int64_t n, int64_t k);
+int sdnq_hip_aq_slab_wanted(int mm_dtype, int64_t m, int64_t n, int64_t k);
+int sdnq_hip_aq_slab_pack(const void* b, int64_t n, int64_t k, int64_t ldb, void* out, sdnq_stream_t stream);
+int sdnq_hip_linear_w8a8_fused_slab(int mm_dtype, const void* x, int x_dtype, int64_t m, int64_t k, int64_t ldx, const void* b,
+                                    const float* sb, const void* bias, int bias_dtype, void* out, int out_dtype, int64_t n,
+                                    const void* b_slab, sdnq_stream_t stream);
 
 typedef struct SdnqLinearArgs {
     int32_t struct_size;
diff --git a/sdnq_amd/capture.py b/sdnq_amd/capture.py
--- a/sdnq_amd/capture.py
+++ b/sdnq_amd/capture.py
@@ -37,7 +37,7 @@
     for mod in model.modules():
         st = mod.__dict__.get("_sdnq_hip_state")
         if st is not None:
-            for name in ("mm_weight", "mm_scale"):
+            for name in ("mm_weight", "mm_scale", "mm_slab"):
                 t = getattr(st, name, None)
                 if isinstance(t, torch.Tensor):
                     fp.append((t.data_ptr(), t.numel(), t.dtype))
diff --git a/sdnq_amd/csrc/fastpath.cpp b/sdnq_amd/csrc/fastpath.cpp
--- a/sdnq_amd/csrc/fastpath.cpp
+++ b/sdnq_amd/csrc/fastpath.cpp
@@ -20,7 +20,7 @@
 namespace {
 
 decltype(&sdnq_hip_linear_w8a8) f_linear_w8a8 = nullptr;
-decltype(&sdnq_hip_linear_w8a8_fused) f_fused = nullptr;
+decltype(&sdnq_hip_linear_w8a8_fused_slab) f_fused = nullptr;
 decltype(&sdnq_hip_linear_w8a8_fused_supported) f_fused_supported = nullptr;
 decltype(&sdnq_hip_prefetch_hint) f_hint = nullptr;
 decltype(&sdnq_hip_stream_capture_id) f_capture_id = nullptr;
@@ -312,6 +312,7 @@
     vectorcallfunc vc;
     std::vector<KeyEnt>* keys;
     at::Tensor* wq;
+    at::Tensor* wslab;
     at::Tensor* ws;
     at::Tensor* bias;
     int mm, had, device, bias_code;
@@ -405,7 +406,7 @@
         int rc;
         if (fused) {
             rc = f_fused(p->mm, x2.data_ptr(), code, m, p->k, x2.stride(0), p->wq->data_ptr(), (const float*)p->ws->data_ptr(), bias, p->bias_code,
-                         out.data_ptr(), code, p->n, stream);
+                         out.data_ptr(), code, p->n, p->wslab->defined() ? p->wslab->data_ptr() : nullptr, stream);
             g_fused_calls.fetch_add(1, std::memory_order_relaxed);
         } else {
             const int64_t xq_bytes = (m * p->k + 255) & ~(int64_t)255;
@@ -426,12 +427,12 @@
 }
 
 PyObject* plan_new(PyTypeObject* type, PyObject* args, PyObject* kw) {
-    static const char* kwlist[] = {"names", "refs", "mm", "n", "k", "wq", "ws", "bias", "had", "allow_fused", "allow_ws", "unit", "group", "idx", nullptr};
-    PyObject *names, *refs, *wq = Py_None, *ws = Py_None, *bias = Py_None, *unit = Py_None, *group = Py_None;
+    static const char* kwlist[] = {"names", "refs", "mm", "n", "k", "wq", "ws", "bias", "had", "allow_fused", "allow_ws", "unit", "group", "idx", "wslab", nullptr};
+    PyObject *names, *refs, *wq = Py_None, *ws = Py_None, *bias = Py_None, *unit = Py_None, *group = Py_None, *wslab = Py_None;
     int mm = 0, had = 0, allow_fused = 0, allow_ws = 0, idx = 0;
     long long n = 0, k = 0;
-    if (!PyArg_ParseTupleAndKeywords(args, kw, "OOiLL|OOOippOOi", (char**)kwlist, &names, &refs, &mm, &n, &k, &wq, &ws, &bias, &had, &allow_fused, &allow_ws, &unit,
-                                     &group, &idx))
+    if (!PyArg_ParseTupleAndKeywords(args, kw, "OOiLL|OOOippOOiO", (char**)kwlist, &names, &refs, &mm, &n, &k, &wq, &ws, &bias, &had, &allow_fused, &allow_ws, &unit,
+                                     &group, &idx, &wslab))
         return nullptr;
     if (!PyTuple_Check(names) || !PyTuple_Check(refs) || PyTuple_GET_SIZE(names) != PyTuple_GET_SIZE(refs)) {
         PyErr_SetString(PyExc_TypeError, "names and refs must be tuples of one length");
@@ -441,11 +442,13 @@
     if (group != Py_None && !PyObject_TypeCheck(group, &GroupType)) { PyErr_SetString(PyExc_TypeError, "group must be a Group"); return nullptr; }
     if (group == Py_None && (!THPVariable_Check(wq) || !THPVariable_Check(ws))) { PyErr_SetString(PyExc_TypeError, "wq / ws must be tensors"); return nullptr; }
     if (bias != Py_None && !THPVariable_Check(bias)) { PyErr_SetString(PyExc_TypeError, "bias must be a tensor or None"); return nullptr; }
+    if (wslab != Py_None && !THPVariable_Check(wslab)) { PyErr_SetString(PyExc_TypeError, "wslab must be a tensor or None"); return nullptr; }
     PlanObj* p = (PlanObj*)type->tp_alloc(type, 0);
     if (!p) return nullptr;
     p->vc = plan_call;
     p->keys = new std::vector<KeyEnt>();
     p->wq = new at::Tensor();
+    p->wslab = new at::Tensor();
     p->ws = new at::Tensor();
     p->bias = new at::Tensor();
     p->unit = nullptr;
@@ -489,6 +492,14 @@
                 return nullptr;
             }
             p->device = (int)p->wq->device().index();
+            if (wslab != Py_None) {
+                *p->wslab = THPVariable_Unpack(wslab);
+                if (!p->wslab->is_cuda() || p->wslab->device() != p->wq->device() || !p->wslab->is_contiguous()) {
+                    PyErr_SetString(PyExc_ValueError, "wslab must be a contiguous tensor on wq's device");
+                    Py_DECREF(p);
+                    return nullptr;
+                }
+            }
             if (bias != Py_None) {
                 *p->bias = THPVariable_Unpack(bias);
                 p->bias_code = float_code(p->bias->scalar_type());
@@ -519,6 +530,7 @@
         delete p->keys;
     }
     delete p->wq;
+    delete p->wslab;
     delete p->ws;
     delete p->bias;
     delete p->unit;
@@ -540,7 +552,7 @@
     var = (decltype(var))dlsym(h, #name);                                                                           \
     if (!var) { PyErr_Format(PyExc_OSError, "%s does not export " #name, path); return nullptr; }
     RESOLVE(f_linear_w8a8, sdnq_hip_linear_w8a8)
-    RESOLVE(f_fused, sdnq_hip_linear_w8a8_fused)
+    RESOLVE(f_fused, sdnq_hip_linear_w8a8_fused_slab)
     RESOLVE(f_fused_supported, sdnq_hip_linear_w8a8_fused_supported)
     RESOLVE(f_hint, sdnq_hip_prefetch_hint)
     RESOLVE(f_capture_id, sdnq_hip_stream_capture_id)
diff --git a/sdnq_amd/csrc/gemm_aq.hip b/sdnq_amd/csrc/gemm_aq.hip
--- a/sdnq_amd/csrc/gemm_aq.hip
+++ b/sdnq_amd/csrc/gemm_aq.hip
@@ -63,10 +63,14 @@
     constexpr bool SLAB = BN / 32 == NW;
     constexpr int KS = BK / MT::KB;
     static_assert(!SLAB || (NSB <= NJ && PPW == 4), "register slab: the ring is no deeper than the stages held; a wave's 32 rows are four pieces");
+    constexpr bool DIRECT = NSB < 0;
+    constexpr int RD = !DIRECT ? 0 : (-NSB < NJ ? -NSB : NJ);
+    constexpr int NSL = DIRECT ? 0 : NSB;
+    static_assert(!DIRECT || (SLAB && MM == SDNQ_MM_I8 && KS == 4 && RD >= 1 && KS * RD <= 48), "direct form: the int8 slab tile; the loads in flight fit the vmcnt counter");
     extern __shared__ __attribute__((aligned(1024))) uint8_t lds[];
     uint8_t* const ldsA = lds;
     uint8_t* const ldsB = lds + NJ * A_STAGE;
-    float* const s_sb = (float*)(ldsB + NSB * B_STAGE);
+    float* const s_sb = (float*)(ldsB + NSL * B_STAGE);
     float* const s_bias = s_sb + BN;
     float* const s_xs = s_bias + BN;
 
@@ -96,7 +100,9 @@
 #pragma unroll
         for (int j = 0; j < NJ; ++j) xr[ps][j] = SDNQ_BUF_LOAD16(rsX, vo, j < nk ? j * 256 : 0x40000000);
     }
-    const auto rsB = SDNQ_MAKE_RSRC_N(w + (int64_t)n0 * ldb, (int64_t)(n_lim - 1) * ldb + K);
+    const int nblk = (n_lim + 31) >> 5;
+    const auto rsB = DIRECT ? SDNQ_MAKE_RSRC_N(w + (int64_t)tile_n * (BN / 32) * nk * 4096, nblk * nk * 4096)
+                            : SDNQ_MAKE_RSRC_N(w + (int64_t)n0 * ldb, (int64_t)(n_lim - 1) * ldb + K);
     int voB[PPW];
     auto pieceB = [&](int u) { return SLAB ? wave * PPW + u : wave + u * NW; };
 #pragma unroll
@@ -110,9 +116,24 @@
 #pragma unroll
         for (int u = 0; u < PPW; ++u) SDNQ_DMA16(rsB, ldsB + slot * B_STAGE + pieceB(u) * 1024, voB[u], s * BK);
     };
-    constexpr int AHEAD = SLAB ? NSB : NSB - 1;
-#pragma unroll
-    for (int s = 0; s < AHEAD; ++s) issueB(s, s);
+    constexpr int AHEAD = DIRECT ? RD : (SLAB ? NSB : NSB - 1);
+    typename MT::frag_t fbd[DIRECT ? RD : 1][KS];
+    const int voD = lane << 4, soD = (wave < nblk ? wave : nblk - 1) * nk * 4096;
+    auto issueD = [&](auto slotc, auto ksc, int st) {
+        constexpr int ks = decltype(ksc)::value;
+        if constexpr (DIRECT) fbd[decltype(slotc)::value][ks] = SDNQ_BUF_LOAD16(rsB, voD, soD + (st < nk ? st : 0) * 4096 + ks * 1024);
+    };
+    if constexpr (DIRECT) {
+        static_for_up<RD>([&](auto sc) {
+            static_for_up<KS>([&](auto ksc) {
+                issueD(sc, ksc, decltype(sc)::value);
+                __builtin_amdgcn_sched_barrier(0);
+            });
+        });
+    } else {
+#pragma unroll
+        for (int s = 0; s < AHEAD; ++s) issueB(s, s);
+    }
     __builtin_amdgcn_sched_barrier(0);
     SDNQ_KERNARGS_NOW("s"(p_.sb), "s"(p_.bias), "s"(p_.out), "s"(p_.ldc), "s"(p_.bias_dtype), "s"(p_.trace));
     if (p.trace != nullptr && tid == 0 && blockIdx.x < 1024) p.trace[blockIdx.x * 8] = t_entry;
@@ -129,7 +150,7 @@
     }
 
     constexpr float QMAX = (MM == SDNQ_MM_I8) ? 127.0f : 448.0f;
-    constexpr int DF = !SLAB ? 0 : (NJ < 2 ? NJ : 2);
+    constexpr int DF = !SLAB || DIRECT ? 0 : (NJ < 2 ? NJ : 2);
     typename MT::frag_t fbr[DF > 0 ? DF : 1][KS], fbs[KS];
     auto drainB = [&](int j, typename MT::frag_t* dst) {
         if (j < nk) {
@@ -244,7 +265,33 @@
     constexpr int lab = 0;
 #endif
     typename MT::frag_t fa[2][NACC][KS];
-    if constexpr (SLAB) {
+    if constexpr (DIRECT) {
+        auto read_a = [&](auto setc, auto ksc, int st) {
+            constexpr int sx = decltype(setc)::value, ks = decltype(ksc)::value;
+#pragma unroll
+            for (int a = 0; a < NACC; ++a) fa[sx][a][ks] = MT::load(ldsA + (st < nk ? st : 0) * A_STAGE, (wm + a) * 32 + frow, ks, fgrp);
+        };
+        __builtin_amdgcn_s_barrier();
+        __builtin_amdgcn_sched_barrier(0);
+        static_for_up<KS>([&](auto ksc) { read_a(std::integral_constant<int, 0>{}, ksc, 0); });
+        static_for_up<NJ>([&](auto ktc) {
+            constexpr int kt = decltype(ktc)::value, sx = kt & 1, slot = kt % (RD > 0 ? RD : 1);
+            if (kt < nk) {
+                __builtin_amdgcn_sched_barrier(0);
+                static_for_up<KS>([&](auto ksc) {
+                    constexpr int ks = decltype(ksc)::value;
+                    if (!(lab & 4)) {
+#pragma unroll
+                        for (int a = 0; a < NACC; ++a) MT::mma(acc[a], fbd[slot][ks], fa[sx][a][ks]);
+                    }
+                    __builtin_amdgcn_sched_barrier(0);
+                    if constexpr (kt + 1 < NJ) { if (!(lab & 2)) read_a(std::integral_constant<int, sx ^ 1>{}, ksc, kt + 1); }
+                    if constexpr (kt + RD < NJ) issueD(std::integral_constant<int, slot>{}, ksc, kt + RD);
+                    __builtin_amdgcn_sched_barrier(0);
+                });
+            }
+        });
+    } else if constexpr (SLAB) {
         auto read_a = [&](auto setc, auto ksc, int st) {
             constexpr int sx = decltype(setc)::value, ks = decltype(ksc)::value;
 #pragma unroll
@@ -322,7 +369,7 @@
     SDNQ_PHASE_STAMP(p.trace, 4);
 
     constexpr int OUT_ROW = BN * 2 + 16;
-    static_assert(BM * OUT_ROW <= NJ * A_STAGE + NSB * B_STAGE, "output staging fits the operand area");
+    static_assert(BM * OUT_ROW <= NJ * A_STAGE + NSL * B_STAGE, "output staging fits the operand area");
 #pragma unroll
     for (int a = 0; a < NACC; ++a) {
         const int ml = (wm + a) * 32 + frow;
@@ -356,6 +403,15 @@
 
 std::atomic<unsigned long long*> g_aq_trace{nullptr};
 std::atomic<int> g_aq_geometry{-1};
+std::atomic<int> g_aq_direct{-1};
+
+constexpr int AQ_DIRECT_STAGES = 3;
+inline int aq_direct_norm(int f) { return f == 0 ? 0 : AQ_DIRECT_STAGES; }
+inline int aq_direct_stages() {
+    static const int env = aq_direct_norm((int)env_int("SDNQ_HIP_FUSED_ROWQUANT_DIRECT", AQ_DIRECT_STAGES));
+    const int forced = g_aq_direct.load(std::memory_order_relaxed);
+    return forced < 0 ? env : aq_direct_norm(forced);
+}
 
 constexpr int64_t AQ_TALL_MAX_K = 640;
 
@@ -393,7 +449,7 @@
 
 template <int X_T, int MM, bool HAS_BIAS, int NJ, int NSB, int BM, int BN, int RESIDENT = 1>
 int launch_aq(const void* x, const void* w, int64_t ldx, int64_t m, int64_t n, int64_t k, const AqPlan& pl, AqParams p, hipStream_t s) {
-    constexpr int LDS_BYTES = NJ * BM * BK + NSB * BN * BK + (2 * BN + BM) * 4;
+    constexpr int LDS_BYTES = NJ * BM * BK + (NSB < 0 ? 3 : NSB) * BN * BK + (2 * BN + BM) * 4;
     static_assert(RESIDENT * LDS_BYTES <= 160 * 1024 && (RESIDENT + 1) * LDS_BYTES > 160 * 1024, "LDS budget: exactly RESIDENT workgroups per CU (aq_plan's prefetch room)");
     auto kern = linear_aq_kernel<X_T, MM, HAS_BIAS, NJ, NSB, BM, BN>;
     static std::atomic<uint64_t> attr_devices{0};
@@ -429,9 +485,44 @@
     return 1;
 }
 
-extern "C" int sdnq_hip_linear_w8a8_fused(int mm_dtype, const void* x, int x_dtype, int64_t m, int64_t k, int64_t ldx, const void* b,
-                                          const float* sb, const void* bias, int bias_dtype, void* out, int out_dtype, int64_t n,
-                                          sdnq_stream_t stream) {
+namespace {
+__global__ __launch_bounds__(256) void aq_slab_pack_kernel(const uint8_t* __restrict__ b, int64_t n, int nk, int64_t ldb, uint8_t* __restrict__ out, int64_t pieces) {
+    const int64_t t = (int64_t)blockIdx.x * 256 + threadIdx.x;
+    if (t >= pieces) return;
+    const int l = (int)(t & 63), ks = (int)(t >> 6) & 3;
+    const int64_t q = t >> 8, g = q / nk, j = q % nk;
+    const int64_t row = g * 32 + (l & 31);
+    const v4i v = *(const v4i*)(b + (row < n ? row : n - 1) * ldb + j * 128 + ks * 32 + (l >> 5) * 16);
+    *(v4i*)(out + t * 16) = v;
+}
+}
+
+extern "C" int64_t sdnq_hip_aq_slab_bytes(int64_t n, int64_t k) {
+    if (n <= 0 || k <= 0 || (k % 128) != 0) return 0;
+    return ((n + 31) / 32) * 32 * k;
+}
+
+extern "C" int sdnq_hip_aq_slab_wanted(int mm_dtype, int64_t m, int64_t n, int64_t k) {
+    if (mm_dtype != SDNQ_MM_I8 || m <= 0 || n <= 0 || k <= 0 || (k % 128) != 0 || k > 1280) return 0;
+    return aq_plan(mm_dtype, m, n, k, cu_count()).geometry == 1 && aq_direct_stages() != 0 ? 1 : 0;
+}
+
+extern "C" int sdnq_hip_aq_slab_pack(const void* b, int64_t n, int64_t k, int64_t ldb, void* out, sdnq_stream_t stream) {
+    if (!b || !out) return SDNQ_ERR_NULL;
+    if (n <= 0 || k <= 0 || ldb < k) return SDNQ_ERR_SHAPE;
+    if ((k % 128) != 0 || k > 1280) return SDNQ_ERR_UNSUPPORTED;
+    if (n > 0x7fffffffll / 2) return SDNQ_ERR_SHAPE;
+    if (((uintptr_t)b % 16) || ((uintptr_t)out % 16) || (ldb % 16)) return SDNQ_ERR_ALIGN;
+    const int64_t pieces = sdnq_hip_aq_slab_bytes(n, k) / 16;
+    hipLaunchKernelGGL(aq_slab_pack_kernel, dim3((unsigned)((pieces + 255) / 256)), dim3(256), 0, (hipStream_t)stream, (const uint8_t*)b, n, (int)(k / 128), ldb,
+                       (uint8_t*)out, pieces);
+    SDNQ_CHECK_LAUNCH();
+    return SDNQ_OK;
+}
+
+extern "C" int sdnq_hip_linear_w8a8_fused_slab(int mm_dtype, const void* x, int x_dtype, int64_t m, int64_t k, int64_t ldx, const void* b,
+                                               const float* sb, const void* bias, int bias_dtype, void* out, int out_dtype, int64_t n,
+                                               const void* b_slab, sdnq_stream_t stream) {
     if (!x || !b || !sb || !out) return SDNQ_ERR_NULL;
     if (mm_dtype != SDNQ_MM_I8 && mm_dtype != SDNQ_MM_FP8) return SDNQ_ERR_DTYPE;
     if ((x_dtype != SDNQ_BF16 && x_dtype != SDNQ_F16) || out_dtype != x_dtype) return SDNQ_ERR_UNSUPPORTED;
@@ -439,12 +530,18 @@
     if (m <= 0 || n <= 0 || k <= 0 || ldx < k || (n % 8) != 0) return SDNQ_ERR_SHAPE;
     if ((k % 128) != 0 || k > 1280) return SDNQ_ERR_UNSUPPORTED;
     if (m > 0x7fffffffll / 2 || n > 0x7fffffffll || ldx * 2 * 128 > 0x7fffffffll || k * 128 > 0x7fffffffll) return SDNQ_ERR_SHAPE;
-    if (((uintptr_t)x % 16) || ((uintptr_t)b % 16) || ((uintptr_t)out % 16) || ((ldx * 2) % 16)) return SDNQ_ERR_ALIGN;
+    if (((uintptr_t)x % 16) || ((uintptr_t)b % 16) || ((uintptr_t)out % 16) || ((ldx * 2) % 16) || ((uintptr_t)b_slab % 16)) return SDNQ_ERR_ALIGN;
     AqParams p{};
     p.sb = sb; p.bias = bias; p.out = out; p.ldc = n; p.bias_dtype = bias_dtype;
     hipStream_t s = (hipStream_t)stream;
     const AqPlan pl = aq_plan(mm_dtype, m, n, k, cu_count());
-#define AQ_L(XT, MMV, HB, NJV, ...) launch_aq<XT, MMV, HB, NJV, __VA_ARGS__>(x, b, ldx, m, n, k, pl, p, s)
+    const bool direct = pl.geometry == 1 && mm_dtype == SDNQ_MM_I8 && b_slab != nullptr && aq_direct_stages() != 0;
+    const void* const w = direct ? b_slab : b;
+#define AQ_L(XT, MMV, HB, NJV, ...) launch_aq<XT, MMV, HB, NJV, __VA_ARGS__>(x, w, ldx, m, n, k, pl, p, s)
+#define AQ_D(XT, HB, NJV) AQ_L(XT, SDNQ_MM_I8, HB, NJV, -AQ_DIRECT_STAGES, 32, 256)
+#define AQ_DB(XT, HB) (k <= 640 ? AQ_D(XT, HB, 5) : AQ_D(XT, HB, 10))
+#define AQ_DX(XT) (bias ? AQ_DB(XT, true) : AQ_DB(XT, false))
+    if (direct) return x_dtype == SDNQ_BF16 ? AQ_DX(SDNQ_BF16) : AQ_DX(SDNQ_F16);
 #define AQ_G(XT, MMV, HB, NJV) (pl.geometry == 1 ? AQ_L(XT, MMV, HB, NJV, 3, 32, 256) : AQ_L(XT, MMV, HB, NJV, 4, 64, 128))
 #define AQ_NJ(XT, MMV, HB) (k <= 640 ? AQ_G(XT, MMV, HB, 5) : AQ_G(XT, MMV, HB, 10))
 #define AQ_B(XT, MMV) (bias ? AQ_NJ(XT, MMV, true) : AQ_NJ(XT, MMV, false))
@@ -460,12 +557,23 @@
 #undef AQ_B
 #undef AQ_NJ
 #undef AQ_G
+#undef AQ_DX
+#undef AQ_DB
+#undef AQ_D
 #undef AQ_L
 }
 
+extern "C" int sdnq_hip_linear_w8a8_fused(int mm_dtype, const void* x, int x_dtype, int64_t m, int64_t k, int64_t ldx, const void* b,
+                                          const float* sb, const void* bias, int bias_dtype, void* out, int out_dtype, int64_t n,
+                                          sdnq_stream_t stream) {
+    return sdnq_hip_linear_w8a8_fused_slab(mm_dtype, x, x_dtype, m, k, ldx, b, sb, bias, bias_dtype, out, out_dtype, n, nullptr, stream);
+}
+
 void sdnq_internal_aq_trace(unsigned long long* device_buf) { g_aq_trace.store(device_buf, std::memory_order_relaxed); }
 
 void sdnq_internal_aq_geometry(int geometry) { g_aq_geometry.store(geometry < 0 ? -1 : (geometry <= 3 ? geometry : 1), std::memory_order_relaxed); }
+
+void sdnq_internal_aq_direct(int form) { g_aq_direct.store(form < 0 ? -1 : aq_direct_norm(form), std::memory_order_relaxed); }
 
 void sdnq_internal_aq_plan(int mm_dtype, long long m, long long n, long long k, int cus, long long* out) {
     const AqPlan pl = aq_plan(mm_dtype, m, n, k, cus);
diff --git a/sdnq_amd/csrc/gemm_dev.h b/sdnq_amd/csrc/gemm_dev.h
--- a/sdnq_amd/csrc/gemm_dev.h
+++ b/sdnq_amd/csrc/gemm_dev.h
@@ -17,6 +17,7 @@
 void sdnq_internal_ks_trace(unsigned long long* device_buf);
 void sdnq_internal_aq_trace(unsigned long long* device_buf);
 void sdnq_internal_aq_geometry(int geometry);
+void sdnq_internal_aq_direct(int form);
 void sdnq_internal_aq_plan(int mm_dtype, long long m, long long n, long long k, int cus, long long* out);
 
 template <int N> __device__ __forceinline__ void wait_vmcnt() { asm volatile("s_waitcnt vmcnt(%0)" ::"n"(N) : "memory"); }
diff --git a/sdnq_amd/linear.py b/sdnq_amd/linear.py
--- a/sdnq_amd/linear.py
+++ b/sdnq_amd/linear.py
@@ -18,6 +18,7 @@
 FUSED_DEQUANT_GEMM_MAX_FLOP = float(os.environ.get("SDNQ_HIP_FUSED_DEQUANT_GEMM_MAX_FLOP", "4e10"))
 FUSED_DEQUANT_GEMM_MAX_K = int(os.environ.get("SDNQ_HIP_FUSED_DEQUANT_GEMM_MAX_K", str(1 << 30)))
 FUSED_ROWQUANT = os.environ.get("SDNQ_HIP_FUSED_ROWQUANT", "1").lower() not in {"0", "false", "no"}
+FUSED_ROWQUANT_SLABCOPY = os.environ.get("SDNQ_HIP_FUSED_ROWQUANT_SLABCOPY", "1").lower() not in {"0", "false", "no"}
 FUSED_LUT4 = os.environ.get("SDNQ_HIP_FUSED_LUT4", "1").lower() not in {"0", "false", "no"}
 CACHE_ACTIVATIONS = int(os.environ.get("SDNQ_HIP_CACHE_ACTIVATIONS", "12"))
 _FP = ops._lib.fastpath()
@@ -193,7 +194,7 @@
 
 
 class _State:
-    __slots__ = ("key", "qw", "mm", "mm_weight", "mm_scale", "mm_zp", "mm_wcs", "svd_up", "svd_down", "svd_down_t", "wd", "bias", "pf", "lut")
+    __slots__ = ("key", "qw", "mm", "mm_weight", "mm_slab", "mm_scale", "mm_zp", "mm_wcs", "svd_up", "svd_down", "svd_down_t", "wd", "bias", "pf", "lut")
 
 
 class _LaunchUnit:
@@ -334,7 +335,7 @@
     st.qw = dq.quant_weight(mod.weight, mod.scale, getattr(mod, "zero_point", None), getattr(mod, "svd_up", None),
                             getattr(mod, "svd_down", None))
     st.mm = None
-    st.mm_weight = st.mm_scale = st.mm_zp = st.mm_wcs = None
+    st.mm_weight = st.mm_slab = st.mm_scale = st.mm_zp = st.mm_wcs = None
     st.svd_up, st.svd_down = st.qw.keep[3], st.qw.keep[4]
     st.svd_down_t = None
     st.wd = None
@@ -522,11 +523,22 @@
                 zp = torch.add(zp, ws, alpha=128) if zp is not None else ws * 128
                 if st.qw.scale_dtype != torch.float32:
                     zp = zp.to(st.qw.scale_dtype).float()
+    st.mm_slab = None
     if CACHE_WEIGHTS:
         st.mm, st.mm_weight, st.mm_scale, st.mm_zp, st.mm_wcs = key, wq, ws, zp, None
     elif dq.re_quantize_for_matmul and not asymmetric:
         st.mm, st.mm_weight, st.mm_scale, st.mm_zp, st.mm_wcs = key, None, ws, None, None
     return wq, ws, zp
+
+
+def _aq_slab(st: _State, mm: int, wq: torch.Tensor, m: int, n: int, k: int):
+    if not FUSED_ROWQUANT_SLABCOPY or mm != ops.MM_I8 or st.mm_weight is not wq:
+        return None
+    slab = st.mm_slab
+    if slab is None and ops.aq_slab_wanted(mm, m, n, k, wq.device) and not torch.cuda.is_current_stream_capturing():
+        if wq.dim() == 2 and wq.stride(1) == 1 and wq.stride(0) % 16 == 0 and wq.data_ptr() % 16 == 0:
+            slab = st.mm_slab = ops.aq_slab_pack(wq)
+    return slab
 
 
 class ProjectionGroup:
@@ -764,23 +776,29 @@
     had = dq.hadamard_group_size if dq.use_hadamard else 0
     has_svd = st.svd_up is not None
     bias = _attr(self, "bias")
+    plain = not has_svd and zp is None and (had == 0 or k <= 5120)
+    use_cache = cache_input and CACHE_ACTIVATIONS > 0
+    x2 = slab = None
+    one_launch = False
+    if (plain and FUSED_ROWQUANT and had == 0 and input.is_cuda
+            and (not use_cache or (UNSHARED_FAST_PATH and self.__dict__.get("_sdnq_unshared", 0) >= UNSHARED_AFTER))):
+        x2 = input if input.dim() == 2 else input.reshape(-1, k)
+        if x2.stride(-1) != 1 or (x2.stride(0) * x2.element_size()) % 16:
+            x2 = x2.contiguous()
+        one_launch = ops.linear_w8a8_fused_supported(mm, x2, n, input.dtype)
+        if one_launch:
+            slab = _aq_slab(st, mm, wq, x2.shape[0], n, k)
     pf_on = PREFETCH_NEXT and st.mm_weight is wq and input.is_cuda
     if pf_on:
-        _pf_launch(st, (wq,))
+        _pf_launch(st, (wq,) if slab is None else (slab,))
     plannable = cache_input and small_batch_branch and group is None and st.mm_weight is wq
-    if not has_svd and zp is None and (had == 0 or k <= 5120):
-        use_cache = cache_input and CACHE_ACTIVATIONS > 0
-        if (FUSED_ROWQUANT and had == 0 and input.is_cuda
-                and (not use_cache or (UNSHARED_FAST_PATH and self.__dict__.get("_sdnq_unshared", 0) >= UNSHARED_AFTER))):
-            x2 = input if input.dim() == 2 else input.reshape(-1, k)
-            if x2.stride(-1) != 1 or (x2.stride(0) * x2.element_size()) % 16:
-                x2 = x2.contiguous()
-            if ops.linear_w8a8_fused_supported(mm, x2, n, input.dtype):
-                y = ops.linear_w8a8_fused(mm, x2, wq, ws, bias, input.dtype)
-                if FAST_PLANS and plannable and "_sdnq_plan_declined" not in self.__dict__:
-                    _install_plan(self, mm=mm, n=n, k=k, wq=wq, ws=ws, bias=bias, had=0, allow_fused=True,
-                                  allow_ws=use_cache and UNSHARED_FAST_PATH, unit=st.pf.c if pf_on else None)
-                return y if input.dim() == 2 else y.view(*input.shape[:-1], n)
+    if plain:
+        if one_launch:
+            y = ops.linear_w8a8_fused(mm, x2, wq, ws, bias, input.dtype, slab)
+            if FAST_PLANS and plannable and "_sdnq_plan_declined" not in self.__dict__:
+                _install_plan(self, mm=mm, n=n, k=k, wq=wq, ws=ws, bias=bias, had=0, allow_fused=True,
+                              allow_ws=use_cache and UNSHARED_FAST_PATH, unit=st.pf.c if pf_on else None, wslab=slab)
+            return y if input.dim() == 2 else y.view(*input.shape[:-1], n)
         if (use_cache and UNSHARED_FAST_PATH and self.__dict__.get("_sdnq_unshared", 0) >= UNSHARED_AFTER and input.is_cuda
                 and not torch.cuda.is_current_stream_capturing()):
             x2 = input if input.dim() == 2 else input.reshape(-1, k)
@@ -968,7 +986,7 @@
             w16, ws = ops.rowquant_f16(ops.dequant(st.qw, torch.float32, 0, use_svd=False).reshape(n, -1))
         else:
             w16, ws = ops.unpack_mm_f16(st.qw), st.qw.keep[1]
-        st.mm, st.mm_weight, st.mm_scale, st.mm_zp, st.mm_wcs = key, w16, ws.reshape(-1), None, None
+        st.mm, st.mm_weight, st.mm_slab, st.mm_scale, st.mm_zp, st.mm_wcs = key, w16, None, ws.reshape(-1), None, None
     x2 = input.reshape(-1, k)
     if x2.stride(-1) != 1 or (x2.stride(0) * x2.element_size()) % 16:
         x2 = x2.contiguous()
diff --git a/sdnq_amd/ops.py b/sdnq_amd/ops.py
--- a/sdnq_amd/ops.py
+++ b/sdnq_amd/ops.py
@@ -429,7 +429,34 @@
         fp.reset_counters()
 
 
-def linear_w8a8_fused(mm: int, x2d: torch.Tensor, b_phys: torch.Tensor, sb: torch.Tensor, bias, out_dtype: torch.dtype) -> torch.Tensor:
+def aq_slab_bytes(n: int, k: int) -> int:
+    return int(_lib.load().sdnq_hip_aq_slab_bytes(n, k))
+
+
+_slab_wanted = {}
+
+
+def aq_slab_wanted(mm: int, m: int, n: int, k: int, device) -> bool:
+    key = (mm, m, n, k, device.index)
+    r = _slab_wanted.get(key)
+    if r is None:
+        with torch.cuda.device(device):
+            r = _slab_wanted[key] = bool(_lib.load().sdnq_hip_aq_slab_wanted(mm, m, n, k))
+    return r
+
+
+def aq_slab_pack(b_phys: torch.Tensor) -> torch.Tensor:
+    _require_cuda(b_phys)
+    n, k = b_phys.shape
+    nbytes = aq_slab_bytes(n, k)
+    if nbytes == 0 or b_phys.stride(1) != 1 or b_phys.element_size() != 1:
+        raise _lib.SdnqHipError(f"aq_slab_pack: no slab copy for a weight of shape {tuple(b_phys.shape)}, strides {b_phys.stride()}, {b_phys.dtype}")
+    out = torch.empty(nbytes, device=b_phys.device, dtype=torch.int8)
+    check(_lib.load().sdnq_hip_aq_slab_pack(b_phys.data_ptr(), n, k, b_phys.stride(0), out.data_ptr(), _stream(b_phys)), "aq_slab_pack")
+    return out
+
+
+def linear_w8a8_fused(mm: int, x2d: torch.Tensor, b_phys: torch.Tensor, sb: torch.Tensor, bias, out_dtype: torch.dtype, slab=None) -> torch.Tensor:
     _require_cuda(x2d, b_phys, sb, bias)
     m, k = x2d.shape
     n = b_phys.shape[0]
@@ -437,6 +464,11 @@
     if bias is not None:
         bias = bias.contiguous()
     fused_calls[0] += 1
+    if slab is not None:
+        check(_lib.load().sdnq_hip_linear_w8a8_fused_slab(mm, x2d.data_ptr(), float_code(x2d.dtype), m, k, x2d.stride(0), b_phys.data_ptr(), sb.data_ptr(),
+                                                          _ptr(bias), 0 if bias is None else float_code(bias.dtype), out.data_ptr(), float_code(out_dtype),
+                                                          n, slab.data_ptr(), _stream(x2d)), "linear_w8a8_fused_slab")
+        return out
     check(_lib.load().sdnq_hip_linear_w8a8_fused(mm, x2d.data_ptr(), float_code(x2d.dtype), m, k, x2d.stride(0), b_phys.data_ptr(), sb.data_ptr(),
                                                  _ptr(bias), 0 if bias is None else float_code(bias.dtype), out.data_ptr(), float_code(out_dtype),
                                                  n, _stream(x2d)), "linear_w8a8_fused")
```
